# jhyau/AdaptiGraph

Hardware: AMD Instinct MI355X
Metric: rollout-steps/sec (higher is better)
Workload: dtype f32; 1 GPU; BASELINE configs[3]: cloth, 1024 candidates x 20 rollout steps (2 look-ahead x repeat 10) x 2025+1 particles, radius graph rebuilt every step; candidates=1024, horizon=20, particles=2026, parallelism=candidates sharded over 1 GPU(s), all-gather of costs

## Files before the change

### adaptigraph_amd/csrc/ag_api.hip

```cpp
#include "ag_host.h"

#include <cstdarg>

using namespace ag;

namespace {

const char* kFamilyNames[FAM_COUNT] = {"edge_count", "edge_emit", "prep", "node_enc", "edge_enc",
                                       "mp", "node_prop", "node_final", "roll_init", "roll_update", "cost", "fps", "assemble", "rule", "surface"};

struct OptName { const char* name; const char* env; int Options::* field; bool env_negates; int lo, hi; };
const OptName kOptions[] = {
    {"streams", "AG_STREAMS", &Options::streams, false, 0, ag_ctx::kMaxStreams},
    {"chunk", "AG_CHUNK", &Options::chunk, false, 0, 1 << 20},
    {"latency", "AG_LATENCY", &Options::latency, false, -1, 1},
    {"ragged", "AG_NO_RAGGED", &Options::ragged, true, 0, 1},
    {"ell_graph", "AG_NO_ELL_GRAPH", &Options::ell_graph, true, 0, 1},
    {"self_dedupe", "AG_NO_SELF_DEDUPE", &Options::self_dedupe, true, 0, 1},
    {"repeat_sort", "AG_NO_REPEAT_SORT", &Options::repeat_sort, true, 0, 1},
    {"edge_wgs", "AG_EDGE_WGS", &Options::edge_wgs, false, 1, 1 << 16},
    {"edge_block_min", "AG_EDGE_BLOCK_MIN", &Options::edge_block_min, false, -1, 0x7fffffff},
    {"enc_persist", "AG_ENC_PERSIST", &Options::enc_persist, false, 0, 1 << 20},
    {"stagger_us", "AG_STAGGER_US", &Options::stagger_us, false, 0, 1000},
    {"device_decode", "AG_DEVICE_DECODE", &Options::device_decode, false, -1, 1},
    {"zigzag", "AG_ZIGZAG", &Options::zigzag, false, 0, 1},
    {"share_first", "AG_SHARE_FIRST", &Options::share_first, false, -1, 1},
    {"zero_skip", "AG_ZERO_SKIP", &Options::zero_skip, false, 0, 1},
    {"half_step", "AG_HALF_STEP", &Options::half_step, false, 0, 1},
    {"share_prefix", "AG_SHARE_PREFIX", &Options::share_prefix, false, -1, 1},
    {"stream_min_rows", "AG_STREAM_MIN_ROWS", &Options::stream_min_rows, false, 0, 0x7fffffff},
    {"pipeline_fork", "AG_PIPELINE_FORK", &Options::pipeline_fork, false, 0, 1},
    {"edge_order", "AG_EDGE_ORDER", &Options::edge_order, false, 0, 1},
    {"ell_lds_words", "AG_ELL_LDS_WORDS", &Options::ell_lds_words, false, 0, 16384},
};
void options_from_env(Options& o) {
    for (const OptName& n : kOptions)
        if (const char* e = getenv(n.env)) o.*(n.field) = n.env_negates ? (atoi(e) ? 0 : 1) : std::min(n.hi, std::max(n.lo, atoi(e)));
}

}

namespace ag {

int fail(ag_ctx* c, int code, const char* fmt, ...) {
    char buf[512];
    va_list ap;
    va_start(ap, fmt);
    vsnprintf(buf, sizeof buf, fmt, ap);
    va_end(ap);
    if (c) c->err = buf;
    return code;
}

int slot_acquire(ag_ctx* c, hipStream_t st, bool capturing, CallSlot** out) {
    CallSlot* s = nullptr;
    for (CallSlot& k : c->slots) if (k.bound && k.stream == st) { s = &k; break; }
    if (!s) for (CallSlot& k : c->slots) if (!k.bound) { s = &k; break; }
    if (!s) {
        s = &c->slots[0];
        for (CallSlot& k : c->slots) if (k.tick < s->tick) s = &k;
        if (!capturing && s->have_done) HIPCHK(c, hipStreamWaitEvent(st, s->ev_done, 0));
        s->census_pending = false;
    }
    if (!s->ev_done) {
        HIPCHK(c, event_new(c, &s->ev_done));
        HIPCHK(c, event_new(c, &s->ev_plan));
        HIPCHK(c, event_new(c, &s->ev_census));
        HIPCHK(c, event_new(c, &s->ev_fork));
        HIPCHK(c, dev_alloc(c, reinterpret_cast<void**>(&s->d_words), 256));
        HIPCHK(c, dev_alloc(c, reinterpret_cast<void**>(&s->d_share_stats), 256));
        HIPCHK(c, hipMemset(s->d_share_stats, 0, 256));
        HIPCHK(c, pin_alloc(c, reinterpret_cast<void**>(&s->h_census), 64));
    }
    s->bound = true; s->stream = st; s->tick = ++c->slot_tick;
    *out = s;
    return AG_OK;
}
void slot_release(CallSlot* s, hipStream_t st, bool capturing) {
    if (capturing || !s || !s->ev_done) return;
    if (hipEventRecord(s->ev_done, st) == hipSuccess) s->have_done = true;
}
bool other_slot_busy(ag_ctx* c, const CallSlot* me) {
    bool busy = false;
    for (CallSlot& k : c->slots)
        if (&k != me && k.bound && k.have_done) {
            if (hipEventQuery(k.ev_done) == hipErrorNotReady) busy = true;
            (void)hipGetLastError();
        }
    return busy;
}
int begin_call(ag_ctx* c, void* stream, SlotGuard& call, bool watch_capture) {
    HIPCHK(c, hipSetDevice(c->device));
    call.st = static_cast<hipStream_t>(stream);
    c->prof_stream = call.st;
    if (watch_capture) {
        hipStreamCaptureStatus status = hipStreamCaptureStatusNone;
        call.capturing = hipStreamIsCapturing(call.st, &status) == hipSuccess && status == hipStreamCaptureStatusActive;
    }
    return slot_acquire(c, call.st, call.capturing, &call.sl);
}
void slot_destroy(ag_ctx* c, CallSlot& s) {
    for (hipEvent_t e : {s.ev_plan, s.ev_census, s.ev_done, s.ev_fork}) if (e) (void)hipEventDestroy(e);
    for (int i = 1; i < CallSlot::kMaxStreams; ++i) {
        if (s.ev_join[i]) (void)hipEventDestroy(s.ev_join[i]);
        if (s.aux_stream[i]) (void)hipStreamDestroy(s.aux_stream[i]);
    }
    if (s.h_plan_max) (void)hipHostFree(s.h_plan_max);
    if (s.h_rep_pin) (void)hipHostFree(s.h_rep_pin);
    if (s.h_census) (void)hipHostFree(s.h_census);
    if (s.d_words) (void)hipFree(s.d_words);
    if (s.d_share_stats) (void)hipFree(s.d_share_stats);
    if (s.d_repeat) (void)hipFree(s.d_repeat);
    if (s.d_plan) (void)hipFree(s.d_plan);
    if (s.d_work) (void)hipFree(s.d_work);
    if (s.slab.base) (void)hipFree(s.slab.base);
    s = CallSlot();
}

void prof_mark(void* vc, int fam, int phase) {
    ag_ctx* c = static_cast<ag_ctx*>(vc);
    if (!(c->prof_mask & (1u << fam))) return;
    auto get = [&]() {
        hipEvent_t e;
        if (!c->prof_pool.empty()) { e = c->prof_pool.back(); c->prof_pool.pop_back(); }
        else (void)hipEventCreate(&e);
        return e;
    };
    if (phase == 0) {
        ProfEvent p{fam, get(), get()};
        (void)hipEventRecord(p.e0, c->prof_stream);
        c->prof_live.push_back(p);
    } else {
        for (auto it = c->prof_live.rbegin(); it != c->prof_live.rend(); ++it)
            if (it->fam == fam) { (void)hipEventRecord(it->e1, c->prof_stream); break; }
    }
}

void carve_work(const ag_ctx* c, Slab& s, Work& w, int Bc, int N, int n_inst, int edge_cap, int c_cap, int slices, bool own_edges,
                bool roll, bool own_group, int N_o, int ell_stride) {
    const size_t rows = (size_t)Bc * N;
    w.g.node_in = s.take<float>(rows * NODE_IN);
    w.g.feat12 = s.take<float>(rows * F15_PITCH);
    w.g.group = own_group ? s.take<float>(rows * n_inst) : nullptr;
    w.g.eff = s.take<float>(rows * NFP);
    w.g.P = s.take<float>(rows * NFP);
    for (int par = 0; par < 2; ++par)
        for (int k = 0; k < 2; ++k) w.g.UV[par][k] = s.take<float>(rows * NFP);
    w.g.C = s.take<float>(((size_t)Bc * c_cap + 256) * NFP);
    w.g.B = Bc; w.g.N = N; w.g.n_inst = n_inst; w.g.edge_cap = edge_cap; w.g.c_cap = c_cap; w.g.n_p = N_o;
    w.g.enc_persist = c->opt.enc_persist; w.g.stagger_us = c->opt.stagger_us; w.g.zigzag = c->opt.zigzag; w.g.diag = c->diag;
    w.g.zero_skip = c->opt.zero_skip && c->w_finite; w.g.half_step = w.g.zero_skip && c->opt.half_step;
    if (own_edges) {
        w.ell = s.take<int>(rows * (size_t)std::max(1, ell_stride));
        w.deg = s.take<int>(rows);
        w.slice_tot = s.take<int>((size_t)Bc * slices);
        w.cta_flag = s.take<int>(Bc);
        w.recv = s.take<int>((size_t)Bc * edge_cap);
        w.send = s.take<int>((size_t)Bc * edge_cap);
        w.row_ptr = s.take<int>((size_t)Bc * (N + 1));
        w.n_edges = s.take<int>(Bc);
        w.ns_edge = s.take<int>((size_t)Bc * edge_cap);
        w.n_ns = s.take<int>(Bc);
        w.n_oo = s.take<int>(Bc);
        w.g.recv = w.recv; w.g.send = w.send; w.g.row_ptr = w.row_ptr; w.g.n_edges = w.n_edges;
    }
    if (roll) {
        w.send_pk = s.take<int>((size_t)Bc * edge_cap);
        w.rowlist = s.take<int>(rows);
        w.n_rows = s.take<int>((size_t)Bc + 64);
        w.r.hist = s.take<float>((size_t)Bc * N_HIS_MAX * N * 3);
        w.r.pred = s.take<float>((size_t)Bc * N_o * 3);
        w.r.motion = s.take<float>((size_t)Bc * N_o * 3);
        w.r.mask = s.take<uint8_t>(rows);
        w.r.tool = s.take<uint8_t>(rows);
        const size_t cr = (size_t)cls_rows(N_o, N - N_o, Bc);
        w.g.cls_on = 1; w.g.N_o = N_o; w.g.M = N - N_o; w.g.vmask = w.r.mask;
        w.g.c_node_in = s.take<float>(cr * NODE_IN);
        w.g.c_eff = s.take<float>(cr * NFP);
        w.g.c_P = s.take<float>(cr * NFP);
        w.g.c_U = s.take<float>(cr * NFP);
        w.g.c_V = s.take<float>(cr * NFP);
    }
}

int pick_slices(const ag_ctx* c, int B, int N) {
    const int target = std::max(1, c->opt.edge_wgs);
    int s = (target + B - 1) / B;
    s = std::min(s, std::max(1, N / 16));
    return std::max(1, std::min(s, 128));
}

int clamp_chunk_for_offsets(int Bc, int N, int c_cap) {
    const long max_rows = ((1L << 32) / NFP) - 512;
    const long by_c = max_rows / std::max(1, c_cap);
    const long by_n = max_rows / std::max(1, N);
    return (int)std::max(1L, std::min<long>(Bc, std::min(by_c, by_n)));
}

int auto_chunk(const ag_ctx* c, int B, int N) {
    if (c->chunk > 0) return std::min(c->chunk, B);
    if (c->opt.chunk > 0) return std::min(c->opt.chunk, B);
    const long max_rows = 4L * 256 * 256;
    long bc = max_rows / N;
    return (int)std::max(1L, std::min<long>(bc, B));
}

bool lat_available(const ag_ctx* c, const GraphBufs& g) { return c->d_wlat && !g.wb3 && g.n_his != 5; }
bool lat_edge_for(const ag_ctx* c, const GraphBufs& g) {
    const long edge_wgs = (long)g.B * g.c_cap / 128;
    return lat_available(c, g) && (c->opt.latency >= 0 ? c->opt.latency == 1 : edge_wgs <= 128);
}
hipError_t node_enc_for(const ag_ctx* c, const GraphBufs& g, long row0, long nrows, hipStream_t st) {
    const long rows = g.cls_on ? nrows : (long)g.B * g.N;
    const bool lat = lat_available(c, g) && (c->opt.latency >= 0 ? c->opt.latency == 1 : rows <= 512L * 32);
    return lat ? launch_node_enc_lat(c->d_wlat, g, row0, nrows, st) : launch_node_enc(c->d_w, g, row0, nrows, st);
}
bool lat_node_for(const ag_ctx* c, const GraphBufs& g) {
    const long node_wgs = ((long)g.B * g.N + 127) / 128;
    return lat_available(c, g) && (c->opt.latency >= 0 ? c->opt.latency == 1 : node_wgs <= 64);
}
int run_edge_chain(ag_ctx* c, const GraphBufs& g, hipStream_t st) {
    Scoped p(c, FAM_EDGE_ENC);
    if (lat_edge_for(c, g)) HIPCHK(c, launch_edge_enc_lat(c->d_wlat, g, st));
    else HIPCHK(c, launch_edge_enc(c->d_w, g, st));
    return AG_OK;
}

int run_model(ag_ctx* c, const GraphBufs& g, float* pred_pos, float* pred_motion, hipStream_t st) {
    if (!g.cls_on) { Scoped p(c, FAM_NODE_ENC); HIPCHK(c, node_enc_for(c, g, 0, (long)g.B * g.N, st)); }
    const bool lat_node = lat_node_for(c, g);
    if (g.send_pk && lat_node) return fail(c, AG_ERR_INVALID, "internal: shared first forward on the latency-mode chains");
    int rc = run_edge_chain(c, g, st);
    if (rc) return rc;
    for (int ps = 0; ps < c->dims.pstep; ++ps) {
        const bool last = ps + 1 == c->dims.pstep;
        Scoped p(c, last ? FAM_NODE_FINAL : FAM_NODE_PROP);
        if (lat_node) HIPCHK(c, launch_node_prop_lat(c->d_wlat, g, ps, last, c->dims.motion_clamp, pred_pos, pred_motion, st));
        else if (!last) HIPCHK(c, launch_node_prop(c->d_w, g, ps, st));
        else HIPCHK(c, launch_node_final(c->d_w, g, ps, c->dims.motion_clamp, pred_pos, pred_motion, st));
    }
    return AG_OK;
}

struct SelfMini { float node_in[2 * NODE_IN]; float feat12[2 * F15_PITCH]; float group[2]; int recv[2]; int send[2]; int n_edges; int pad; };
int enqueue_self_rows(ag_ctx* c, hipStream_t st) {
    HIPCHK(c, hipSetDevice(c->device));
    if (!c->d_cself) HIPCHK(c, dev_alloc(c, reinterpret_cast<void**>(&c->d_cself), 256 * NFP * 4));
    if (!c->d_self_mini) {
        SelfMini h{};
        h.node_in[0] = 1.f; h.node_in[6] = 1.f;
        h.node_in[NODE_IN + 1] = 1.f; h.node_in[NODE_IN + 6] = 1.f;
        h.group[0] = 1.f;
        h.recv[0] = 0; h.recv[1] = 1; h.send[0] = 0; h.send[1] = 1; h.n_edges = 2;
        HIPCHK(c, dev_alloc(c, reinterpret_cast<void**>(&c->d_self_mini), sizeof(SelfMini)));
        HIPCHK(c, hipMemcpy(c->d_self_mini, &h, sizeof(SelfMini), hipMemcpyHostToDevice));
    }
    char* d = c->d_self_mini;
    GraphBufs g{};
    g.n_his = c->dims.n_his;
    g.node_in = reinterpret_cast<float*>(d + offsetof(SelfMini, node_in));
    g.feat12 = reinterpret_cast<float*>(d + offsetof(SelfMini, feat12));
    g.group = reinterpret_cast<float*>(d + offsetof(SelfMini, group));
    g.recv = reinterpret_cast<int*>(d + offsetof(SelfMini, recv));
    g.send = reinterpret_cast<int*>(d + offsetof(SelfMini, send));
    g.n_edges = reinterpret_cast<int*>(d + offsetof(SelfMini, n_edges));
    g.C = c->d_cself; g.B = 1; g.N = 2; g.n_p = 1; g.n_inst = 1; g.edge_cap = 2; g.c_cap = 256;
    g.wb3 = c->precision == 1 ? c->d_wb3 : nullptr;
    hipError_t e = launch_edge_enc(c->d_w, g, st);
    if (e != hipSuccess) return fail(c, AG_ERR_HIP, "self-loop C rows: %s", hipGetErrorString(e));
    return AG_OK;
}
int compute_self_rows(ag_ctx* c) {
    int rc = enqueue_self_rows(c, nullptr);
    if (rc) return rc;
    hipError_t e = hipDeviceSynchronize();
    if (e != hipSuccess) return fail(c, AG_ERR_HIP, "self-loop C rows: %s", hipGetErrorString(e));
    return AG_OK;
}

int check_topk(ag_ctx* c, int N, int topk) {
    if (N < 1 || topk < 1) return fail(c, AG_ERR_INVALID, "N and topk must be >= 1");
    if ((size_t)N > edge_build_max_particles()) return fail(c, AG_ERR_UNSUPPORTED, "N=%d exceeds the LDS-resident edge builder limit %zu", N, edge_build_max_particles());
    if (topk < N && topk > 128) return fail(c, AG_ERR_UNSUPPORTED, "topk=%d: 128 < topk < N is not implemented", topk);
    return AG_OK;
}

ForwardFrame::ForwardFrame(const ag_ctx* c, int B, int N_, int n_inst_, int edge_cap_, int n_p_, int n_guard_)
    : N(N_), n_inst(n_inst_), edge_cap(edge_cap_), n_p(n_p_), n_guard(n_guard_), c_cap((int)round_up(edge_cap_, 256)),
      Bc(clamp_chunk_for_offsets(auto_chunk(c, B, N_), N_, c_cap)) {}
void ForwardFrame::carve(const ag_ctx* c, Slab& s) {
    carve_work(c, s, w, Bc, N, n_inst, edge_cap, c_cap, 1, false, false, false, n_p, 0);
    n_eff = n_guard ? s.take<int>((size_t)n_guard) : nullptr;
}

int enqueue_forward(ag_ctx* c, const ForwardFrame& f, const float* d_state, const float* d_attrs, const float* d_action,
                    const float* d_phys, const float* d_group, const int32_t* d_recv, const int32_t* d_send,
                    const int32_t* d_row_ptr, const int* n_eff, int B, float* d_pred_pos, float* d_pred_motion, hipStream_t st) {
    const int Bc = f.Bc, N = f.N, n_inst = f.n_inst, edge_cap = f.edge_cap, n_p = f.n_p;
    int rc = AG_OK;
    for (int b0 = 0; b0 < B; b0 += Bc) {
        const int nb = std::min(Bc, B - b0);
        GraphBufs g = f.w.g;
        g.B = nb; g.n_p = n_p; g.n_his = c->dims.n_his;
        g.wb3 = c->precision == 1 ? c->d_wb3 : nullptr;
        g.group = const_cast<float*>(d_group) + (size_t)b0 * N * n_inst;
        g.recv = d_recv + (size_t)b0 * edge_cap; g.send = d_send + (size_t)b0 * edge_cap;
        g.row_ptr = d_row_ptr + (size_t)b0 * (N + 1); g.n_edges = n_eff + b0; g.n_guard = n_eff + b0;
        { Scoped p(c, FAM_PREP);
          HIPCHK(c, launch_prep(d_state + (size_t)b0 * c->dims.n_his * N * 3, d_attrs + (size_t)b0 * N * 2,
                                d_action + (size_t)b0 * N * 3, d_phys + (size_t)b0 * N, g, st)); }
        rc = run_model(c, g, d_pred_pos + (size_t)b0 * n_p * 3, d_pred_motion + (size_t)b0 * n_p * 3, st);
        if (rc) return rc;
    }
    return AG_OK;
}

// ... 321 lines not shown
```

### adaptigraph_amd/csrc/ag_api_rollout.hip

```cpp
#include "ag_host.h"

using namespace ag;

namespace {
struct ActionSrc {
    const float* d_eef_xz = nullptr; const float* d_eef_delta = nullptr; const int32_t* h_repeat = nullptr;
    const float* d_action = nullptr; float push_length = 0.f; const float* h_tool_off = nullptr; int max_repeat = 0;
    float* d_action_seqs = nullptr;
    int32_t* h_work = nullptr;
};

struct RollCall {
    ag_ctx* c = nullptr; const ag_rollout_params* p = nullptr; const ActionSrc* src = nullptr;
    const float* d_state0 = nullptr; const uint8_t* d_obj_mask = nullptr; const float* d_phys_vec = nullptr;
    float* d_state_seqs = nullptr; int32_t* d_overflow = nullptr;
    hipStream_t st = nullptr; CallSlot* sl = nullptr;
    bool capturing = false, dev_plan = false, work_only = false;
    int N = 0, n_his = 0, R = 0;
    size_t nrep = 0;
    int k = 0, edge_cap = 0;
    bool dedupe = false, ell_full = false, ragged = false, sort_on = false;
    int ns = 1, Bc = 1, Ba = 1, slices = 1, ell = 0, n_chunks_all = 0;
    bool prefix = false, auto_prefix = false, base_in_ctx = false, share = false;
    int R_base = 0, kb = 0, base_cap = 0, base_slices = 0;
// ... 105 lines not shown
            r.b_zero = s.take<int>(1);
        }
        for (int i = 0; i < r.ns; ++i)
            carve_work(c, s, r.ws[i], r.Ba, r.N, 1, r.edge_cap, r.edge_cap, r.slices, true, true, true, p->N_o, r.ell);
        if (r.share) {
            RollCall::BaseGraph& b = r.bg;
            b.C = s.take<float>((size_t)r.base_cap * NFP);
            b.send = s.take<int>(r.base_cap); b.recv = s.take<int>(r.base_cap); b.ns = s.take<int>(r.base_cap);
            b.node_in = s.take<float>((size_t)p->N_o * NODE_IN); b.feat = s.take<float>((size_t)p->N_o * F15_PITCH);
            b.group = s.take<float>(p->N_o); b.deg = s.take<int>(p->N_o);
            b.mask = s.take<uint8_t>(p->N_o); b.tool = s.take<uint8_t>(p->N_o);
            b.slice_tot = s.take<int>(r.base_slices); b.cta = s.take<int>(1);
            b.n_edges = s.take<int>(1); b.n_ns = s.take<int>(1);
        }
    });
    if (rc) return rc;
    if (r.prefix || r.work_only) return grow(c, true, sl.h_rep_pin, sl.rep_pin_cap, 2 * nrep + 8, 2 * nrep + 64);
    return AG_OK;
}

int upload_host_plan(RollCall& r, const int32_t* rep_src) {
    ag_ctx* c = r.c; const ag_rollout_params* p = r.p; CallSlot& sl = *r.sl; const size_t nrep = r.nrep; const int Bc = r.Bc;
    int rc = grow(c, false, sl.d_repeat, sl.repeat_cap, 2 * nrep, 2 * nrep + (nrep >> 2));
    if (rc) return rc;
    sl.h_repeat.resize(2 * nrep);
    if (rep_src != sl.h_repeat.data()) std::copy(rep_src, rep_src + nrep, sl.h_repeat.begin());
    const int32_t* h_repeat = r.h_repeat = sl.h_repeat.data();
    int* h_cand = r.h_cand = sl.h_repeat.data() + nrep;
    for (int li = 0; li < p->H; ++li)
        for (int b0 = 0; b0 < p->B; b0 += Bc) {
            const int nb = std::min(Bc, p->B - b0);
            int* seg = h_cand + (size_t)li * p->B + b0;
            for (int b = 0; b < nb; ++b) seg[b] = b0 + b;
            if (r.sort_on)
                std::stable_sort(seg, seg + nb, [&](int x, int y) { return h_repeat[(size_t)x * p->H + li] > h_repeat[(size_t)y * p->H + li]; });
        }
    HIPCHK(c, hipMemcpyAsync(sl.d_repeat, h_repeat, 2 * nrep * 4, hipMemcpyHostToDevice, r.st));
    return AG_OK;
}

int launch_device_plan(RollCall& r) {
    ag_ctx* c = r.c; const ag_rollout_params* p = r.p; CallSlot& sl = *r.sl; const size_t nrep = r.nrep; const int R = r.R;
    const size_t tab = (size_t)r.n_chunks_all * p->H * (R + 2);
    const size_t n_int = 2 * nrep + 2 * tab + (size_t)r.n_chunks_all * p->H * 3;
    const size_t n_flt = nrep * p->M * 5;
    const size_t bytes = round_up(n_int * 4, 256) + n_flt * 4;
    int rc = grow(c, false, sl.d_plan, sl.plan_cap, bytes, bytes + (bytes >> 2));
    if (rc) return rc;
    r.pl_repeat = reinterpret_cast<int*>(sl.d_plan); r.pl_cand = r.pl_repeat + nrep; r.pl_live = r.pl_cand + nrep;
    r.pl_rows = r.pl_live + tab; r.pl_sums = r.pl_rows + tab;
    float* pl_xz = reinterpret_cast<float*>(sl.d_plan + round_up(n_int * 4, 256)); float* pl_delta = pl_xz + nrep * p->M * 2;
    RollPlan rp{};
    rp.action = r.src->d_action; rp.push_length = r.src->push_length; rp.M = p->M;
    for (int kk = 1; kk < p->M; ++kk) rp.tool_off[kk] = r.src->h_tool_off[kk];
    rp.B = p->B; rp.H = p->H; rp.Bc = r.Bc; rp.N = r.N; rp.max_repeat = R;
    rp.decoded = r.src->d_action_seqs; rp.eef_xz = pl_xz; rp.eef_delta = pl_delta; rp.repeat = r.pl_repeat; rp.cand = r.pl_cand;
    rp.live = r.pl_live; rp.rows = r.pl_rows; rp.sums = r.pl_sums; rp.flags = r.d_overflow; rp.sort = r.sort_on ? 1 : 0;
    rp.maxrep = r.pl_sums + (size_t)r.n_chunks_all * p->H * 2;
    HIPCHK(c, launch_roll_plan(rp, r.st));
    const size_t n_max = (size_t)r.n_chunks_all * p->H;
    rc = grow(c, true, sl.h_plan_max, sl.plan_max_cap, n_max, n_max + 64);
    if (rc) return rc;
    if (!r.capturing) {
        HIPCHK(c, hipMemcpyAsync(sl.h_plan_max, rp.maxrep, n_max * 4, hipMemcpyDeviceToHost, r.st));
        HIPCHK(c, hipEventRecord(sl.ev_plan, r.st));
    }
    r.d_eef_xz = pl_xz; r.d_eef_delta = pl_delta;
    c->d_plan_sums = r.pl_sums; c->plan_sums_n = r.n_chunks_all * p->H;
    c->fwd_executed = -1; c->fwd_needed = -1;
    return AG_OK;
}

int contact_plan_and_wait(RollCall& r, const float* base_states, const float* base_y, int R, const int* d_cnt) {
    ag_ctx* c = r.c; const ag_rollout_params* p = r.p; CallSlot& sl = *r.sl; const size_t nrep = r.nrep; hipStream_t st = r.st;
    ContactPlan cp{};
    cp.base_states = base_states; cp.base_y = base_y; cp.R = R;
    cp.R_bound = r.dev_plan ? r.R : 0x7fffffff;
    cp.eef_xz = r.d_eef_xz; cp.eef_delta = r.d_eef_delta; cp.repeat = r.rep_orig();
    cp.B = p->B; cp.H = p->H; cp.N_o = p->N_o; cp.M = p->M; cp.thr = p->adj_thresh; cp.rep_eff = r.b_rep_eff; cp.start = r.b_start;
    cp.state_seqs = r.d_state_seqs;
    HIPCHK(c, launch_contact_plan(cp, st));
    HIPCHK(c, hipMemcpyAsync(sl.h_rep_pin, r.b_rep_eff, nrep * 4, hipMemcpyDeviceToHost, st));
    if (r.dev_plan) HIPCHK(c, hipMemcpyAsync(sl.h_rep_pin + nrep, r.pl_repeat, nrep * 4, hipMemcpyDeviceToHost, st));
    HIPCHK(c, hipMemcpyAsync(sl.h_rep_pin + 2 * nrep, r.d_overflow, 4, hipMemcpyDeviceToHost, st));
    if (d_cnt) HIPCHK(c, hipMemcpyAsync(sl.h_rep_pin + 2 * nrep + 1, d_cnt, 16, hipMemcpyDeviceToHost, st));
    HIPCHK(c, hipEventRecord(sl.ev_plan, st));
    HIPCHK(c, hipEventSynchronize(sl.ev_plan));
    return AG_OK;
}

int decide_prefix(RollCall& r) {
    ag_ctx* c = r.c; const ag_rollout_params* p = r.p; CallSlot& sl = *r.sl; hipStream_t st = r.st;
    BaseKey& key = r.key;
    memset(&key, 0, sizeof key);
    key.N_o = p->N_o; key.M = p->M; key.topk = p->topk; key.cta = p->connect_tools_all;
    key.max_nR = p->max_nR; key.n_his = r.n_his; key.precision = c->precision;
    key.pstep = c->dims.pstep; key.grip_on = p->gripper_enable; key.thr = p->adj_thresh;
    key.grip = p->gripper_offset; key.phys = p->physics_param; key.clamp = c->dims.motion_clamp;
    key.phys_vec = r.d_phys_vec; key.weights_version = c->weights_version;
    for (CallSlot& q : c->slots)
        if (q.census_pending && !r.capturing) {
            if (hipEventQuery(q.ev_census) == hipSuccess) {
                q.census_pending = false;
                const int free_now = q.h_census[1] - q.h_census[0], rb = std::min(q.census_R, std::max(1, q.h_census[2]));
                if (c->decision.decline && c->decision.B == q.census_B && c->decision.H == q.census_H &&
                    memcmp(&c->decision.key, &q.census_key, sizeof(BaseKey)) == 0 && free_now >= std::max(64, 8 * rb))
                    c->decision.decline = false;
            } else (void)hipGetLastError();
        }
    if (!r.auto_prefix) return AG_OK;
    int* d_cnt = sl.d_words + 8;
    const bool key_ok = c->base_cache_R >= 1 && !r.d_phys_vec && memcmp(&key, &c->base_key, sizeof key) == 0;
    const bool declined = !key_ok && c->decision.decline && c->decision.B == p->B && c->decision.H == p->H &&
                          memcmp(&key, &c->decision.key, sizeof key) == 0;
    if (declined) {
        r.prefix = false;
        if (sl.census_pending) return AG_OK;
    }
    ContactPlan cen{};
    cen.base_states = r.d_state0; cen.R = 1; cen.eef_xz = r.d_eef_xz; cen.eef_delta = r.d_eef_delta; cen.repeat = r.rep_orig();
    cen.B = p->B; cen.H = p->H; cen.N_o = p->N_o; cen.M = p->M; cen.thr = p->adj_thresh;
    cen.grip = p->gripper_offset; cen.grip_on = p->gripper_enable; cen.count = d_cnt;
    HIPCHK(c, hipMemsetAsync(d_cnt, 0, 16, st));
    HIPCHK(c, launch_contact_plan(cen, st));
    if (declined) {
        HIPCHK(c, hipMemcpyAsync(sl.h_census, d_cnt, 16, hipMemcpyDeviceToHost, st));
        HIPCHK(c, hipEventRecord(sl.ev_census, st));
        sl.census_pending = true; sl.census_B = p->B; sl.census_H = p->H; sl.census_R = r.R_base;
        memcpy(&sl.census_key, &key, sizeof key);
        return AG_OK;
    }
    const int* h_cnt = nullptr;
    if (key_ok) {
        HIPCHK(c, launch_count_diff(r.d_state0, c->d_base_cache, (long)p->N_o * 3, d_cnt + 3, st));
        const int rc = contact_plan_and_wait(r, c->d_base_cache, c->d_base_cache + (size_t)(c->base_cache_capR + 1) * p->N_o * 3,
                                             c->base_cache_R, d_cnt);
        if (rc) return rc;
        h_cnt = sl.h_rep_pin + 2 * r.nrep + 1;
    } else {
        HIPCHK(c, hipMemcpyAsync(sl.h_census + 4, d_cnt, 16, hipMemcpyDeviceToHost, st));
        HIPCHK(c, hipEventRecord(sl.ev_plan, st));
        HIPCHK(c, hipEventSynchronize(sl.ev_plan));
        h_cnt = sl.h_census + 4;
    }
    r.R_base = std::min(r.R_base, std::max(1, h_cnt[2]));
    r.kept = key_ok && h_cnt[3] == 0 && c->base_cache_R >= r.R_base;
    if (key_ok && !r.kept && r.d_state_seqs) HIPCHK(c, hipMemsetAsync(r.d_state_seqs, 0, (size_t)p->B * p->H * p->N_o * 3 * 4, st));
    if (!r.kept && h_cnt[1] - h_cnt[0] < std::max(64, 8 * r.R_base)) r.prefix = false;
    c->decision.decline = !r.prefix;
    if (!r.prefix) { memcpy(&c->decision.key, &key, sizeof key); c->decision.B = p->B; c->decision.H = p->H; }
    return AG_OK;
}

int workspace_graph(RollCall& r, Work& w, int nb, hipStream_t s, GraphBufs& g) {
    ag_ctx* c = r.c;
    g = w.g;
    g.B = nb; g.n_p = r.p->N_o; g.n_his = r.n_his;
    g.wb3 = c->precision == 1 ? c->d_wb3 : nullptr;
    if (r.dedupe) {
        g.c_self = c->d_cself; g.ns_edge = w.ns_edge; g.n_ns = w.n_ns;
        g.n_oo = r.ell_full && c->opt.edge_order ? w.n_oo : nullptr;
        g.self_row = (long)r.Ba * r.edge_cap;
        HIPCHK(c, hipMemcpyAsync(w.g.C + (size_t)g.self_row * NFP, c->d_cself, 2 * NFP * 4, hipMemcpyDeviceToDevice, s));
    }
    if (r.ell_full) { g.deg = w.deg; g.ell_stride = r.k + r.p->M; }
    w.r.ragged = r.ragged ? 1 : 0; w.r.clamp = c->dims.motion_clamp;
    return AG_OK;
}

EdgeArgs workspace_edge_args(const RollCall& r, const Work& w, int nb) {
    const ag_rollout_params* p = r.p; const int N = r.N, n_his = r.n_his;
    EdgeArgs ea{};
    ea.pos = w.r.hist + (size_t)(n_his - 1) * N * 3; ea.pos_bstride = (long)n_his * N * 3;
    ea.mask = w.r.mask; ea.tool = w.r.tool; ea.thr_vec = nullptr; ea.thr = p->adj_thresh;
    ea.B = nb; ea.N = N; ea.topk = p->topk; ea.cta = p->connect_tools_all ? 1 : 0; ea.edge_cap = r.edge_cap;
    ea.slices = r.slices; ea.ell = w.ell; ea.deg = w.deg; ea.slice_tot = w.slice_tot; ea.cta_flag = w.cta_flag;
    ea.recv = w.recv; ea.send = w.send; ea.row_ptr = w.row_ptr; ea.n_edges = w.n_edges;
    ea.overflow = r.d_overflow; ea.max_nR = p->max_nR; ea.zero_on_overflow = 1; ea.block_min_rows = r.c->opt.edge_block_min;
    if (r.ell_full) {
        ea.ell_full = 1; ea.ell = w.send; ea.ell_stride = r.k + p->M; ea.ell_bstride = r.edge_cap;
        ea.ns_edge = w.ns_edge; ea.n_ns = w.n_ns;
        ea.n_oo = r.c->opt.edge_order ? w.n_oo : nullptr; ea.lds_words = r.c->opt.ell_lds_words;
    }
    return ea;
}

RollArgs roll_args(const RollCall& r, int b0, int nb) {
    const ag_rollout_params* p = r.p;
    RollArgs ra{};
    ra.B = nb; ra.B_slots = nb; ra.b0 = b0; ra.N_o = p->N_o; ra.M = p->M;
    ra.grip = p->gripper_offset; ra.grip_on = p->gripper_enable; ra.phys = p->physics_param; ra.phys_vec = r.d_phys_vec;
    ra.state0 = r.d_state0;
    return ra;
}

int build_shared_base_graph(RollCall& r) {
    ag_ctx* c = r.c; const ag_rollout_params* p = r.p; hipStream_t st = r.st; const int base_cap = r.base_cap;
    const RollCall::BaseGraph& b = r.bg;
    HIPCHK(c, launch_share_prep(r.d_state0, p->N_o, r.n_his, b.node_in, b.feat, b.group, b.mask, b.tool, st));
    EdgeArgs be{};
    be.pos = r.d_state0; be.pos_bstride = (long)p->N_o * 3; be.mask = b.mask; be.tool = b.tool; be.thr = p->adj_thresh;
    be.B = 1; be.N = p->N_o; be.topk = p->topk; be.cta = 0; be.edge_cap = base_cap; be.slices = r.base_slices;
    be.ell_full = 1; be.ell = b.send; be.ell_stride = r.kb; be.ell_bstride = base_cap; be.deg = b.deg;
    be.slice_tot = b.slice_tot; be.cta_flag = b.cta; be.recv = b.recv; be.send = b.send; be.n_edges = b.n_edges;
    be.ns_edge = b.ns; be.n_ns = b.n_ns; be.max_nR = 0x7fffffff; be.block_min_rows = c->opt.edge_block_min;
    HIPCHK(c, launch_edge_build(be, st, prof_mark, c));
    GraphBufs gb{};
    gb.node_in = b.node_in; gb.feat12 = b.feat; gb.group = b.group; gb.C = b.C; gb.recv = b.recv; gb.send = b.send;
    gb.n_edges = b.n_edges; gb.ns_edge = b.ns; gb.n_ns = b.n_ns; gb.B = 1; gb.N = p->N_o; gb.n_p = p->N_o; gb.n_inst = 1;
    gb.edge_cap = base_cap; gb.c_cap = base_cap; gb.n_his = r.n_his; gb.wb3 = c->precision == 1 ? c->d_wb3 : nullptr;
    gb.diag = c->diag; gb.zero_skip = c->opt.zero_skip && c->w_finite; gb.half_step = gb.zero_skip && c->opt.half_step;
    int rc = run_edge_chain(c, gb, st);
    if (rc) return rc;
    r.base_send = b.send; r.base_deg = b.deg; r.C_share = b.C; c->d_share_nns = b.n_ns;
    return AG_OK;
}

int run_base_rollout(RollCall& r) {
    ag_ctx* c = r.c; const ag_rollout_params* p = r.p; hipStream_t st = r.st;
    const float far = 1.0e6f;
    int far_bits; memcpy(&far_bits, &far, 4);
    HIPCHK(c, hipMemsetD32Async(reinterpret_cast<hipDeviceptr_t>(r.b_eef), far_bits, (size_t)2 * p->M, st));
    HIPCHK(c, hipMemsetAsync(r.b_eef + 2 * p->M, 0, (size_t)3 * p->M * 4, st));
    HIPCHK(c, hipMemsetAsync(r.b_zero, 0, 4, st));
    HIPCHK(c, hipMemcpyAsync(r.b_states, r.d_state0, (size_t)p->N_o * 3 * 4, hipMemcpyDeviceToDevice, st));
    Work& w = r.ws[0];
    GraphBufs g;
    int rc = workspace_graph(r, w, 1, st, g);
    if (rc) return rc;
    RollArgs ra = roll_args(r, 0, 1);
    ra.H = 1; ra.eef_xz = r.b_eef; ra.eef_delta = r.b_eef + 2 * p->M; ra.repeat = r.b_zero;
    ra.write_obj_cls = 1; ra.all_states = r.b_states; ra.all_y = r.b_y;
    const EdgeArgs ea = workspace_edge_args(r, w, 1);
    { Scoped sc(c, FAM_ROLL_INIT); HIPCHK(c, launch_roll_init(ra, w.r, g, st)); }
    { Scoped sc(c, FAM_NODE_ENC); HIPCHK(c, node_enc_for(c, g, 0, 2L * p->N_o + p->M, st)); }
    for (int ai = 1; ai <= r.R_base; ++ai) {
        HIPCHK(c, launch_edge_build(ea, st, prof_mark, c));
        if (g.ns_edge && !r.ell_full) { Scoped sc(c, FAM_EDGE_EMIT); HIPCHK(c, launch_edge_nonself(w.recv, w.send, w.row_ptr, 1, r.N, r.edge_cap, w.ns_edge, w.n_ns, nullptr, st)); }
        rc = run_model(c, g, w.r.pred, w.r.motion, st);
        if (rc) return rc;
        ra.ai = ai;
        { Scoped sc(c, FAM_ROLL_UPDATE); HIPCHK(c, launch_roll_update(ra, w.r, g, st)); }
    }
    return AG_OK;
}

int run_prefix(RollCall& r) {
    ag_ctx* c = r.c; const ag_rollout_params* p = r.p; CallSlot& sl = *r.sl; const size_t nrep = r.nrep;
    int rc = AG_OK;
    if (r.base_in_ctx) {
        const size_t row = (size_t)p->N_o * 3 + 1;
        if (!r.kept) {
            for (CallSlot& q : c->slots)
                if (&q != &sl && q.bound && q.have_done) HIPCHK(c, hipStreamWaitEvent(r.st, q.ev_done, 0));
            c->base_cache_R = -1;
            const size_t need = (size_t)(r.R_base + 1) * row;
            rc = grow(c, false, c->d_base_cache, c->base_cache_cap, need, std::max(need, (size_t)((r.dev_plan ? r.R : r.R_base) + 1) * row));
            if (rc) return rc;
            c->base_cache_capR = (int)(c->base_cache_cap / row) - 1;
        }
        r.b_states = c->d_base_cache; r.b_y = c->d_base_cache + (size_t)(c->base_cache_capR + 1) * p->N_o * 3;
    }
    if (!r.kept) {
        rc = run_base_rollout(r);
        if (rc) return rc;
        rc = contact_plan_and_wait(r, r.b_states, r.b_y, r.R_base, nullptr);
        if (rc) return rc;
        if (r.base_in_ctx) {
            const bool clean = sl.h_rep_pin[2 * nrep] <= p->max_nR;
            c->base_cache_R = clean ? r.R_base : -1;
            memcpy(&c->base_key, &r.key, sizeof r.key);
        }
    }
    if (r.dev_plan) {
        c->fwd_needed = 0;
        for (size_t i = 0; i < nrep; ++i) c->fwd_needed += std::min(std::max(0, sl.h_rep_pin[nrep + i]), r.R);
        c->d_plan_sums = nullptr;
    }
    c->fwd_executed = r.kept ? 0 : r.R_base;
    if (!r.work_only) {
        rc = upload_host_plan(r, sl.h_rep_pin);
        if (rc) return rc;
    }
    r.d_start = r.b_start; r.d_base_states = r.b_states; r.d_base_y = r.b_y;
    return AG_OK;
}

int report_work(RollCall& r) {
    ag_ctx* c = r.c; const ag_rollout_params* p = r.p; CallSlot& sl = *r.sl;
    if (!r.prefix) {
        HIPCHK(c, hipMemcpyAsync(sl.h_rep_pin, r.pl_repeat, r.nrep * 4, hipMemcpyDeviceToHost, r.st));
        HIPCHK(c, hipEventRecord(sl.ev_plan, r.st));
        HIPCHK(c, hipEventSynchronize(sl.ev_plan));
    }
    for (int b = 0; b < p->B; ++b) {
        long w = 0;
        for (int li = 0; li < p->H; ++li) w += std::min(std::max(0, sl.h_rep_pin[(size_t)b * p->H + li]), r.R);
        r.src->h_work[b] = (int32_t)w;
    }
    c->d_plan_sums = nullptr;
    return AG_OK;
}

int enqueue_chunks(RollCall& r) {
    ag_ctx* c = r.c; const ag_rollout_params* p = r.p; CallSlot& sl = *r.sl;
    const int N = r.N, ns = r.ns, Bc = r.Bc, R = r.R; const size_t nrep = r.nrep; const int32_t* h_repeat = r.h_repeat;
    const bool loop_dev = r.dev_plan && !r.prefix;
    int fail_at = -1, timing_skip = 0;
#ifdef AG_DIAG
    fail_at = diag_fail_at_chunk(c->diag);
    timing_skip = diag_timing_skip(c->diag);
#endif
    bool obj_cls_ready[ag_ctx::kMaxStreams] = {false, false, false, false};
    bool plan_landed = false;
    c->steps_enqueued = 0; c->steps_bound = 0;
    int ci = 0;
    for (int b0 = 0; b0 < p->B; b0 += Bc, ++ci) {
        if (ci == fail_at) return fail(c, AG_ERR_HIP, "test hook: injected failure before chunk %d", ci);
        const int nb = std::min(Bc, p->B - b0);
        Work& w = r.ws[ci % ns];
        hipStream_t cs = r.streams[ci % ns];
        c->prof_stream = cs;
        GraphBufs g;
        int rc = workspace_graph(r, w, nb, cs, g);
        if (rc) return rc;
        RollArgs ra = roll_args(r, b0, nb);
        ra.H = p->H; ra.y_mode = p->y_mode; ra.state0_batched = p->y_mode == 1; ra.obj_mask = r.d_obj_mask;
        ra.eef_xz = r.d_eef_xz; ra.eef_delta = r.d_eef_delta; ra.repeat = loop_dev ? r.pl_repeat : sl.d_repeat; ra.state_seqs = r.d_state_seqs;
        ra.start = r.d_start; ra.base_states = r.d_base_states; ra.base_y = r.d_base_y;
        EdgeArgs ea = workspace_edge_args(r, w, nb);
        if (r.ragged) {
            const int* d_cand0 = r.sort_on ? sl.d_repeat + nrep + b0 : nullptr;
            HIPCHK(c, launch_build_rowlist(r.d_obj_mask, d_cand0, b0, nb, p->N_o, p->M, w.rowlist, w.n_rows, w.r.mask, w.deg, cs));
            HIPCHK(c, hipMemsetAsync(w.row_ptr + (size_t)nb * (N + 1), 0, (size_t)(N + 1) * 4, cs));
            g.rowlist = w.rowlist; g.n_rows = w.n_rows + nb;
        }
        for (int li = 0; li < p->H; ++li) {
            const int* seg = loop_dev ? nullptr : r.h_cand + (size_t)li * p->B + b0;
            int max_rep = loop_dev ? R : 0;
            if (!loop_dev) for (int b = 0; b < nb; ++b) max_rep = std::max(max_rep, h_repeat[(size_t)seg[b] * p->H + li]);
            if (max_rep == 0 && !loop_dev) continue;
            ra.li = li; ra.ai = 0; ra.B = nb; ra.live = nullptr;
            ra.cand = loop_dev ? r.pl_cand + (size_t)li * p->B + b0 : r.sort_on ? sl.d_repeat + nrep + (size_t)li * p->B + b0 : nullptr;
            const int* live_row = loop_dev ? r.pl_live + ((size_t)ci * p->H + li) * (R + 2) : nullptr;
            const int* rows_row = loop_dev ? r.pl_rows + ((size_t)ci * p->H + li) * (R + 2) : nullptr;
            ra.write_obj_cls = obj_cls_ready[ci % ns] ? 0 : 1;
            { Scoped s(c, FAM_ROLL_INIT); HIPCHK(c, launch_roll_init(ra, w.r, g, cs)); }
            { Scoped s(c, FAM_NODE_ENC);
              const long tool0 = 2L * p->N_o;
              if (!obj_cls_ready[ci % ns]) HIPCHK(c, node_enc_for(c, g, 0, tool0 + (long)nb * p->M, cs));
              else HIPCHK(c, node_enc_for(c, g, tool0, (long)nb * p->M, cs)); }
            obj_cls_ready[ci % ns] = true;
            int n_live = nb;
            c->steps_bound += max_rep;
            for (int ai = 1; ai <= max_rep; ++ai) {
                if (loop_dev) {
                    if (!plan_landed && ai > 1 && !r.capturing) {
                        if (hipEventQuery(sl.ev_plan) == hipSuccess) plan_landed = true;
                        else (void)hipGetLastError();
                    }
                    if (plan_landed && ai > sl.h_plan_max[(size_t)ci * p->H + li]) break;
                }
                ++c->steps_enqueued;
                if (loop_dev) {
                    ea.live = live_row + ai; ra.live = live_row + ai; g.n_rows = rows_row + ai;
                } else {
                    if (r.sort_on) while (n_live > 0 && h_repeat[(size_t)seg[n_live - 1] * p->H + li] < ai) --n_live;
                    c->fwd_executed += n_live;
                    if (r.ragged) g.n_rows = w.n_rows + n_live;
                }
                ea.B = n_live; g.B = n_live; ra.B = n_live;
                const bool share_step = r.share && li == 0 && ai == 1 && !lat_node_for(c, g);
                ea.send_pk = share_step ? w.send_pk : nullptr; g.send_pk = ea.send_pk;
                if (share_step) {
                    ea.base_send = r.base_send; ea.base_deg = r.base_deg; ea.base_stride = r.kb; ea.share_No = p->N_o;
                    ea.share_stats = sl.d_share_stats; g.C_share = r.C_share; g.share_kb = r.kb;
                    ea.share_start = r.d_start; ea.share_cand = ra.cand; ea.share_b0 = b0;
                }
                if (!(timing_skip & 1) || ai == 1) {
                    HIPCHK(c, launch_edge_build(ea, cs, prof_mark, c));
                    if (g.ns_edge && !r.ell_full) { Scoped s(c, FAM_EDGE_EMIT); HIPCHK(c, launch_edge_nonself(w.recv, w.send, w.row_ptr, n_live, N, r.edge_cap, w.ns_edge, w.n_ns, ea.live, cs)); }
                }
                rc = run_model(c, g, w.r.pred, w.r.motion, cs);
                if (rc) return rc;
                ra.ai = ai;
                if (!(timing_skip & 2) || ai == max_rep) { Scoped s(c, FAM_ROLL_UPDATE); HIPCHK(c, launch_roll_update(ra, w.r, g, cs)); }
            }
        }
    }
    return AG_OK;
}

int rollout_impl(ag_ctx* c, void* stream, const ag_rollout_params* p, const float* d_state0, const uint8_t* d_obj_mask,
                 const ActionSrc& src, const float* d_phys_vec, float* d_state_seqs, int32_t* d_overflow_flag) {
    int rc = check_rollout_args(c, p, d_state0, src, d_state_seqs, d_overflow_flag);
    if (rc) return rc;
    RollCall r;
    SlotGuard call;
    rc = begin_call(c, stream, call, true);
    if (rc) return rc;
    r.c = c; r.p = p; r.src = &src; r.st = call.st; r.sl = call.sl; r.capturing = call.capturing;
    r.d_state0 = d_state0; r.d_obj_mask = d_obj_mask; r.d_phys_vec = d_phys_vec; r.d_state_seqs = d_state_seqs; r.d_overflow = d_overflow_flag;
    r.dev_plan = src.d_action != nullptr; r.work_only = src.h_work != nullptr; r.R = src.max_repeat;
    r.h_repeat = src.h_repeat; r.d_eef_xz = src.d_eef_xz; r.d_eef_delta = src.d_eef_delta;
    r.N = p->N_o + p->M; r.n_his = c->dims.n_his;
    r.nrep = (size_t)p->B * p->H;
    c->last_slot = (int)(r.sl - c->slots);
    c->d_share_nns = nullptr;
    if (d_state_seqs) HIPCHK(c, hipMemsetAsync(d_state_seqs, 0, (size_t)p->B * p->H * p->N_o * 3 * 4, r.st));

    plan_launch(r);
    rc = reserve_call_memory(r);
    if (rc) return rc;
    rc = r.dev_plan ? launch_device_plan(r) : upload_host_plan(r, src.h_repeat);
    if (rc) return rc;
    if (!r.dev_plan) {
        c->fwd_executed = 0; c->fwd_needed = 0;
        for (size_t i = 0; i < r.nrep; ++i) c->fwd_needed += std::max(0, r.h_repeat[i]);
    }
    rc = decide_prefix(r);
    if (rc) return rc;
    HIPCHK(c, hipMemsetAsync(r.sl->d_share_stats, 0, 16, r.st));
    if (r.share) {
        rc = build_shared_base_graph(r);
        if (rc) return rc;
    }
    if (r.prefix) {
        rc = run_prefix(r);
        if (rc) return rc;
    }
    if (r.work_only) return report_work(r);
    CallSlot& sl = *r.sl;
    for (hipStream_t& s : r.streams) s = r.st;
    if (r.ns > 1) {
        HIPCHK(c, hipEventRecord(sl.ev_fork, r.st));
        for (int i = 1; i < r.ns; ++i) {
            if (!sl.aux_stream[i]) {
                HIPCHK(c, stream_new(c, &sl.aux_stream[i]));
                HIPCHK(c, event_new(c, &sl.ev_join[i]));
            }
            r.streams[i] = sl.aux_stream[i];
            HIPCHK(c, hipStreamWaitEvent(sl.aux_stream[i], sl.ev_fork, 0));
        }
    }
    const int rc_loop = enqueue_chunks(r);
    int rc_join = AG_OK;
    for (int i = 1; i < r.ns; ++i) {
        hipError_t e = hipEventRecord(sl.ev_join[i], sl.aux_stream[i]);
        if (e == hipSuccess) e = hipStreamWaitEvent(r.st, sl.ev_join[i], 0);
        if (e != hipSuccess && rc_join == AG_OK && rc_loop == AG_OK)
            rc_join = fail(c, AG_ERR_HIP, "joining stream %d failed: %s", i, hipGetErrorString(e));
    }
    c->prof_stream = r.st;
    return rc_loop ? rc_loop : rc_join;
}
}

extern "C" {

int ag_rollout_async(ag_ctx* c, void* stream, const ag_rollout_params* p, const float* d_state0,
                     const uint8_t* d_obj_mask, const float* d_eef_xz, const float* d_eef_delta,
                     const int32_t* h_repeat, const float* d_phys_vec, float* d_state_seqs, int32_t* d_overflow_flag) {
    ActionSrc src;
    src.d_eef_xz = d_eef_xz; src.d_eef_delta = d_eef_delta; src.h_repeat = h_repeat;
    if (c && (!d_eef_xz || !d_eef_delta || !h_repeat)) return fail(c, AG_ERR_INVALID, "ag_rollout: null pointer");
    return rollout_impl(c, stream, p, d_state0, d_obj_mask, src, d_phys_vec, d_state_seqs, d_overflow_flag);
}

int ag_rollout_actions(ag_ctx* c, void* stream, const ag_rollout_params* p, const float* d_state0, const float* d_action,
                       float push_length, const float* h_tool_offsets, int32_t max_repeat, const float* d_phys_vec,
                       float* d_state_seqs, float* d_action_seqs, int32_t* d_flags) {
    if (!c) return AG_ERR_INVALID;
    if (!d_action || !d_action_seqs || !d_flags) return fail(c, AG_ERR_INVALID, "ag_rollout_actions: null pointer");
    ActionSrc src;
    src.d_action = d_action; src.push_length = push_length; src.h_tool_off = h_tool_offsets; src.max_repeat = max_repeat;
    src.d_action_seqs = d_action_seqs;
    return rollout_impl(c, stream, p, d_state0, nullptr, src, d_phys_vec, d_state_seqs, d_flags);
}

int ag_rollout_work(ag_ctx* c, void* stream, const ag_rollout_params* p, const float* d_state0, const float* d_action,
                    float push_length, const float* h_tool_offsets, int32_t max_repeat, const float* d_phys_vec, int32_t* h_work) {
    if (!c) return AG_ERR_INVALID;
    if (!p || !d_action || !h_work) return fail(c, AG_ERR_INVALID, "ag_rollout_work: null pointer");
    SlotGuard call;
    int rc = begin_call(c, stream, call);
    if (rc) return rc;
    hipStream_t st = call.st; CallSlot* sl = call.sl;
    const size_t nrep = (size_t)p->B * p->H;
    rc = grow(c, false, sl->d_work, sl->work_cap, nrep * 4 + 64, (nrep * 4 + 64) * 2);
    if (rc) return rc;
    HIPCHK(c, hipMemsetAsync(sl->d_work, 0, 64 * 4, st));
    ActionSrc src;
    src.d_action = d_action; src.push_length = push_length; src.h_tool_off = h_tool_offsets; src.max_repeat = max_repeat;
    src.d_action_seqs = sl->d_work + 64; src.h_work = h_work;
    return rollout_impl(c, stream, p, d_state0, nullptr, src, d_phys_vec, nullptr, reinterpret_cast<int32_t*>(sl->d_work));
}

int ag_rollout(ag_ctx* c, void* stream, const ag_rollout_params* p, const float* d_state0, const uint8_t* d_obj_mask,
               const float* d_eef_xz, const float* d_eef_delta, const int32_t* h_repeat, const float* d_phys_vec,
               float* d_state_seqs) {
    if (!c) return AG_ERR_INVALID;
    SlotGuard call;
    int rc = begin_call(c, stream, call);
    if (rc) return rc;
    hipStream_t st = call.st; CallSlot* sl = call.sl;
    int* d_word = sl->d_words;
    HIPCHK(c, hipMemsetAsync(d_word, 0, 4, st));
    rc = ag_rollout_async(c, stream, p, d_state0, d_obj_mask, d_eef_xz, d_eef_delta, h_repeat, d_phys_vec, d_state_seqs, d_word);
    if (rc) return rc;
    int seen = 0;
    HIPCHK(c, hipMemcpyAsync(&seen, d_word, 4, hipMemcpyDeviceToHost, st));
    HIPCHK(c, hipStreamSynchronize(st));
    if (seen > p->max_nR) return fail(c, AG_ERR_MAX_NR, "Exceeds max dims: a graph had %d edges, max_nR=%d", seen, p->max_nR);
    return AG_OK;
}

}
```

### adaptigraph_amd/csrc/ag_common.h

```cpp
#pragma once
#include <hip/hip_runtime.h>
#include <stdint.h>

namespace ag {

constexpr int NF = 150;
constexpr int NFP = 160;
constexpr int ONE_F = 150;
constexpr int N_HIS = 4;
constexpr int IN_DIM = 6;
constexpr int REL_DIM = 17;
constexpr int F12 = 3 * N_HIS;
constexpr int N_HIS_MAX = 5;
constexpr int F15_PITCH = 16;
inline int feat_pitch(int n_his) { return n_his == 5 ? F15_PITCH : F12; }
constexpr int NODE_IN = 8;

constexpr int KSTEPS = 76;
constexpr int KCH = 19;
constexpr int KCH_H0 = 10;
constexpr int KCH_H1 = KCH - KCH_H0;
constexpr int CHUNK_FLOATS_MB5 = 5 * 64 * 4;
constexpr int CHUNK_FLOATS_MB1 = 1 * 64 * 4;
constexpr int HALF0_FLOATS = KCH_H0 * CHUNK_FLOATS_MB5;
constexpr int HALF1_FLOATS = KCH_H1 * CHUNK_FLOATS_MB5;
constexpr int LAYER_FLOATS = HALF0_FLOATS + HALF1_FLOATS;
constexpr int EDGE_L1_CHUNKS = 3;
constexpr int NODE_L1_CHUNKS = 1;
constexpr int OUT3_FLOATS = KCH * CHUNK_FLOATS_MB1;

struct WeightLayout {
    static constexpr int E_L1 = 0;
    static constexpr int E_L2 = E_L1 + EDGE_L1_CHUNKS * CHUNK_FLOATS_MB5;
    static constexpr int E_L3 = E_L2 + LAYER_FLOATS;
    static constexpr int E_W1 = E_L3 + LAYER_FLOATS;
    static constexpr int N_L1 = E_W1 + LAYER_FLOATS;
    static constexpr int N_L2 = N_L1 + NODE_L1_CHUNKS * CHUNK_FLOATS_MB5;
    static constexpr int N_L3 = N_L2 + LAYER_FLOATS;
    static constexpr int N_WA = N_L3 + LAYER_FLOATS;
    static constexpr int N_W2 = N_WA + LAYER_FLOATS;
    static constexpr int N_W3 = N_W2 + LAYER_FLOATS;
    static constexpr int P_WB = N_W3 + LAYER_FLOATS;
    static constexpr int P_P0 = P_WB + LAYER_FLOATS;
    static constexpr int P_P1 = P_P0 + LAYER_FLOATS;
    static constexpr int P_P2 = P_P1 + LAYER_FLOATS;
    static constexpr int TOTAL = P_P2 + OUT3_FLOATS;
};

#ifndef AG_ZS_EDGE
#define AG_ZS_EDGE 2
#endif
#ifndef AG_ZS_ENC
#define AG_ZS_ENC 0
#endif
#ifndef AG_ZS_NODE
#define AG_ZS_NODE 1
#endif
#ifndef AG_HS_EDGE
#define AG_HS_EDGE 1
#endif
#ifndef AG_HS_NODE
#define AG_HS_NODE 1
#endif
constexpr bool ZS_EDGE = AG_ZS_EDGE != 0, ZS_EDGE_ALL = AG_ZS_EDGE == 2, ZS_ENC = AG_ZS_ENC != 0, ZS_NODE = AG_ZS_NODE != 0;
constexpr bool HS_EDGE = ZS_EDGE && AG_HS_EDGE != 0, HS_NODE = ZS_NODE && AG_HS_NODE != 0;

enum Family { FAM_EDGE_COUNT = 0, FAM_EDGE_EMIT, FAM_PREP, FAM_NODE_ENC, FAM_EDGE_ENC, FAM_MP, FAM_NODE_PROP,
              FAM_NODE_FINAL, FAM_ROLL_INIT, FAM_ROLL_UPDATE, FAM_COST, FAM_FPS, FAM_ASSEMBLE, FAM_RULE, FAM_SURFACE, FAM_COUNT };

struct Options {
    int streams = 0;
    int chunk = 0;
    int latency = -1;
    int ragged = 1;
    int ell_graph = 1;
    int self_dedupe = 1;
    int repeat_sort = 1;
    int edge_wgs = 256;
    int edge_block_min = -1;
    int enc_persist = 0;
    int stagger_us = 0;
    int zigzag = 1;
    int device_decode = -1;
    int share_prefix = -1;
    int stream_min_rows = 32768;
    int pipeline_fork = 0;
    int zero_skip = 1;
    int half_step = 1;
    int edge_order = 1;
    int ell_lds_words = 0;
    int share_first = -1;
};

struct EdgeArgs {
    const float* pos;
    long pos_bstride;
    const uint8_t* mask;
    const uint8_t* tool;
    const float* thr_vec;
    float thr;
    float thr2_override; int use_thr2;
    const float* thr2_vec;
    int B, N, topk, cta, edge_cap, slices;
    int* ell;
    int* deg;
    int* slice_tot;
    int* cta_flag;
    int* recv; int* send;
    int* row_ptr;
    int* n_edges;
    int* overflow;
    int max_nR;
    int zero_on_overflow;
    int ell_full; int ell_stride; long ell_bstride;
    int* ns_edge; int* n_ns;
    int* n_oo; int lds_words;
    int block_min_rows;
    const int* live;
    int* send_pk; const int* base_send; const int* base_deg; int base_stride; int share_No;
    unsigned long long* share_stats;
    const int* share_start; const int* share_cand; int share_b0;
};
hipError_t launch_edge_build(const EdgeArgs& a, hipStream_t st, void (*mark)(void*, int, int), void* mark_ctx);
struct FpsArgs {
    const float* pos; const long long* pt_off; const long long* npts; int stride;
    const int* fps_start; const float* fps_radius; const int* rad_start;
    int B, max_nobj, max_pts;
    int* fps_idx; int* n_obj;
};
hipError_t launch_fps_batch(const FpsArgs& a, hipStream_t st);
size_t fps_max_points();
int fps_max_nobj();
hipError_t launch_fps_cloud(const FpsArgs& a, float* ws, hipStream_t st);
size_t fps_cloud_max_points();
size_t fps_cloud_switch_points();
size_t fps_cloud_ws_floats(int B, int max_pts);
struct RuleArgs {
    const float* pos; const uint8_t* mask; const uint8_t* tool; const uint8_t* subset;
    const int* send_in; const int* row_ptr_in;
    int N, n_tools, edge_cap, use_knn; double kNN;
    int* tlist; int* misc; float* pdis; uint8_t* keep; uint8_t* kept;
    int* recv; int* send; int* row_ptr; int* n_out;
};
hipError_t launch_tool_rule(const RuleArgs& a, hipStream_t st);
struct RuleGraphsBase {
    const float* pos; long pos_bstride; const uint8_t* mask; const uint8_t* tool;
    const int* send_in; const int* row_ptr_in; const int* n_edges_in; int base_cap;
    int B, N, n_tools, edge_cap;
    const float* bnd_pos; long bnd_points; const long long* bnd_first; const int* bnd_idx; int idx_stride; const int* bnd_n;
    int pad_rows; float ratio;
    int* recv; int* send; int* row_ptr; int* n_out;
};
constexpr int RULE_GRAPHS_MAX_PAIRS = 8192;
constexpr int RULE_GRAPHS_MAX_TOOLS = 64;
struct RuleGraphsArgs {
    RuleGraphsBase g;
    const double* kNN; float* thr_out;
};
hipError_t launch_rule_graphs(const RuleGraphsArgs& a, hipStream_t st);
struct SurfaceGraphsArgs {
    RuleGraphsBase g;
    int bounds_order; float one_minus_ratio;
    float* bounds_out; int* planes_out;
};
hipError_t launch_surface_graphs(const SurfaceGraphsArgs& a, hipStream_t st);
hipError_t launch_edge_nonself(const int* recv, const int* send, const int* row_ptr, int B, int N, int edge_cap,
                               int* ns_edge, int* n_ns, const int* live, hipStream_t st);

struct GraphBufs {
    float* node_in;
    float* feat12;
    float* group;
    float* eff;
    float* P;
    float* UV[2][2];
    float* C;
    const int* recv; const int* send; const int* row_ptr; const int* n_edges;
    const int* deg; int ell_stride;
    int B, N, n_p, n_inst;
    int edge_cap;
    int c_cap;
    int cls_on, N_o, M;
    const uint8_t* vmask;
    float* c_node_in;
    float* c_eff; float* c_P; float* c_U; float* c_V;
    const float* c_self;
    long self_row;
    const int* ns_edge; const int* n_ns;
    const int* n_oo;
    const float* wb3;
    const int* n_guard;
    const int* rowlist; const int* n_rows;
    const int* send_pk; const float* C_share; int share_kb;
    int n_his;
    int enc_persist, stagger_us, zigzag;
    int zero_skip;
    int half_step;
    void* diag;
};
constexpr int B3_PHASE_BYTES = 2 * 5 * 3 * 64 * 16;
constexpr int B3_PHASES = 58;
inline long cls_rows(int N_o, int M, int B) { return 2L * N_o + (long)B * M; }
hipError_t launch_node_enc(const float* wblob, const GraphBufs& g, long row0, long nrows, hipStream_t st);
hipError_t launch_edge_enc(const float* wblob, const GraphBufs& g, hipStream_t st);
hipError_t launch_node_prop(const float* wblob, const GraphBufs& g, int round, hipStream_t st);
hipError_t launch_node_final(const float* wblob, const GraphBufs& g, int round, float clamp, float* pred_pos,
                             float* pred_motion, hipStream_t st);

hipError_t launch_edge_guard(const int* n_edges, int B, int edge_cap, int* n_eff, int* overflow, hipStream_t st);
hipError_t launch_prep(const float* state, const float* attrs, const float* action, const float* phys,
                       const GraphBufs& g, hipStream_t st);

struct RollBufs {
    float* hist;
    float* pred;
    float* motion;
    int ragged;
    float clamp;
    uint8_t* mask;
    uint8_t* tool;
};
struct RollArgs {
    int B, N_o, M, H, li, ai, y_mode, b0;
    int B_slots;
    float grip; int grip_on; float phys;
    int write_obj_cls;
    const float* phys_vec;
    const float* state0; int state0_batched;
    const uint8_t* obj_mask;
    const float* eef_xz; const float* eef_delta;
    const int* repeat;
    const int* live;
    const int* cand;
    float* state_seqs;
    const float* base_states; const float* base_y; const int* start;
    float* all_states; float* all_y;
};
struct ContactPlan {
    const float* base_states; const float* base_y; int R;
    const float* eef_xz; const float* eef_delta; const int* repeat;
    int B, H, N_o, M; float thr;
    int* rep_eff;
    int* start;
    float* state_seqs;
    int* count; float grip; int grip_on;
    int R_bound;
};
hipError_t launch_count_diff(const float* a, const float* b, long n, int* count, hipStream_t st);
hipError_t launch_contact_plan(const ContactPlan& p, hipStream_t st);
hipError_t launch_chamfer(const float* x, const float* y, const uint8_t* xm, const uint8_t* ym, int R, int N, int M,
                          int By, float* out, hipStream_t st);
hipError_t launch_state_stats(const float* state, int R, int N, const float* box4, float* out, hipStream_t st);
hipError_t launch_penalty(const float* state_pred, const float* action, const float* state_init, int B, int H, int N,
                          int kind, float ratio, float* out, hipStream_t st);
size_t chamfer_max_points();
hipError_t launch_chamfer_backward(const float* x, const float* y, const uint8_t* xm, const uint8_t* ym, int R, int N, int M,
                                   int By, const float* gout, int* nn, float* cnt, float* gx, hipStream_t st);
hipError_t launch_reward(const float* error, const float* pen, const float* stats, const float* emax, const double* bbox4, int B,
                         int H, float* out, hipStream_t st);
hipError_t launch_cloth_combine(const float* raw, const float* dmax, long n, float* out, hipStream_t st);

hipError_t launch_mppi_sample(const float* act_seq, const float* lo, const float* hi, const float* rnd,
                              const float* scale, int S, int H, int mode, float pl, float* out, hipStream_t st);
hipError_t launch_mppi_update(const float* acts, const float* reward, const float* lo, const float* hi, int B, int H,
                              float rw, float pl, float* out, hipStream_t st);
hipError_t launch_mppi_clip(const float* in, const float* lo, const float* hi, float* out, long n, hipStream_t st);

struct RollPlan {
    const float* action;
    float push_length; int M; float tool_off[8];
    int B, H, Bc, N, max_repeat;
    float* decoded;
    float* eef_xz; float* eef_delta; int* repeat;
    int* cand;
    int* live; int* rows;
    int* sums;
    int* maxrep;
    int* flags;
    int sort;
};
hipError_t launch_roll_plan(const RollPlan& p, hipStream_t st);

hipError_t launch_build_rowlist(const uint8_t* obj_mask, const int* cand, int b0, int B, int N_o, int M, int* rowlist, int* tab,
                                uint8_t* mask, int* deg, hipStream_t st);
hipError_t launch_share_prep(const float* state0, int N_o, int n_his, float* node_in, float* feat, float* group, uint8_t* mask,
                             uint8_t* tool, hipStream_t st);
hipError_t launch_roll_init(const RollArgs& a, const RollBufs& r, const GraphBufs& g, hipStream_t st);
hipError_t launch_roll_update(const RollArgs& a, const RollBufs& r, const GraphBufs& g, hipStream_t st);

struct TrainArgs {
    const float* state; const float* attrs; const float* action; const float* phys; const float* group; int n_inst;
    const int* recv; const int* send; const int* row_ptr; const int* n_edges; int edge_cap;
    int B, N, n_p, n_his, pstep; float clamp;
    int Ep;
    const float* w[22]; float* g[22];
    const float* dpos; const float* dmot;
    float* dstate;
    float* dphys; float* daction;
    bool want_w;
    bool wide;
};
size_t train_slab_floats();
size_t train_work_floats(int Bc, int N, int Ep, int n_his, int pstep);
size_t train_work_ints(int Bc, int N, int Ep);
hipError_t train_backward_chunk(const TrainArgs& t, int b0, int nb, float* wsf, int* wsi, float* slab, hipStream_t st);

void pack_weights_host(int rel_dim, const float* const* t, float* blob, uint16_t* b3, float* lat);
hipError_t launch_pack_weights(int rel_dim, const float* const* d_t, float* d_blob, uint16_t* d_b3, float* d_lat, hipStream_t st);
void weight_tensor_sizes(int rel_dim, int* n22);
struct AdamArgs {
    float* w[22]; const float* g[22]; float* m[22]; float* v[22]; int n[22];
    float wd, one_minus_b1, b2, one_minus_b2, bc2_sqrt, eps, neg_step_size;
    int* status;
};
hipError_t launch_adam(const AdamArgs& a, hipStream_t st);
size_t train_glue_doubles();
hipError_t launch_step_loss(const float* pred, const float* fut, int B, int n_p, int n_future, int fi, int B_total, int accumulate,
                            double* part, float* loss, hipStream_t st);
hipError_t launch_next_state(const float* state, const float* pred, const float* eef, const float* act_f, int B, int N, int n_p,
                             int n_his, int n_future, int fi, int rest, float* state_next, float* action_next, hipStream_t st);
hipError_t launch_pred_grad(const float* pred, const float* fut, const float* dnext, int B, int N, int n_p, int n_his, int n_future,
                            int fi, int B_total, float* dpos, hipStream_t st);
hipError_t launch_dstate_carry(float* d, const float* dnext, int B, int N, int n_his, int rest, hipStream_t st);
hipError_t launch_mse_part(const float* pred, const float* fut, int B, int n_p, int n_future, int fi, double* part, hipStream_t st);
hipError_t launch_pred_grad_scaled(const float* pred, const float* fut, const float* dnext, int B, int N, int n_p, int n_his,
                                   int n_future, int fi, float mse_scale, float* dpos, hipStream_t st);

constexpr int SET_LOSS_MSE = 0, SET_LOSS_CHAMFER = 1, SET_LOSS_HAUSDORFF = 2, SET_LOSS_EMD = 3;
constexpr int SET_LOSS_ROWS = 16;
struct SetRows {
    const int* nx; const int* ny;
};
__device__ __forceinline__ int clamp_count(int v, int n) { return v < 0 ? 0 : (v > n ? n : v); }
__device__ __forceinline__ void set_rows_of(const SetRows& r, int b, int N, int M, int& nx, int& ny) {
    nx = clamp_count(r.nx[b], N); ny = clamp_count(r.ny[b], M);
    if (nx == 0 || ny == 0) nx = ny = 0;
}
__device__ __forceinline__ float set_dist(float ax, float ay, float az, float bx, float by, float bz) {
    const float dx = __fsub_rn(ax, bx), dy = __fsub_rn(ay, by), dz = __fsub_rn(az, bz);
    return __fsqrt_rn(__fadd_rn(__fadd_rn(__fmul_rn(dx, dx), __fmul_rn(dy, dy)), __fmul_rn(dz, dz)));
}
__device__ __forceinline__ void set_pull(const float* xi, const float* yj, float s, float (&g)[3]) {
// ... 85 lines not shown
```

### adaptigraph_amd/csrc/ag_diag.hip

```cpp
#ifdef AG_DIAG
#include "ag_common.h"
#include <algorithm>
#include <cstdio>
#include <cstdlib>
#include <vector>

namespace ag {

struct Diag {
    int clock_left = 0, node_left = 0, fail_at_chunk = -1, timing_skip = 0;
    bool node_tail = false;
    unsigned long long* dbg_e = nullptr; unsigned cap_e = 0;
    unsigned long long* dbg_n = nullptr; unsigned cap_n = 0; unsigned tail_nwg = 0;
};

void* diag_create() {
    Diag* d = new Diag();
    if (const char* e = getenv("AG_CLOCK_PROBE")) d->clock_left = atoi(e);
    if (const char* e = getenv("AG_NODE_PROBE")) { const int v = atoi(e); d->node_left = v > 0 ? v : 0; d->node_tail = v < 0; }
    if (const char* e = getenv("AG_TEST_FAIL_AT_CHUNK")) d->fail_at_chunk = atoi(e);
    if (const char* e = getenv("AG_TIMING_SKIP")) d->timing_skip = atoi(e);
    return d;
}
int diag_fail_at_chunk(void* v) { return v ? static_cast<Diag*>(v)->fail_at_chunk : -1; }
int diag_timing_skip(void* v) { return v ? static_cast<Diag*>(v)->timing_skip : 0; }

static double node_clock(const std::vector<unsigned long long>& h, unsigned nwg, int* n_out) {
    double ghz = 0; int n = 0;
    for (unsigned i = 0; i < nwg; ++i) {
        const unsigned long long c0 = h[(size_t)nwg * 5 + 2 * i], c1 = h[(size_t)nwg * 5 + 2 * i + 1];
        if (c1 > c0 && h[4 * i + 3] > h[4 * i]) { ghz += (double)(c1 - c0) / (double)(h[4 * i + 3] - h[4 * i]) * 0.1; ++n; }
    }
    *n_out = n;
    return n ? ghz / n : 0.0;
}

void diag_destroy(void* v) {
    Diag* d = static_cast<Diag*>(v);
    if (!d) return;
    if (d->node_tail && d->dbg_n && d->tail_nwg) {
        (void)hipDeviceSynchronize();
        std::vector<unsigned long long> h((size_t)d->tail_nwg * 7);
        (void)hipMemcpy(h.data(), d->dbg_n, (size_t)d->tail_nwg * 56, hipMemcpyDeviceToHost);
        int n = 0;
        const double ghz = node_clock(h, d->tail_nwg, &n);
        if (n) fprintf(stderr, "[ag node probe] last k_node_prop<false> launch of the context: in-kernel clock %.3f GHz over %d workgroups\n", ghz, n);
    }
    if (d->dbg_e) (void)hipFree(d->dbg_e);
    if (d->dbg_n) (void)hipFree(d->dbg_n);
    delete d;
}

unsigned long long* diag_edge_begin(void* v, unsigned nwg, hipStream_t st) {
    Diag* d = static_cast<Diag*>(v);
    if (!d || d->clock_left <= 0) return nullptr;
    if (d->cap_e < nwg) { if (d->dbg_e) (void)hipFree(d->dbg_e); (void)hipMalloc((void**)&d->dbg_e, (size_t)nwg * 32); d->cap_e = nwg; }
    (void)hipMemsetAsync(d->dbg_e, 0, (size_t)nwg * 32, st);
    return d->dbg_e;
}
void diag_edge_end(void* v, unsigned nwg, hipStream_t st) {
    Diag* d = static_cast<Diag*>(v);
    --d->clock_left;
    (void)hipStreamSynchronize(st);
    std::vector<unsigned long long> h((size_t)nwg * 4);
    (void)hipMemcpy(h.data(), d->dbg_e, (size_t)nwg * 32, hipMemcpyDeviceToHost);
    double sum = 0, sumc = 0; int n = 0; double mn = 1e9, mx = 0;
    for (unsigned i = 0; i < nwg; ++i) {
        if (!h[4 * i + 3] || h[4 * i + 3] == h[4 * i + 1]) continue;
        const double cyc = (double)(h[4 * i + 2] - h[4 * i + 0]), rt = (double)(h[4 * i + 3] - h[4 * i + 1]);
        const double ghz = cyc / rt * 0.1;
        sum += ghz; sumc += cyc; ++n; mn = ghz < mn ? ghz : mn; mx = ghz > mx ? ghz : mx;
    }
    if (n) fprintf(stderr, "[ag clock probe] k_edge_enc: %d workgroups, in-kernel clock mean %.3f GHz (min %.3f max %.3f), mean WG lifetime %.0f cycles\n", n, sum / n, mn, mx, sumc / n);
}

unsigned long long* diag_node_begin(void* v, unsigned nwg, hipStream_t st) {
    Diag* d = static_cast<Diag*>(v);
    if (!d || (!d->node_tail && d->node_left <= 0)) return nullptr;
    if (d->cap_n < nwg) {
        if (d->dbg_n) (void)hipFree(d->dbg_n);
        (void)hipMalloc((void**)&d->dbg_n, (size_t)nwg * 56); d->cap_n = nwg;
        (void)hipMemset(d->dbg_n, 0, (size_t)nwg * 56);
    }
    if (d->node_tail) d->tail_nwg = nwg;
    else (void)hipMemsetAsync(d->dbg_n, 0, (size_t)nwg * 56, st);
    return d->dbg_n;
}
void diag_node_end(void* v, unsigned nwg, int round, hipStream_t st) {
    Diag* d = static_cast<Diag*>(v);
    if (d->node_tail) return;
    --d->node_left;
    (void)hipStreamSynchronize(st);
    std::vector<unsigned long long> h((size_t)nwg * 7);
    (void)hipMemcpy(h.data(), d->dbg_n, (size_t)nwg * 56, hipMemcpyDeviceToHost);
    int nghz = 0;
    const double ghz = node_clock(h, nwg, &nghz);
    unsigned long long t0 = ~0ull, t1 = 0;
    double a = 0, b = 0, c2 = 0; int n = 0;
    for (unsigned i = 0; i < nwg; ++i) {
        if (!h[4 * i + 3]) continue;
        t0 = std::min(t0, h[4 * i]); t1 = std::max(t1, h[4 * i + 3]);
        a += (double)(h[4 * i + 1] - h[4 * i]); b += (double)(h[4 * i + 2] - h[4 * i + 1]); c2 += (double)(h[4 * i + 3] - h[4 * i + 2]); ++n;
    }
    std::vector<std::vector<unsigned>> by_cu(2048);
    for (unsigned i = 0; i < nwg; ++i) if (h[4 * i + 3]) by_cu[h[(size_t)nwg * 4 + i] & 0x7ff].push_back(i);
    double chain[3] = {0, 0, 0}, gath[3] = {0, 0, 0}; int ncu = 0;
    for (auto& vv : by_cu) {
        if (vv.empty()) continue;
        ++ncu;
        std::vector<std::pair<unsigned long long, int>> ev, eg;
        for (unsigned i : vv) {
            ev.push_back({h[4 * i + 1], +1}); ev.push_back({h[4 * i + 3], -1});
            eg.push_back({h[4 * i + 0], +1}); eg.push_back({h[4 * i + 1], -1});
        }
        auto sweep = [&](std::vector<std::pair<unsigned long long, int>>& e, double* acc) {
            std::sort(e.begin(), e.end());
            int lvl = 0; unsigned long long prev = t0;
            for (auto& x : e) { acc[std::min(lvl, 2)] += (double)(x.first - prev); prev = x.first; lvl += x.second; }
            acc[0] += (double)(t1 - prev);
        };
        sweep(ev, chain); sweep(eg, gath);
    }
    const double span = (double)(t1 - t0) * ncu;
    if (n) fprintf(stderr, "[ag node probe] round %d: %d workgroups on %d CUs, span %.1f us; mean per workgroup: gather+loads %.1f us, Wb layer %.1f us, "
                           "W2+W3 layers+stores %.1f us, in-kernel clock %.3f GHz | CU time with 0/1/2 workgroups in chain: %.0f%% %.0f%% %.0f%%; in gather: %.0f%% %.0f%% %.0f%%\n",
                   round, n, ncu, (t1 - t0) * 0.01, a / n * 0.01, b / n * 0.01, c2 / n * 0.01, ghz,
                   100 * chain[0] / span, 100 * chain[1] / span, 100 * chain[2] / span, 100 * gath[0] / span, 100 * gath[1] / span, 100 * gath[2] / span);
}

}
#endif
```

### adaptigraph_amd/csrc/ag_edges.hip

```cpp
#include "ag_common.h"
#include <cstdlib>

namespace ag {

constexpr int EW = 1024;
constexpr int EWAVES = EW / 64;
constexpr int CAP = 256;
constexpr int MAXCH = 64;
constexpr unsigned long long KEY_INF = ~0ull;

struct EdgeDev {
    const float* pos; long pos_bstride;
    const uint8_t* mask; const uint8_t* tool; const float* thr_vec; float thr;
    float thr2_override; int use_thr2;
    const float* thr2_vec;
    int B, N, k, topk_active, cta, edge_cap, slices, rows_per_slice;
    int* ell;
    int ell_full, ell_stride; long ell_bstride;
    int* ns_edge; int* n_ns;
    int* n_oo; int n_cls;
    int* deg; int* slice_tot; int* cta_flag;
    int* recv; int* send; int* row_ptr; int* n_edges; int* overflow; int max_nR; int zero_on_overflow;
    int block_min_rows;
    const int* live;
    int* send_pk; const int* base_send; const int* base_deg; int base_stride, share_No;
    unsigned long long* share_stats;
    const int* share_start; const int* share_cand; int share_b0;
};

__device__ __forceinline__ float dist_exact(float xi, float yi, float zi, float xj, float yj, float zj) {
    const float dx = __fsub_rn(xi, xj), dy = __fsub_rn(yi, yj), dz = __fsub_rn(zi, zj);
    return __fadd_rn(__fadd_rn(__fmul_rn(dx, dx), __fmul_rn(dy, dy)), __fmul_rn(dz, dz));
}
__device__ __forceinline__ int lane_id() { return threadIdx.x & 63; }
__device__ __forceinline__ void wave_lds_sync() {
    __builtin_amdgcn_fence(__ATOMIC_SEQ_CST, "wavefront");
    __builtin_amdgcn_wave_barrier();
}
__device__ __forceinline__ unsigned long long lanes_below(int lane) { return (1ull << lane) - 1ull; }

struct EdgeLds {
    unsigned long long* keys;
    int* scan;
    unsigned short* tprefix;
    unsigned short* tlist;
    float* x; float* y; float* z;
    float* bb;
    int* misc;
    uint8_t* fl;
};
__host__ __device__ inline size_t edge_lds_bytes(int N) {
    const size_t Np = (size_t)((N + 3) & ~3), Nc = (size_t)((N + 63) & ~63);
    return (size_t)EWAVES * CAP * 8 + EW * 4 + (2 * Np + 8) * 2 + Nc * 12 + 6 * MAXCH * 4 + 64 * 4 + Np + 16;
}
__device__ __forceinline__ EdgeLds carve(unsigned char* base, int N) {
    EdgeLds l;
    const int Np = (N + 3) & ~3, Nc = (N + 63) & ~63;
    l.keys = reinterpret_cast<unsigned long long*>(base);
    l.scan = reinterpret_cast<int*>(base + (size_t)EWAVES * CAP * 8);
    l.x = reinterpret_cast<float*>(l.scan + EW);
    l.y = l.x + Nc;
    l.z = l.y + Nc;
    l.bb = l.z + Nc;
    l.misc = reinterpret_cast<int*>(l.bb + 6 * MAXCH);
    l.tprefix = reinterpret_cast<unsigned short*>(l.misc + 64);
    l.tlist = l.tprefix + Np + 4;
    l.fl = reinterpret_cast<uint8_t*>(l.tlist + Np + 4);
    return l;
}

__device__ __forceinline__ float wave_min(float v) {
#pragma unroll
    for (int o = 32; o > 0; o >>= 1) v = fminf(v, __shfl_xor(v, o));
    return v;
}
__device__ __forceinline__ float wave_max(float v) {
#pragma unroll
    for (int o = 32; o > 0; o >>= 1) v = fmaxf(v, __shfl_xor(v, o));
    return v;
}

__device__ void load_candidate(const EdgeDev& a, const EdgeLds& l, int b, bool want_pos) {
    const float* p = a.pos + (long)b * a.pos_bstride;
    if (threadIdx.x < 64) l.misc[threadIdx.x] = 0;
#pragma unroll 2
    for (int i = threadIdx.x; i < a.N; i += EW) {
        if (want_pos) {
            l.x[i] = p[3 * i + 0];
            l.y[i] = p[3 * i + 1];
            l.z[i] = p[3 * i + 2];
        }
        l.fl[i] = (a.mask[(long)b * a.N + i] ? 1 : 0) | (a.tool[(long)b * a.N + i] ? 2 : 0);
    }
    __syncthreads();
    const int lane = lane_id(), wave = threadIdx.x >> 6;
    const int nch = (a.N + 63) >> 6;
    int ntool = 0;
    for (int c = wave; c < nch; c += EWAVES) {
        const int j = 64 * c + lane;
        const bool inb = j < a.N;
        const int f = inb ? l.fl[j] : 0;
        ntool += __popcll(__ballot(inb && (f & 2)));
        if (want_pos) {
            const bool v = inb && (f & 1);
            const float INF = __builtin_huge_valf();
            const float xj = v ? l.x[j] : 0.f, yj = v ? l.y[j] : 0.f, zj = v ? l.z[j] : 0.f;
            const float mnx = wave_min(v ? xj : INF), mxx = wave_max(v ? xj : -INF);
            const float mny = wave_min(v ? yj : INF), mxy = wave_max(v ? yj : -INF);
            const float mnz = wave_min(v ? zj : INF), mxz = wave_max(v ? zj : -INF);
            if (lane == 0) {
                l.bb[0 * MAXCH + c] = mnx; l.bb[1 * MAXCH + c] = mxx; l.bb[2 * MAXCH + c] = mny;
                l.bb[3 * MAXCH + c] = mxy; l.bb[4 * MAXCH + c] = mnz; l.bb[5 * MAXCH + c] = mxz;
            }
        }
    }
    if (lane == 0 && ntool) atomicAdd(&l.misc[2], ntool);
    if (want_pos) {
        const int Nc = (a.N + 63) & ~63;
        for (int j = threadIdx.x; j < Nc; j += EW)
            if (j >= a.N || !(l.fl[j] & 1)) { l.x[j] = __builtin_huge_valf(); l.y[j] = 0.f; l.z[j] = 0.f; }
    }
    __syncthreads();
}

__device__ __forceinline__ unsigned long long survivors(const EdgeLds& l, int N, float xi, float yi, float zi, float thr) {
    thr = fabsf(thr);
    const int lane = lane_id();
    const int nch = (N + 63) >> 6;
    bool keep = false;
    if (lane < nch) {
        const float mnx = l.bb[0 * MAXCH + lane], mxx = l.bb[1 * MAXCH + lane];
        const float mny = l.bb[2 * MAXCH + lane], mxy = l.bb[3 * MAXCH + lane];
        const float mnz = l.bb[4 * MAXCH + lane], mxz = l.bb[5 * MAXCH + lane];
        const bool out = (__fsub_rn(xi, mxx) >= thr) || (__fsub_rn(mnx, xi) >= thr) ||
                         (__fsub_rn(yi, mxy) >= thr) || (__fsub_rn(mny, yi) >= thr) ||
                         (__fsub_rn(zi, mxz) >= thr) || (__fsub_rn(mnz, zi) >= thr);
        keep = !out;
    }
    return __ballot(keep);
}

__device__ __forceinline__ bool pair_within(const EdgeLds& l, int N, float xi, float yi, float zi, int fi, int j,
                                            float thr2, float& d, int& fj) {
    const bool vj = j < N;
    const int jj = vj ? j : 0;
    fj = l.fl[jj];
    d = dist_exact(xi, yi, zi, l.x[jj], l.y[jj], l.z[jj]);
    if (!(fj & 1) || ((fi & 2) && (fj & 2))) d = 1e10f;
    return vj && (__fsub_rn(d, thr2) < 0.0f);
}

template <int U>
__device__ __forceinline__ unsigned long long select_kth_slots(unsigned long long* keys, int nb, int k, bool compact) {
    const int lane = lane_id();
    unsigned long long mine[U];
    int rank[U];
#pragma unroll
    for (int u = 0; u < U; ++u) {
        const int e = lane + 64 * u;
        mine[u] = e < nb ? keys[e] : KEY_INF;
        rank[u] = 0;
    }
#pragma unroll 4
    for (int t = 0; t < nb; ++t) {
        const unsigned long long other = keys[t];
#pragma unroll
        for (int u = 0; u < U; ++u) rank[u] += other < mine[u] ? 1 : 0;
    }
    wave_lds_sync();
    unsigned long long kth = 0;
#pragma unroll
    for (int u = 0; u < U; ++u) {
        const int e = lane + 64 * u;
// ... 323 lines not shown
            d += ntool;
        }
        a.deg[(long)b * a.N + i] = d;
        my += d;
    }
#pragma unroll
    for (int o = 32; o > 0; o >>= 1) my += __shfl_xor(my, o);
    if (lane == 0 && my) atomicAdd(&l.misc[1], my);
    __syncthreads();
    if (threadIdx.x == 0) {
        a.slice_tot[b * a.slices + sl] = l.misc[1];
        if (sl == 0) a.cta_flag[b] = flag;
    }
}

__global__ __launch_bounds__(EW) void k_edge_emit(EdgeDev a) {
    extern __shared__ __attribute__((aligned(16))) unsigned char smem[];
    const int b = blockIdx.x / a.slices, sl = blockIdx.x % a.slices;
    if (a.live && b >= *a.live) {
        if (sl == 0 && threadIdx.x == 0) a.n_edges[b] = 0;
        return;
    }
    const EdgeLds l = carve(smem, a.N);
    load_candidate(a, l, b, !a.topk_active);
    const int lane = lane_id(), wave = threadIdx.x >> 6;
    const int r0 = sl * a.rows_per_slice;
    const int r1 = min(a.N, r0 + a.rows_per_slice);
    const int nrows = max(0, r1 - r0);
    const int flag = a.cta_flag[b];
    const int ntool = l.misc[2];
    const bool tools_on = a.cta && flag && ntool > 0;
    int base = 0, total = 0;
    {
        int pb = 0, pt = 0;
        for (int s = threadIdx.x; s < a.slices; s += EW) {
            const int v = a.slice_tot[b * a.slices + s];
            pb += s < sl ? v : 0;
            pt += v;
        }
#pragma unroll
        for (int o = 32; o > 0; o >>= 1) { pb += __shfl_xor(pb, o); pt += __shfl_xor(pt, o); }
        if (lane == 0) { l.scan[2 * wave] = pb; l.scan[2 * wave + 1] = pt; }
        __syncthreads();
#pragma unroll
        for (int w = 0; w < EWAVES; ++w) { base += l.scan[2 * w]; total += l.scan[2 * w + 1]; }
        __syncthreads();
    }
    const int per = (nrows + EW - 1) / EW;
    const int t0 = min(nrows, (int)threadIdx.x * per), t1 = min(nrows, t0 + per);
    int mysum = 0;
    for (int t = t0; t < t1; ++t) mysum += a.deg[(long)b * a.N + r0 + t];
    l.scan[threadIdx.x] = mysum;
    __syncthreads();
    for (int off = 1; off < EW; off <<= 1) {
        int v = 0;
        if ((int)threadIdx.x >= off) v = l.scan[threadIdx.x - off];
        __syncthreads();
        l.scan[threadIdx.x] += v;
        __syncthreads();
    }
    int run = base + l.scan[threadIdx.x] - mysum;
    const bool fits = total <= a.edge_cap;
    const bool hide = !fits && a.zero_on_overflow;
    for (int t = t0; t < t1; ++t) {
        a.row_ptr[(long)b * (a.N + 1) + r0 + t] = hide ? 0 : run;
        run += a.deg[(long)b * a.N + r0 + t];
    }
    if (sl == a.slices - 1 && threadIdx.x == 0) {
        a.row_ptr[(long)b * (a.N + 1) + a.N] = hide ? 0 : total;
        a.n_edges[b] = hide ? 0 : total;
        if (a.overflow && total > a.max_nR) atomicMax(a.overflow, total);
    }
    if (tools_on) {
        __syncthreads();
        const int perN = (a.N + EW - 1) / EW;
        const int j0 = min(a.N, (int)threadIdx.x * perN), j1 = min(a.N, j0 + perN);
        int c = 0;
        for (int j = j0; j < j1; ++j) c += (l.fl[j] & 2) ? 1 : 0;
        l.scan[threadIdx.x] = c;
        __syncthreads();
        for (int off = 1; off < EW; off <<= 1) {
            int v = 0;
            if ((int)threadIdx.x >= off) v = l.scan[threadIdx.x - off];
            __syncthreads();
            l.scan[threadIdx.x] += v;
            __syncthreads();
        }
        int r = l.scan[threadIdx.x] - c;
        for (int j = j0; j < j1; ++j) {
            l.tprefix[j] = (unsigned short)r;
            if (l.fl[j] & 2) { l.tlist[r] = (unsigned short)j; ++r; }
        }
    }
    __syncthreads();
    if (!fits) return;
    int* recv = a.recv + (long)b * a.edge_cap;
    int* send = a.send + (long)b * a.edge_cap;
    if (a.topk_active) {
        for (int i = r0 + wave; i < r1; i += EWAVES) {
            const int off = a.row_ptr[(long)b * (a.N + 1) + i];
            const int d = a.deg[(long)b * a.N + i];
            const bool row_tools = tools_on && (l.fl[i] & 1) && !(a.cta == 2 && (l.fl[i] & 2));
            const int nt = row_tools ? ntool : 0;
            const int nk = d - nt;
            const int* ell = a.ell + (long)b * a.ell_bstride + (long)i * a.ell_stride;
            for (int t = lane; t < nk; t += 64) {
                const int j = ell[t];
                const int p = off + t + (row_tools ? l.tprefix[j] : 0);
                recv[p] = i; send[p] = j;
            }
            for (int m = lane; m < nt; m += 64) {
                const int j = l.tlist[m];
                int before = 0;
                for (int t = 0; t < nk; ++t) before += ell[t] < j ? 1 : 0;
                const int p = off + m + before;
                recv[p] = i; send[p] = j;
            }
        }
    } else {
        const float thr = thr_of(a, b);
        const float thr2 = thr2_of(a, b, thr);
        for (int i = r0 + wave; i < r1; i += EWAVES) {
            const float xi = l.x[i], yi = l.y[i], zi = l.z[i];
            const int fi = l.fl[i];
            int off = a.row_ptr[(long)b * (a.N + 1) + i];
            unsigned long long todo = (a.cta && flag) ? ~0ull : survivors(l, a.N, xi, yi, zi, thr);
            const int nch = (a.N + 63) >> 6;
            if (nch < 64) todo &= (1ull << nch) - 1ull;
            while (todo) {
                const int c = __ffsll((long long)todo) - 1;
                todo &= todo - 1;
                const bool m = member_radius(a, l, i, 64 * c + lane, xi, yi, zi, fi, thr2, flag);
                const unsigned long long bm = __ballot(m);
                if (m) {
                    const int p = off + __popcll(bm & lanes_below(lane));
                    recv[p] = i; send[p] = 64 * c + lane;
                }
                off += __popcll(bm);
            }
        }
    }
}

constexpr int ELL_BITMAP_MAX_WORDS64 = 16384;
constexpr int ELL_CLASSES = 25;
__device__ __forceinline__ int edge_class(const float* __restrict__ p, int i, int j) {
    const float dx = __fsub_rn(p[3 * i + 0], p[3 * j + 0]), dy = __fsub_rn(p[3 * i + 1], p[3 * j + 1]), dz = __fsub_rn(p[3 * i + 2], p[3 * j + 2]);
    int ax = 0;
    float m = fabsf(dx);
    if (fabsf(dy) > m) { ax = 1; m = fabsf(dy); }
    if (fabsf(dz) > m) ax = 2;
    return ((dx < 0.0f ? 1 : 0) | (dy < 0.0f ? 2 : 0) | (dz < 0.0f ? 4 : 0)) * 3 + ax;
}
template <bool CLS>
__global__ __launch_bounds__(EW) void k_ell_index(EdgeDev a) {
    extern __shared__ __attribute__((aligned(16))) unsigned char smem[];
    unsigned long long* bits = reinterpret_cast<unsigned long long*>(smem);
    __shared__ int wave_tot[EWAVES];
    __shared__ int n_shared;
    const int b = blockIdx.x, tid = threadIdx.x, lane = tid & 63, wave = tid >> 6;
    if (a.live && b >= *a.live) {
        if (tid == 0) { a.n_ns[b] = 0; a.n_edges[b] = 0; if (a.n_oo) a.n_oo[b] = 0; }
        return;
    }
    if (tid == 0) n_shared = 0;
    int total = 0;
    {
        int part = 0;
        for (int s = tid; s < a.slices; s += EW) part += a.slice_tot[b * a.slices + s];
#pragma unroll
        for (int o = 32; o > 0; o >>= 1) part += __shfl_xor(part, o);
        if (lane == 0) wave_tot[wave] = part;
        __syncthreads();
#pragma unroll
        for (int w = 0; w < EWAVES; ++w) total += wave_tot[w];
        __syncthreads();
    }
    const bool hide = total > a.max_nR && a.zero_on_overflow;
    int* deg = a.deg + (long)b * a.N;
    const int* ell = a.ell + (long)b * a.ell_bstride;
    int* recv = a.recv + (long)b * a.edge_cap;
    int* ns = a.ns_edge + (long)b * a.edge_cap;
    int* pk = a.send_pk ? a.send_pk + (long)b * a.edge_cap : nullptr;
    const bool eligible = !a.share_start || a.share_start[a.share_cand ? a.share_cand[b] : a.share_b0 + b] == 0;
    const int stride = a.ell_stride;
    const int nslots = a.N * stride;
    const int nw = (nslots + 63) >> 6;
    const int K = CLS ? a.n_cls : 1;
    const float* cpos = a.pos + (long)b * a.pos_bstride;
    const uint8_t* ctool = a.tool + (long)b * a.N;
    int shared = 0;
    constexpr int UN = 8;
    for (int eb = wave * 64; eb < nw * 64; eb += UN * EW) {
      int iu[UN], du[UN], ju[UN];
#pragma unroll
      for (int u = 0; u < UN; ++u) {
        const int e = eb + u * EW + lane;
        const bool in = e < nslots;
        iu[u] = in ? e / stride : 0;
        du[u] = (in && !hide) ? deg[iu[u]] : 0;
        ju[u] = in ? ell[e] : 0;
      }
#pragma unroll
      for (int u = 0; u < UN; ++u) {
        const int e0 = eb + u * EW;
        if (e0 >= nw * 64) break;
        const int e = e0 + lane;
        const bool in = e < nslots;
        const int i = iu[u], d = du[u], j = ju[u];
        const int t = e - i * stride;
        const bool valid = in && t < d;
        bool own = valid && j != i;
        if (pk && valid) {
            int v = j;
            if (own && eligible && i < a.share_No && j < a.share_No) {
                const int bd = a.base_deg[i];
                const int* brow = a.base_send + (long)i * a.base_stride;
                for (int u = 0; u < bd; ++u)
                    if (brow[u] == j) { v = j | ((u + 1) << 12); own = false; ++shared; break; }
            }
            pk[e] = v;
        }
        if (valid) recv[e] = i;
        if (CLS) {
            int cls = 0;
            if (own) cls = (ctool[i] | ctool[j]) ? K - 1 : (K == 2 ? 0 : edge_class(cpos, i, j));
            unsigned long long keep = 0;
            for (int k = 0; k < K; ++k) {
                const unsigned long long bal = __ballot(own && cls == k);
                if (lane == k) keep = bal;
            }
            if (lane < K) bits[lane * nw + (e0 >> 6)] = keep;
        } else {
        const unsigned long long bal = __ballot(own);
        if (lane == 0) bits[e0 >> 6] = bal;
        }
      }
    }
    if (hide) for (int i = tid; i < a.N; i += EW) deg[i] = 0;
    __syncthreads();
    const int nwt = K * nw;
    const int per = (nwt + EW - 1) / EW;
    const int w0 = min(nwt, tid * per), w1 = min(nwt, w0 + per);
    int mine = 0;
    for (int w = w0; w < w1; ++w) mine += __popcll(bits[w]);
    int incl = mine;
#pragma unroll
    for (int o = 1; o < 64; o <<= 1) {
        const int v = __shfl_up(incl, o);
        if (lane >= o) incl += v;
    }
    if (lane == 63) wave_tot[wave] = incl;
    __syncthreads();
    int before = 0, all = 0;
#pragma unroll
    for (int w = 0; w < EWAVES; ++w) { const int v = wave_tot[w]; before += w < wave ? v : 0; all += v; }
    int pos = before + incl - mine;
    if (CLS) {
        const int wt = (K - 1) * nw;
        for (int w = w0; w < w1; ++w) {
            if (w == wt) a.n_oo[b] = pos;
            const int ws = w % nw;
            unsigned long long m = bits[w];
            while (m) {
                ns[pos++] = (ws << 6) + __ffsll((long long)m) - 1;
                m &= m - 1;
            }
        }
    } else {
    for (int w = w0; w < w1; ++w) {
        unsigned long long m = bits[w];
        while (m) {
            ns[pos++] = (w << 6) + __ffsll((long long)m) - 1;
            m &= m - 1;
        }
    }
    }
    if (pk && a.share_stats) {
#pragma unroll
        for (int o = 32; o > 0; o >>= 1) shared += __shfl_xor(shared, o);
        if (lane == 0 && shared) atomicAdd(&n_shared, shared);
        __syncthreads();
    }
    if (tid == EW - 1) {
        a.n_ns[b] = all;
        if (!CLS && a.n_oo) a.n_oo[b] = 0;
        a.n_edges[b] = hide ? 0 : total;
        if (a.overflow && total > a.max_nR) atomicMax(a.overflow, total);
        if (pk && a.share_stats) {
            atomicAdd(a.share_stats + 0, (unsigned long long)n_shared);
            atomicAdd(a.share_stats + 1, (unsigned long long)all);
        }
    }
}

hipError_t launch_edge_build(const EdgeArgs& h, hipStream_t st, void (*mark)(void*, int, int), void* mark_ctx) {
    EdgeDev a;
    a.pos = h.pos; a.pos_bstride = h.pos_bstride; a.mask = h.mask; a.tool = h.tool; a.thr_vec = h.thr_vec; a.thr = h.thr;
    a.thr2_override = h.thr2_override; a.use_thr2 = h.use_thr2; a.thr2_vec = h.thr2_vec;
    a.B = h.B; a.N = h.N; a.k = min(h.N, h.topk); a.topk_active = a.k < h.N; a.cta = h.cta; a.edge_cap = h.edge_cap;
    a.slices = h.slices; a.rows_per_slice = (h.N + h.slices - 1) / h.slices;
    a.ell = h.ell; a.deg = h.deg; a.slice_tot = h.slice_tot; a.cta_flag = h.cta_flag;
    a.ell_full = h.ell_full && a.topk_active;
    a.ell_stride = a.ell_full ? h.ell_stride : a.k;
    a.ell_bstride = a.ell_full ? h.ell_bstride : (long)h.N * a.k;
    a.ns_edge = h.ns_edge; a.n_ns = h.n_ns; a.n_oo = h.n_oo; a.n_cls = 1;
    a.recv = h.recv; a.send = h.send; a.row_ptr = h.row_ptr; a.n_edges = h.n_edges; a.overflow = h.overflow;
    a.max_nR = h.max_nR; a.zero_on_overflow = h.zero_on_overflow; a.live = h.live;
    a.send_pk = a.ell_full ? h.send_pk : nullptr; a.base_send = h.base_send; a.base_deg = h.base_deg; a.base_stride = h.base_stride;
    a.share_No = h.share_No; a.share_stats = h.share_stats;
    a.share_start = h.share_start; a.share_cand = h.share_cand; a.share_b0 = h.share_b0;
    a.block_min_rows = h.block_min_rows >= 0 ? h.block_min_rows : BLOCK_MIN_ROWS;
    const size_t lds = edge_lds_bytes(h.N);
    static unsigned long long attr_devices = 0;
    int dev_id = 0;
    if (hipGetDevice(&dev_id) != hipSuccess) dev_id = 0;
    if (dev_id >= 64 || !(attr_devices >> dev_id & 1ull)) {
        hipError_t e = hipFuncSetAttribute(reinterpret_cast<const void*>(k_edge_count),
                                           hipFuncAttributeMaxDynamicSharedMemorySize, 160 * 1024 - 256);
        if (e != hipSuccess) return e;
        e = hipFuncSetAttribute(reinterpret_cast<const void*>(k_edge_emit), hipFuncAttributeMaxDynamicSharedMemorySize,
                                160 * 1024 - 256);
        if (e != hipSuccess) return e;
        e = hipFuncSetAttribute(reinterpret_cast<const void*>(k_ell_index<false>), hipFuncAttributeMaxDynamicSharedMemorySize,
                                160 * 1024 - 256);
        if (e != hipSuccess) return e;
        e = hipFuncSetAttribute(reinterpret_cast<const void*>(k_ell_index<true>), hipFuncAttributeMaxDynamicSharedMemorySize,
                                160 * 1024 - 256);
        if (e != hipSuccess) return e;
        if (dev_id < 64) attr_devices |= 1ull << dev_id;
    }
    if (mark) mark(mark_ctx, FAM_EDGE_COUNT, 0);
    hipLaunchKernelGGL(k_edge_count, dim3(h.B * h.slices), dim3(EW), lds, st, a);
    if (mark) mark(mark_ctx, FAM_EDGE_COUNT, 1);
    if (mark) mark(mark_ctx, FAM_EDGE_EMIT, 0);
    if (a.ell_full) {
        const long nw = ((long)h.N * a.ell_stride + 63) >> 6;
        if (nw > ELL_BITMAP_MAX_WORDS64) return hipErrorInvalidValue;
        const long budget = h.lds_words > 0 && h.lds_words < ELL_BITMAP_MAX_WORDS64 ? h.lds_words : ELL_BITMAP_MAX_WORDS64;
        a.n_cls = !a.n_oo ? 1 : ELL_CLASSES * nw <= budget ? ELL_CLASSES : 2 * nw <= budget ? 2 : 1;
        if (a.n_cls > 1) hipLaunchKernelGGL(k_ell_index<true>, dim3(h.B), dim3(EW), (size_t)a.n_cls * nw * 8, st, a);
        else hipLaunchKernelGGL(k_ell_index<false>, dim3(h.B), dim3(EW), (size_t)nw * 8, st, a);
    }
    else hipLaunchKernelGGL(k_edge_emit, dim3(h.B * h.slices), dim3(EW), lds, st, a);
    if (mark) mark(mark_ctx, FAM_EDGE_EMIT, 1);
    return hipGetLastError();
}

__global__ __launch_bounds__(EW) void k_edge_nonself(const int* __restrict__ send_all, const int* __restrict__ row_ptr_all,
                                                      int N, int edge_cap, int* __restrict__ ns_all, int* __restrict__ n_ns,
                                                      const int* __restrict__ live) {
    __shared__ int scan[EW];
    const int b = blockIdx.x, tid = threadIdx.x;
    if (live && b >= *live) { if (tid == 0) n_ns[b] = 0; return; }
    const int* send = send_all + (long)b * edge_cap;
    const int* rp = row_ptr_all + (long)b * (N + 1);
    int* ns = ns_all + (long)b * edge_cap;
    const int per = (N + EW - 1) / EW;
    const int i0 = min(N, tid * per), i1 = min(N, i0 + per);
    int mine = 0;
    for (int i = i0; i < i1; ++i) {
        const int e0 = rp[i], e1 = rp[i + 1];
        for (int e = e0; e < e1; ++e) mine += send[e] == i ? 1 : 0;
    }
    scan[tid] = mine;
    __syncthreads();
    for (int off = 1; off < EW; off <<= 1) {
        int v = 0;
        if (tid >= off) v = scan[tid - off];
        __syncthreads();
        scan[tid] += v;
        __syncthreads();
    }
    int S = scan[tid] - mine;
    for (int i = i0; i < i1; ++i) {
        const int e0 = rp[i], e1 = rp[i + 1];
        for (int e = e0; e < e1; ++e) {
            if (send[e] == i) ++S;
            else ns[e - S] = e;
        }
    }
    if (tid == EW - 1) n_ns[b] = rp[N] - scan[EW - 1];
}
hipError_t launch_edge_nonself(const int* recv, const int* send, const int* row_ptr, int B, int N, int edge_cap,
                               int* ns_edge, int* n_ns, const int* live, hipStream_t st) {
    (void)recv;
    hipLaunchKernelGGL(k_edge_nonself, dim3(B), dim3(EW), 0, st, send, row_ptr, N, edge_cap, ns_edge, n_ns, live);
    return hipGetLastError();
}

size_t edge_build_max_particles() { return MAXCH * 64; }
int edge_ell_stride(int N, int topk) { return topk < N ? topk : 0; }

}
```

### adaptigraph_amd/csrc/ag_host.h

```cpp
#pragma once
#include "../../include/adaptigraph_amd.h"
#include "ag_common.h"

#include <algorithm>
#include <cmath>
#include <cstddef>
#include <cstdio>
#include <cstdlib>
#include <cstring>
#include <string>
#include <vector>

namespace ag {
size_t edge_build_max_particles();
int edge_ell_stride(int N, int topk);
size_t lat_weights_floats();
hipError_t launch_edge_enc_lat(const float* wl, const GraphBufs& g, hipStream_t st);
hipError_t launch_node_enc_lat(const float* wl, const GraphBufs& g, long row0, long nrows, hipStream_t st);
hipError_t launch_node_prop_lat(const float* wl, const GraphBufs& g, int round, bool last, float clamp, float* pred_pos,
                                float* pred_motion, hipStream_t st);
#ifdef AG_DIAG
void* diag_create();
void diag_destroy(void* diag);
int diag_fail_at_chunk(void* diag);
int diag_timing_skip(void* diag);
#endif

struct Slab {
    char* base = nullptr;
    size_t cap = 0, used = 0;
    template <typename T> T* take(size_t n) {
        used = (used + 255) & ~size_t(255);
        T* p = base ? reinterpret_cast<T*>(base + used) : nullptr;
        used += n * sizeof(T);
        return p;
    }
};
struct ProfEvent { int fam; hipEvent_t e0, e1; };

struct BaseKey { int N_o, M, topk, cta, max_nR, n_his, precision, pstep, grip_on; float thr, grip, phys, clamp; const float* phys_vec;
                 unsigned long long weights_version; };

struct CallSlot {
    hipStream_t stream = nullptr; bool bound = false; unsigned long long tick = 0;
    Slab slab;
    int* d_repeat = nullptr; size_t repeat_cap = 0;
    std::vector<int> h_repeat;
    char* d_plan = nullptr; size_t plan_cap = 0;
    int* h_rep_pin = nullptr; size_t rep_pin_cap = 0;
    int* h_plan_max = nullptr; size_t plan_max_cap = 0;
    int* h_census = nullptr;
    hipEvent_t ev_plan = nullptr;
    hipEvent_t ev_census = nullptr; bool census_pending = false;
    BaseKey census_key{}; int census_B = 0, census_H = 0, census_R = 0;
    hipEvent_t ev_done = nullptr; bool have_done = false;
    float* d_work = nullptr; size_t work_cap = 0;
    int* d_words = nullptr;
    unsigned long long* d_share_stats = nullptr;
    static constexpr int kMaxStreams = 4;
    hipStream_t aux_stream[kMaxStreams] = {nullptr, nullptr, nullptr, nullptr};
    hipEvent_t ev_fork = nullptr, ev_join[kMaxStreams] = {nullptr, nullptr, nullptr, nullptr};
};
}

struct ag_ctx {
    int device = 0;
    ag_dims dims{};
    std::string err;
    float* d_w = nullptr;
    float* d_wb3 = nullptr;
    float* d_wlat = nullptr;
    int precision = 0;
    bool have_w = false;
    bool w_finite = false;
    int chunk = 0;
    ag::Options opt;
    void* diag = nullptr;
    static constexpr int kMaxSlots = 8;
    static constexpr int kMaxStreams = ag::CallSlot::kMaxStreams;
    ag::CallSlot slots[kMaxSlots];
    unsigned long long slot_tick = 0;
    int last_slot = 0;
    long long n_allocs = 0;
    long long fwd_executed = 0, fwd_needed = 0;
    int* d_plan_sums = nullptr; int plan_sums_n = 0;
    float* d_base_cache = nullptr; size_t base_cache_cap = 0; int base_cache_R = -1, base_cache_capR = 0;
    ag::BaseKey base_key{};
    struct Decision { bool decline = false; ag::BaseKey key{}; int B = 0, H = 0; } decision;
    unsigned long long weights_version = 0;
    long long steps_enqueued = 0, steps_bound = 0;
    const int* d_share_nns = nullptr;
    float* d_cself = nullptr;
    char* d_self_mini = nullptr;
    int n_streams = 2;
    unsigned prof_mask = 0;
    std::vector<ag::ProfEvent> prof_live;
    std::vector<hipEvent_t> prof_pool;
    double prof_ms[ag::FAM_COUNT] = {0};
    long long prof_n[ag::FAM_COUNT] = {0};
    hipStream_t prof_stream = nullptr;
};

namespace ag {

int fail(ag_ctx* c, int code, const char* fmt, ...);
#define HIPCHK(c, expr)                                                                                   \
    do {                                                                                                  \
        hipError_t _e = (expr);                                                                           \
        if (_e != hipSuccess) return fail(c, AG_ERR_HIP, "%s failed: %s", #expr, hipGetErrorString(_e)); \
    } while (0)

inline hipError_t dev_alloc(ag_ctx* c, void** p, size_t bytes) { ++c->n_allocs; return hipMalloc(p, bytes); }
inline hipError_t dev_free(ag_ctx* c, void* p) { ++c->n_allocs; return hipFree(p); }
inline hipError_t pin_alloc(ag_ctx* c, void** p, size_t bytes) { ++c->n_allocs; return hipHostMalloc(p, bytes, hipHostMallocDefault); }
inline hipError_t pin_free(ag_ctx* c, void* p) { ++c->n_allocs; return hipHostFree(p); }
inline hipError_t event_new(ag_ctx* c, hipEvent_t* e) { ++c->n_allocs; return hipEventCreateWithFlags(e, hipEventDisableTiming); }
inline hipError_t stream_new(ag_ctx* c, hipStream_t* s) { ++c->n_allocs; return hipStreamCreateWithFlags(s, hipStreamNonBlocking); }
template <typename T>
int grow(ag_ctx* c, bool pinned, T*& buf, size_t& cap, size_t need, size_t want) {
    if (cap >= need) return AG_OK;
    if (buf) HIPCHK(c, pinned ? pin_free(c, buf) : dev_free(c, buf));
    buf = nullptr; cap = 0;
    void** q = reinterpret_cast<void**>(&buf);
    HIPCHK(c, pinned ? pin_alloc(c, q, want * sizeof(T)) : dev_alloc(c, q, want * sizeof(T)));
    cap = want;
    return AG_OK;
}

int slot_acquire(ag_ctx* c, hipStream_t st, bool capturing, CallSlot** out);
void slot_release(CallSlot* s, hipStream_t st, bool capturing);
bool other_slot_busy(ag_ctx* c, const CallSlot* me);
struct SlotGuard {
    hipStream_t st = nullptr; CallSlot* sl = nullptr; bool capturing = false;
    SlotGuard() = default;
    SlotGuard(const SlotGuard&) = delete; SlotGuard& operator=(const SlotGuard&) = delete;
    ~SlotGuard() { slot_release(sl, st, capturing); }
};
int begin_call(ag_ctx* c, void* stream, SlotGuard& call, bool watch_capture = false);

void prof_mark(void* vc, int fam, int phase);
struct Scoped {
    ag_ctx* c; int fam;
    Scoped(ag_ctx* c_, int f) : c(c_), fam(f) { prof_mark(c, fam, 0); }
    ~Scoped() { prof_mark(c, fam, 1); }
};

struct Work {
    GraphBufs g{};
    RollBufs r{};
    int* ell; int* deg; int* slice_tot; int* cta_flag;
    int* recv; int* send; int* row_ptr; int* n_edges;
    int* ns_edge; int* n_ns; int* n_oo;
    int* send_pk;
    int* rowlist; int* n_rows;
};

inline size_t round_up(size_t v, size_t m) { return (v + m - 1) / m * m; }
inline int ensure_slab(ag_ctx* c, CallSlot& sl, size_t bytes) {
    sl.slab.used = 0;
    return grow(c, false, sl.slab.base, sl.slab.cap, bytes, round_up(bytes + (bytes >> 3), 1 << 20));
}
template <typename Carve>
int carve_slab(ag_ctx* c, CallSlot& sl, Carve&& carve) {
    Slab measure;
    carve(measure);
    int rc = ensure_slab(c, sl, measure.used);
    if (rc) return rc;
    carve(sl.slab);
    if (sl.slab.used > sl.slab.cap) return fail(c, AG_ERR_INVALID, "internal: workspace carve overflow");
    return AG_OK;
}
void carve_work(const ag_ctx* c, Slab& s, Work& w, int Bc, int N, int n_inst, int edge_cap, int c_cap, int slices, bool own_edges,
                bool roll, bool own_group, int N_o, int ell_stride);

int pick_slices(const ag_ctx* c, int B, int N);
int clamp_chunk_for_offsets(int Bc, int N, int c_cap);
int auto_chunk(const ag_ctx* c, int B, int N);
bool lat_node_for(const ag_ctx* c, const GraphBufs& g);
hipError_t node_enc_for(const ag_ctx* c, const GraphBufs& g, long row0, long nrows, hipStream_t st);
int run_edge_chain(ag_ctx* c, const GraphBufs& g, hipStream_t st);
int run_model(ag_ctx* c, const GraphBufs& g, float* pred_pos, float* pred_motion, hipStream_t st);
int enqueue_self_rows(ag_ctx* c, hipStream_t st);
int check_topk(ag_ctx* c, int N, int topk);

struct ForwardFrame {
    int B, N, n_inst, edge_cap, n_p, n_guard, c_cap, Bc;
    Work w{}; int* n_eff = nullptr;
    ForwardFrame(const ag_ctx* c, int B, int N, int n_inst, int edge_cap, int n_p, int n_guard);
    void carve(const ag_ctx* c, Slab& s);
};
int enqueue_forward(ag_ctx* c, const ForwardFrame& f, const float* d_state, const float* d_attrs, const float* d_action,
                    const float* d_phys, const float* d_group, const int32_t* d_recv, const int32_t* d_send,
                    const int32_t* d_row_ptr, const int* n_eff, int B, float* d_pred_pos, float* d_pred_motion, hipStream_t st);

}
```

### adaptigraph_amd/csrc/ag_mlp.hip

```cpp
#include "ag_common.h"
#include <cstdint>

namespace ag {
#ifdef AG_DIAG
unsigned long long* diag_edge_begin(void* diag, unsigned nwg, hipStream_t st);
void diag_edge_end(void* diag, unsigned nwg, hipStream_t st);
unsigned long long* diag_node_begin(void* diag, unsigned nwg, hipStream_t st);
void diag_node_end(void* diag, unsigned nwg, int round, hipStream_t st);
#endif

typedef float f32x16 __attribute__((ext_vector_type(16)));
typedef float f32x32 __attribute__((ext_vector_type(32)));
typedef float f32x4 __attribute__((ext_vector_type(4)));

constexpr int WG = 256;
constexpr int WG_ROWS = 128;
constexpr int QCH = 5;
constexpr int BUF_FLOATS = QCH * CHUNK_FLOATS_MB5;
constexpr int Q_FLOATS = BUF_FLOATS;
constexpr int Q3_FLOATS = (KCH - 3 * QCH) * CHUNK_FLOATS_MB5;
constexpr int STG_TILE_PITCH = 36;
constexpr int STG_ROW_PITCH = 164;
constexpr int STG_ROWS = 8;
constexpr int STG_FLOATS = STG_ROWS * STG_ROW_PITCH;
// ... 105 lines not shown
        for (int r = 0; r < 16; ++r) a.t[t][r] = 0.0f;
}
__device__ __forceinline__ void materialize(Act& a) {
#pragma unroll
    for (int t = 0; t < 5; ++t) asm volatile("" : "+v"(a.t[t]));
}
__device__ __forceinline__ void relu_one(Act& a, int lane) {
#pragma unroll
    for (int t = 0; t < 5; ++t)
#pragma unroll
        for (int r = 0; r < 16; ++r) a.t[t][r] = __builtin_fmaxf(a.t[t][r], 0.0f);
    a.t[4][10] = lane >= 32 ? 1.0f : a.t[4][10];
    materialize(a);
}

template <bool HS = false>
__device__ __forceinline__ Live live_of(const Act& a, int on, int half = 0) {
    Live lv = {{~0u, ~0u, ~0u}, {~0u, ~0u, ~0u}, {~0u, ~0u, ~0u}};
    if (on) {
#pragma unroll
        for (int i = 0; i < 3; ++i) lv.m[i] = lv.lo[i] = lv.hi[i] = 0u;
#pragma unroll
        for (int s = 0; s < 4 * KCH; ++s) {
            const int t = s < 64 ? s / 16 : 4;
            const int r = s < 64 ? s % 16 : s - 64;
            const unsigned long long bal = __builtin_amdgcn_ballot_w64(a.t[t][r] != 0.0f);
            const bool any = bal != 0;
            lv.m[s >> 5] |= any ? 1u << (s & 31) : 0u;
            if (HS) {
                unsigned bh = (unsigned)(bal >> 32);
                asm("" : "+s"(bh));
                lv.lo[s >> 5] |= (unsigned)bal != 0u ? 1u << (s & 31) : 0u;
                lv.hi[s >> 5] |= bh != 0u ? 1u << (s & 31) : 0u;
            }
        }
        if (HS && !half) {
#pragma unroll
            for (int i = 0; i < 3; ++i) lv.lo[i] = lv.hi[i] = lv.m[i];
        }
    }
    return lv;
}

__device__ __forceinline__ void load_rows(Act& a, const float* __restrict__ base, long row, int lane) {
    const float* p = base + row * NFP + 4 * (lane >> 5);
#pragma unroll
    for (int t = 0; t < 5; ++t)
#pragma unroll
        for (int q = 0; q < 4; ++q) {
            const f32x4 v = *reinterpret_cast<const f32x4*>(p + 32 * t + 8 * q);
            a.t[t][4 * q + 0] = v[0]; a.t[t][4 * q + 1] = v[1]; a.t[t][4 * q + 2] = v[2]; a.t[t][4 * q + 3] = v[3];
        }
}
__device__ __forceinline__ long pin_after(Act& a) {
    int z = 0;
    float v = a.t[0][0];
    asm volatile("" : "+v"(z), "+v"(v));
    a.t[0][0] = v;
    return z;
}
template <int T0, int T1>
__device__ __forceinline__ void add_rows_part(Act& a, const float* __restrict__ base, long row, int lane) {
    const float* p = base + row * NFP + 4 * (lane >> 5);
#pragma unroll
    for (int t = T0; t < T1; ++t)
#pragma unroll
        for (int q = 0; q < 4; ++q) {
            const f32x4 v = *reinterpret_cast<const f32x4*>(p + 32 * t + 8 * q);
            a.t[t][4 * q + 0] += v[0]; a.t[t][4 * q + 1] += v[1]; a.t[t][4 * q + 2] += v[2]; a.t[t][4 * q + 3] += v[3];
        }
}
__device__ __forceinline__ void store_rows(const Act& a, float* __restrict__ base, long row, int lane, bool valid) {
    if (!valid) return;
    float* p = base + row * NFP + 4 * (lane >> 5);
#pragma unroll
    for (int t = 0; t < 5; ++t)
#pragma unroll
        for (int q = 0; q < 4; ++q) {
            f32x4 v;
            v[0] = a.t[t][4 * q + 0]; v[1] = a.t[t][4 * q + 1]; v[2] = a.t[t][4 * q + 2]; v[3] = a.t[t][4 * q + 3];
            *reinterpret_cast<f32x4*>(p + 32 * t + 8 * q) = v;
        }
    __builtin_amdgcn_sched_barrier(0);
}

__device__ __forceinline__ void store_rows_t(const Act& a, float* __restrict__ base, int myrow, bool valid, float* stg, int lane) {
    const int j = lane & 31, h = lane >> 5, sr = lane >> 3, sc = lane & 7;
    int srow[4];
#pragma unroll
    for (int i = 0; i < 4; ++i) {
        const int r = __shfl(valid ? myrow : -1, sr + 8 * i, 64);
        srow[i] = r;
    }
    float* wp = stg + j * STG_TILE_PITCH + 4 * h;
    const float* rp = stg + sr * STG_TILE_PITCH + 4 * sc;
#pragma unroll
    for (int t = 0; t < 5; ++t) {
#pragma unroll
        for (int q = 0; q < 4; ++q) {
            f32x4 v;
            v[0] = a.t[t][4 * q + 0]; v[1] = a.t[t][4 * q + 1]; v[2] = a.t[t][4 * q + 2]; v[3] = a.t[t][4 * q + 3];
            *reinterpret_cast<f32x4*>(wp + 8 * q) = v;
        }
#pragma unroll
        for (int i = 0; i < 4; ++i) {
            const f32x4 v = *reinterpret_cast<const f32x4*>(rp + 8 * i * STG_TILE_PITCH);
            if (srow[i] >= 0) *reinterpret_cast<f32x4*>(base + (long)srow[i] * NFP + 32 * t + 4 * sc) = v;
        }
    }
    __builtin_amdgcn_sched_barrier(0);
}

template <int NEXT, bool ZERO = true, bool PRE = false, bool SKIP = false, bool HS = false>
__device__ __forceinline__ void layer160(float* lds, const float* __restrict__ w, const float* __restrict__ next,
                                         const Act& in, Act& out, int tid, int lane, const Live& lv = Live()) {
    float* b0 = lds;
    float* b1 = lds + BUF_FLOATS;
    if (ZERO) zero(out);
    f32x32 pr[2];
    if (HS) { pr[0] = cat32(out.t[0], out.t[1]); pr[1] = cat32(out.t[2], out.t[3]); }
    if (!PRE) dma_copy<Q_FLOATS>(b1, w + Q_FLOATS, tid);
    mma_act<0, QCH, 5, SKIP, HS>(b0, in, out.t, lane, lv, pr);
    __syncthreads();
    dma_copy<Q_FLOATS>(b0, w + 2 * Q_FLOATS, tid);
    mma_act<QCH, 2 * QCH, 5, SKIP, HS>(b1, in, out.t, lane, lv, pr);
    __syncthreads();
    dma_copy<Q3_FLOATS>(b1, w + 3 * Q_FLOATS, tid);
    mma_act<2 * QCH, 3 * QCH, 5, SKIP, HS>(b0, in, out.t, lane, lv, pr);
    __syncthreads();
    if (NEXT > 0) dma_copy<(NEXT > 0 ? NEXT : 256)>(b0, next, tid);
    mma_act<3 * QCH, KCH, 5, SKIP, HS>(b1, in, out.t, lane, lv, pr);
    if (HS) { out.t[0] = lo16(pr[0]); out.t[1] = hi16(pr[0]); out.t[2] = lo16(pr[1]); out.t[3] = hi16(pr[1]); }
    if (NEXT > 0) __syncthreads();
}

template <int NFLOATS>
__device__ __forceinline__ void stage_now(float* dst, const float* __restrict__ src, int tid) {
    dma_copy<NFLOATS>(dst, src, tid);
    __syncthreads();
}

struct GDev {
    const float* w;
    const float* node_in; const float* feat12; const float* group;
    float* eff; float* P; float* U; float* V; float* C;
    const int* recv; const int* send; const int* row_ptr; const int* n_edges;
    int B, N, n_p, n_inst, edge_cap, c_cap;
    float clamp; float* pred_pos; float* pred_motion;
    int cls_on, N_o, M, first_round; const uint8_t* vmask;
    const float* c_eff; const float* c_P;
    long row0, nrows;
    const int* ns_edge; const int* n_ns;
    const int* n_oo;
    const float* wb3;
    const float* Uin; const float* Vin; const int* deg; int ell_stride; int dedupe; unsigned self_row; const int* n_guard;
    int stagger_ticks; unsigned first_wave;
    int reverse;
    unsigned n_tiles;
    const int* rowlist; const int* n_rows;
    const float* C_share; unsigned share_kb;
    int f_pitch, cur_off;
    int zero_skip;
    int half_step;
#ifdef AG_DIAG
    unsigned long long* dbg;
#endif
};

using WL = WeightLayout;

__device__ __forceinline__ long dense_row(const GDev& g, long slot, long nslots) {
    const long s = slot < nslots ? slot : nslots - 1;
    return g.rowlist ? (long)g.rowlist[s] : s;
}

struct EdgeBuf { f32x4 c[5], v[5]; };
struct PassRow {
    int i, deg, b, e0;
};
template <bool SHARE>
__device__ __forceinline__ void gather_addr(const GDev& g, const PassRow& r, bool cls, int k, int sjp, const float* __restrict__ C,
                                            const float* __restrict__ V, int lane, const float*& cp, const float*& vp) {
    const unsigned c4 = 4u * (lane & 7);
    const bool on = k < r.deg;
    const int sj = SHARE ? (sjp & 0xfff) : sjp;
    const unsigned selfrow = g.self_row + (r.i >= g.N_o ? 1u : 0u);
    const unsigned crow = (!on || (g.dedupe && sj == r.i)) ? selfrow : (unsigned)r.b * (unsigned)g.c_cap + (unsigned)(r.e0 + k);
    const unsigned tool0 = (unsigned)g.N_o + (unsigned)r.b * g.M;
    const unsigned vrow = cls ? (sj >= g.N_o ? tool0 + (unsigned)sj : (unsigned)sj) : (unsigned)r.b * (unsigned)g.N + (unsigned)sj;
    cp = C + crow * (unsigned)NFP + c4;
    if (SHARE) {
        const unsigned sp = (unsigned)sjp >> 12;
        const float* sh = g.C_share + ((unsigned)r.i * g.share_kb + (sp - 1u)) * (unsigned)NFP + c4;
        cp = (on && sp != 0u) ? sh : cp;
    }
    vp = V + vrow * (unsigned)NFP + c4;
}
template <bool SHARE>
__device__ __forceinline__ void gather_issue(const GDev& g, const PassRow& r, bool cls, int k, int sjp, EdgeBuf& buf,
                                             const float* __restrict__ C, const float* __restrict__ V, int lane) {
    const float *cp, *vp;
    gather_addr<SHARE>(g, r, cls, k, sjp, C, V, lane, cp, vp);
#pragma unroll
    for (int t = 0; t < 5; ++t) {
        buf.c[t] = *reinterpret_cast<const f32x4*>(cp + 32 * t);
        buf.v[t] = *reinterpret_cast<const f32x4*>(vp + 32 * t);
    }
}
__device__ __forceinline__ void gather_consume(const EdgeBuf& buf, const f32x4* u, f32x4* acc, bool on) {
#pragma unroll
    for (int t = 0; t < 5; ++t)
#pragma unroll
        for (int e = 0; e < 4; ++e) {
            const float m = fmaxf((buf.c[t][e] + u[t][e]) + buf.v[t][e], 0.0f);
            acc[t][e] += on ? m : 0.0f;
        }
}
__device__ __forceinline__ int wave_max(int v) {
#pragma unroll
    for (int o = 1; o < 64; o <<= 1) v = max(v, __shfl_xor(v, o, 64));
    return __builtin_amdgcn_readfirstlane(v);
}

template <bool SHARE>
__device__ __forceinline__ void gather_agg(const GDev& g, float* stg, long wave_row0, long nrows, Act& x, int lane) {
    const int rr = lane >> 3, c = lane & 7, j = lane & 31, h = lane >> 5;
    const bool cls = g.cls_on && g.first_round;
    const float* __restrict__ C = g.C;
    const float* __restrict__ U = g.Uin;
    const float* __restrict__ V = g.Vin;
    int pb[4], pe0[4], pdeg[4], pidx0[4], pkmax[4];
    long prow[4]; bool prv[4];
#pragma unroll
    for (int p = 0; p < 4; ++p) {
        const long slot = wave_row0 + 8 * p + rr;
        prv[p] = slot < nrows;
        prow[p] = dense_row(g, slot, nrows);
        pb[p] = (int)(prow[p] / g.N);
    }
    const bool ell = g.ell_stride != 0;
    int d0[4], d1[4];
#pragma unroll
    for (int p = 0; p < 4; ++p) {
        const int i = (int)(prow[p] - (long)pb[p] * g.N);
        const int* dp = ell ? g.deg + prow[p] : g.row_ptr + (long)pb[p] * (g.N + 1) + i;
        d0[p] = dp[0];
        d1[p] = ell ? 0 : dp[1];
        if (ell) pe0[p] = i * g.ell_stride;
    }
    if (ell) {
#pragma unroll
        for (int p = 0; p < 4; ++p) {
            const long o = (long)pb[p] * g.edge_cap + min(pe0[p] + c, g.edge_cap - 1);
            pidx0[p] = g.send[o];
        }
    }
#pragma unroll
    for (int p = 0; p < 4; ++p) {
        int deg = ell ? d0[p] : d1[p] - d0[p];
        if (!ell) pe0[p] = d0[p];
        const int guard = g.n_guard ? g.n_guard[pb[p]] : 1;
        if (!prv[p] || guard == 0) deg = 0;
        if (guard == 0) pe0[p] = 0;
        pdeg[p] = deg;
    }
    if (!ell) {
#pragma unroll
        for (int p = 0; p < 4; ++p) {
            const int e = min(max(pe0[p], 0) + c, g.edge_cap - 1);
            pidx0[p] = g.send[(long)pb[p] * g.edge_cap + e];
        }
    }
    auto row_of = [&](int p) {
        PassRow r;
        r.b = pb[p]; r.e0 = pe0[p]; r.deg = pdeg[p];
        r.i = (int)(prow[p] - (long)pb[p] * g.N);
        return r;
    };
    auto senders_of = [&](const PassRow& r) { return g.send + (long)r.b * g.edge_cap + r.e0; };
#pragma unroll
    for (int p = 0; p < 4; ++p) {
        if (c >= pdeg[p]) pidx0[p] = (int)(prow[p] - (long)pb[p] * g.N);
        pkmax[p] = wave_max(pdeg[p]);
    }
    const int N_o = g.N_o;
    auto issue_u = [&](const PassRow& r, f32x4* u) {
        const unsigned urow = cls ? (r.i >= N_o ? (unsigned)N_o + (unsigned)r.b * g.M + r.i : (unsigned)r.i)
                                  : (unsigned)r.b * (unsigned)g.N + (unsigned)r.i;
        const float* up = U + urow * (unsigned)NFP + 4u * c;
#pragma unroll
        for (int t = 0; t < 5; ++t) u[t] = *reinterpret_cast<const f32x4*>(up + 32 * t);
    };
    constexpr int KFAST = 32;
    f32x4 u[5];
    EdgeBuf A, B;
    PassRow r = row_of(0);
    int idx0 = pidx0[0];
    issue_u(r, u);
    if (pkmax[0] > 0) gather_issue<SHARE>(g, r, cls, 0, __shfl(idx0, lane & 56, 64), A, C, V, lane);
#pragma unroll
    for (int p = 0; p < 4; ++p) {
        const int kmax = pkmax[p], kfast = min(kmax, KFAST);
        const int* snd = senders_of(r);
        const int lastk = max(r.deg - 1, 0);
        const int room = g.edge_cap - 1 - r.e0;
        int idx1 = snd[min(min(8 + c, lastk), room)], idx2 = snd[min(min(16 + c, lastk), room)], idx3 = snd[min(min(24 + c, lastk), room)];
        if (8 + c >= r.deg) idx1 = r.i;
        if (16 + c >= r.deg) idx2 = r.i;
        if (24 + c >= r.deg) idx3 = r.i;
        auto sender = [&](int k) {
            const int blk = k >> 3;
            const int v = blk == 0 ? idx0 : blk == 1 ? idx1 : blk == 2 ? idx2 : idx3;
            return __shfl(v, (lane & 56) + (k & 7), 64);
        };
        f32x4 acc[5];
#pragma unroll
        for (int t = 0; t < 5; ++t) acc[t] = f32x4{0.f, 0.f, 0.f, 0.f};
        int k = 0;
        for (; k + 2 < kfast; k += 2) {
            gather_issue<SHARE>(g, r, cls, k + 1, sender(k + 1), B, C, V, lane);
            gather_consume(A, u, acc, k < r.deg);
            gather_issue<SHARE>(g, r, cls, k + 2, sender(k + 2), A, C, V, lane);
            gather_consume(B, u, acc, k + 1 < r.deg);
        }
        const int left = kfast - k;
        if (left == 2) gather_issue<SHARE>(g, r, cls, k + 1, sender(k + 1), B, C, V, lane);
        if (left >= 1) gather_consume(A, u, acc, k < r.deg);
        if (left == 2) gather_consume(B, u, acc, k + 1 < r.deg);
        for (k = KFAST; k < kmax; ++k) {
            const int sj = k < r.deg ? snd[k] : r.i;
            gather_issue<SHARE>(g, r, cls, k, sj, A, C, V, lane);
            gather_consume(A, u, acc, k < r.deg);
        }
        if (p + 1 < 4) {
            r = row_of(p + 1);
            idx0 = pidx0[p + 1];
            issue_u(r, u);
            if (pkmax[p + 1] > 0) gather_issue<SHARE>(g, r, cls, 0, __shfl(idx0, lane & 56, 64), A, C, V, lane);
        }
        float* wp = stg + rr * STG_ROW_PITCH + 4 * c;
#pragma unroll
        for (int t = 0; t < 5; ++t) *reinterpret_cast<f32x4*>(wp + 32 * t) = acc[t];
        if ((j >> 3) == p) {
            const float* rp = stg + (j & 7) * STG_ROW_PITCH + 4 * h;
#pragma unroll
            for (int t = 0; t < 5; ++t)
#pragma unroll
                for (int q = 0; q < 4; ++q) {
                    const f32x4 v = *reinterpret_cast<const f32x4*>(rp + 32 * t + 8 * q);
                    x.t[t][4 * q + 0] = v[0]; x.t[t][4 * q + 1] = v[1]; x.t[t][4 * q + 2] = v[2]; x.t[t][4 * q + 3] = v[3];
                }
        }
    }
}

__device__ __forceinline__ long cls_row(const GDev& g, int b, int i) {
    if (i >= g.N_o) return 2L * g.N_o + (long)b * g.M + (i - g.N_o);
    return g.vmask[(long)b * g.N + i] ? i : g.N_o + i;
}

__device__ __forceinline__ void stagger_second_workgroup(const GDev& g) {
    if (g.stagger_ticks > 0 && blockIdx.x < g.first_wave) {
        const unsigned lds_base = __builtin_amdgcn_s_getreg(6 | (0 << 6) | (7 << 11));
        if (lds_base != 0) {
            const unsigned long long t0 = __builtin_amdgcn_s_memrealtime();
            while (__builtin_amdgcn_s_memrealtime() - t0 < (unsigned long long)g.stagger_ticks) __builtin_amdgcn_s_sleep(64);
        }
    }
}

template <int NH>
__global__ __launch_bounds__(WG, 2) void k_edge_enc(GDev g) {
    constexpr int FP = NH == 5 ? F15_PITCH : F12, NQ = FP / 4, RD = 5 + 3 * NH;
    __shared__ __attribute__((aligned(16))) float lds[CHAIN_LDS_FLOATS];
    const int tid = threadIdx.x, lane = tid & 63, wave = tid >> 6;
    float* stg = lds + 2 * BUF_FLOATS + wave * STG_FLOATS;
    const unsigned n_tiles = g.n_tiles ? g.n_tiles : gridDim.x;
    for (unsigned blk = blockIdx.x; blk < n_tiles; blk += gridDim.x) {
    int zi = 0;
    asm volatile("" : "+s"(zi));
    const float* const wts = g.w + zi;
    const int b = (int)(blk % (unsigned)g.B);
    const int e0 = (int)(blk / (unsigned)g.B) * WG_ROWS;
    const int ne = g.n_ns ? g.n_ns[b] : g.n_edges[b];
    if (e0 >= ne) continue;
    int skip = 0;
    if (ZS_EDGE) skip = g.zero_skip && (ZS_EDGE_ALL || (g.n_oo && e0 < g.n_oo[b])) ? 1 : 0;
#ifdef AG_DIAG
    if (g.dbg && tid == 0) {
        g.dbg[blk * 4 + 0] = __builtin_amdgcn_s_memtime();
        g.dbg[blk * 4 + 1] = __builtin_amdgcn_s_memrealtime();
    }
#endif

    stage_now<EDGE_L1_CHUNKS * CHUNK_FLOATS_MB5>(lds + BUF_FLOATS, wts + WL::E_L1, tid);
    dma_copy<Q_FLOATS>(lds, wts + WL::E_L2, tid);

    const int t = e0 + wave * 32 + (lane & 31);
    const bool valid = t < ne;
    const int el = g.ns_edge ? g.ns_edge[(long)b * g.edge_cap + (valid ? t : 0)] : t;
    const int elc = valid ? el : (g.ns_edge ? el : 0);
    const int r = g.recv[(long)b * g.edge_cap + elc], s = g.send[(long)b * g.edge_cap + elc];
    const long pr = (long)b * g.N + r, ps = (long)b * g.N + s;
    float f[8 * EDGE_L1_CHUNKS];
    {
        const float* nr = g.node_in + pr * NODE_IN; const float* nsnd = g.node_in + ps * NODE_IN;
        f[0] = nr[0]; f[1] = nr[1]; f[2] = nsnd[0]; f[3] = nsnd[1];
        float gd = 0.0f;
        for (int k = 0; k < g.n_inst; ++k) gd += fabsf(g.group[pr * g.n_inst + k] - g.group[ps * g.n_inst + k]);
        f[4] = gd;
        const f32x4* fr = reinterpret_cast<const f32x4*>(g.feat12 + pr * FP);
        const f32x4* fs = reinterpret_cast<const f32x4*>(g.feat12 + ps * FP);
#pragma unroll
        for (int q = 0; q < NQ; ++q) {
            const f32x4 a = fr[q], c = fs[q];
            f[5 + 4 * q + 0] = a[0] - c[0]; f[5 + 4 * q + 1] = a[1] - c[1];
            f[5 + 4 * q + 2] = a[2] - c[2]; f[5 + 4 * q + 3] = a[3] - c[3];
        }
        f[RD] = 1.0f;
#pragma unroll
        for (int k = RD + 1; k < 8 * EDGE_L1_CHUNKS; ++k) f[k] = 0.0f;
    }
    Act x, y;
    zero(y);
    mma_feat<EDGE_L1_CHUNKS, (RD + 2) / 2>(lds + BUF_FLOATS, f, y.t, lane);
    __syncthreads();
    relu_one(y, lane);
    layer160<Q_FLOATS, true, false, ZS_EDGE, HS_EDGE>(lds, wts + WL::E_L2, wts + WL::E_L3, y, x, tid, lane, live_of<HS_EDGE>(y, skip, g.half_step));
    relu_one(x, lane);
    layer160<Q_FLOATS, true, false, ZS_EDGE, HS_EDGE>(lds, wts + WL::E_L3, wts + WL::E_W1, x, y, tid, lane, live_of<HS_EDGE>(x, skip, g.half_step));
    relu_one(y, lane);
    layer160<0, true, false, ZS_EDGE, HS_EDGE>(lds, wts + WL::E_W1, nullptr, y, x, tid, lane, live_of<HS_EDGE>(y, skip, g.half_step));
    store_rows_t(x, g.C, (int)((long)b * g.c_cap + el), valid, stg, lane);
#ifdef AG_DIAG
    if (g.dbg && tid == 0) {
        g.dbg[blk * 4 + 2] = __builtin_amdgcn_s_memtime();
        g.dbg[blk * 4 + 3] = __builtin_amdgcn_s_memrealtime();
    }
#endif
    __syncthreads();
    }
}

__global__ __launch_bounds__(WG, 2) void k_node_enc(GDev g) {
    __shared__ __attribute__((aligned(16))) float lds[CHAIN_LDS_FLOATS];
    const int tid = threadIdx.x, lane = tid & 63, wave = tid >> 6;
    float* stg = lds + 2 * BUF_FLOATS + wave * STG_FLOATS;
    const long rend = g.row0 + g.nrows;
    const long row = g.row0 + (long)blockIdx.x * WG_ROWS + wave * 32 + (lane & 31);
    const bool valid = row < rend;
    const long rowc = valid ? row : rend - 1;

    stage_now<NODE_L1_CHUNKS * CHUNK_FLOATS_MB5>(lds + BUF_FLOATS, g.w + WL::N_L1, tid);
    dma_copy<Q_FLOATS>(lds, g.w + WL::N_L2, tid);
    float f[8];
    {
        const f32x4* p = reinterpret_cast<const f32x4*>(g.node_in + rowc * NODE_IN);
        const f32x4 a = p[0], c = p[1];
        f[0] = a[0]; f[1] = a[1]; f[2] = a[2]; f[3] = a[3]; f[4] = c[0]; f[5] = c[1]; f[6] = c[2]; f[7] = c[3];
    }
    Act x, y;
    zero(y);
    mma_feat<NODE_L1_CHUNKS>(lds + BUF_FLOATS, f, y.t, lane);
    __syncthreads();
    relu_one(y, lane);
    layer160<Q_FLOATS, true, false, ZS_ENC>(lds, g.w + WL::N_L2, g.w + WL::N_L3, y, x, tid, lane, live_of(y, g.zero_skip));
    relu_one(x, lane);
    layer160<Q_FLOATS, true, false, ZS_ENC>(lds, g.w + WL::N_L3, g.w + WL::N_WA, x, y, tid, lane, live_of(x, g.zero_skip));
    relu_one(y, lane);
    const Live lv = live_of<HS_NODE>(y, g.zero_skip);
    store_rows_t(y, g.eff, (int)row, valid, stg, lane);
    layer160<Q_FLOATS, true, false, ZS_ENC>(lds, g.w + WL::N_WA, g.w + WL::N_W2, y, x, tid, lane, lv);
    store_rows_t(x, g.P, (int)row, valid, stg, lane);
    layer160<Q_FLOATS, true, false, ZS_ENC, HS_NODE>(lds, g.w + WL::N_W2, g.w + WL::N_W3, y, x, tid, lane, lv);
    store_rows_t(x, g.U, (int)row, valid, stg, lane);
    layer160<0, true, false, ZS_ENC, HS_NODE>(lds, g.w + WL::N_W3, nullptr, y, x, tid, lane, lv);
    store_rows_t(x, g.V, (int)row, valid, stg, lane);
}

template <bool LAST, bool SHARE>
__global__ __launch_bounds__(WG, 2) void k_node_prop(GDev g) {
    __shared__ __attribute__((aligned(16))) float lds[CHAIN_LDS_FLOATS];
    const int tid = threadIdx.x, lane = tid & 63, wave = tid >> 6;
    float* stg = lds + 2 * BUF_FLOATS + wave * STG_FLOATS;
    const long nrows = g.n_rows ? (long)*g.n_rows : (long)g.B * g.N;
    const unsigned bid = g.reverse ? gridDim.x - 1u - blockIdx.x : blockIdx.x;
    if ((long)bid * WG_ROWS >= nrows) return;
    const long slot = (long)bid * WG_ROWS + wave * 32 + (lane & 31);
    const bool valid = slot < nrows;
    const long rowc = dense_row(g, slot, nrows);
    const long row = rowc;

    stagger_second_workgroup(g);
#ifdef AG_DIAG
    if (g.dbg && tid == 0) {
        g.dbg[blockIdx.x * 4 + 0] = __builtin_amdgcn_s_memrealtime();
        const unsigned hw = __builtin_amdgcn_s_getreg(4 | (0 << 6) | (31 << 11));
        const unsigned xcc = __builtin_amdgcn_s_getreg(20 | (0 << 6) | (3 << 11));
        g.dbg[(unsigned long)gridDim.x * 4 + blockIdx.x] = (xcc << 8) | (((hw >> 13) & 7) << 4) | ((hw >> 8) & 15);
        g.dbg[(unsigned long)gridDim.x * 5 + 2 * blockIdx.x] = __builtin_amdgcn_s_memtime();
    }
#endif
    dma_copy<Q_FLOATS>(lds, g.w + WL::P_WB, tid);
    Act x, y;
    gather_agg<SHARE>(g, stg, (long)bid * WG_ROWS + wave * 32, nrows, x, lane);
    __builtin_amdgcn_sched_barrier(0);
#ifdef AG_DIAG
    if (g.dbg && tid == 0) g.dbg[blockIdx.x * 4 + 1] = __builtin_amdgcn_s_memrealtime();
#endif
    const int pb = (int)(rowc / g.N), pi = (int)(rowc - (long)pb * g.N);
    const long crow = g.cls_on ? cls_row(g, pb, pi) : rowc;
    const bool ceff = g.cls_on && g.first_round;
    load_rows(y, g.cls_on ? g.c_P : g.P, crow, lane);
    add_rows_part<0, 2>(y, ceff ? g.c_eff : g.eff, ceff ? crow : rowc, lane);
    materialize(y);
    add_rows_part<2, 5>(y, ceff ? g.c_eff : g.eff, (ceff ? crow : rowc) + pin_after(y), lane);
    __syncthreads();
    layer160<Q_FLOATS, false, false, ZS_NODE, HS_NODE>(lds, g.w + WL::P_WB, g.w + (LAST ? WL::P_P0 : WL::N_W2), x, y, tid, lane,
                                                       live_of<HS_NODE>(x, g.zero_skip, g.half_step));
    relu_one(y, lane);
    const Live lv = live_of<HS_NODE>(y, g.zero_skip, g.half_step);
#ifdef AG_DIAG
    if (g.dbg && tid == 0) g.dbg[blockIdx.x * 4 + 2] = __builtin_amdgcn_s_memrealtime();
#endif
    if (!LAST) {
        dma_copy<Q_FLOATS>(lds + BUF_FLOATS, g.w + WL::N_W2 + Q_FLOATS, tid);
        store_rows_t(y, g.eff, (int)row, valid, stg, lane);
        layer160<Q_FLOATS, true, true, ZS_NODE, HS_NODE>(lds, g.w + WL::N_W2, g.w + WL::N_W3, y, x, tid, lane, lv);
        dma_copy<Q_FLOATS>(lds + BUF_FLOATS, g.w + WL::N_W3 + Q_FLOATS, tid);
        store_rows_t(x, g.U, (int)row, valid, stg, lane);
        layer160<0, true, true, ZS_NODE, HS_NODE>(lds, g.w + WL::N_W3, nullptr, y, x, tid, lane, lv);
        store_rows_t(x, g.V, (int)row, valid, stg, lane);
#ifdef AG_DIAG
        if (g.dbg && tid == 0) {
            g.dbg[blockIdx.x * 4 + 3] = __builtin_amdgcn_s_memrealtime();
            g.dbg[(unsigned long)gridDim.x * 5 + 2 * blockIdx.x + 1] = __builtin_amdgcn_s_memtime();
        }
#endif
    } else {
        layer160<Q_FLOATS, true, false, ZS_NODE, HS_NODE>(lds, g.w + WL::P_P0, g.w + WL::P_P1, y, x, tid, lane, lv);
        relu_one(x, lane);
        layer160<OUT3_FLOATS, true, false, ZS_NODE, HS_NODE>(lds, g.w + WL::P_P1, g.w + WL::P_P2, x, y, tid, lane, live_of<HS_NODE>(x, g.zero_skip, g.half_step));
        relu_one(y, lane);
        f32x16 m[1];
#pragma unroll
        for (int r = 0; r < 16; ++r) m[0][r] = 0.0f;
        mma_act<0, KCH, 1, false>(lds, y, m, lane, Live());
        const int b = pb, i = pi;
        if (valid && lane < 32 && i < g.n_p) {
            const float* cur = g.feat12 + rowc * g.f_pitch + g.cur_off;
            const long o = ((long)b * g.n_p + i) * 3;
#pragma unroll
            for (int c = 0; c < 3; ++c) {
                const float mo = m[0][c];
                g.pred_motion[o + c] = mo;
                g.pred_pos[o + c] = cur[c] + fminf(fmaxf(mo, -g.clamp), g.clamp);
            }
        }
    }
}


typedef __bf16 bf16x8 __attribute__((ext_vector_type(8)));
constexpr int PH_FLOATS = 2 * 5 * 3 * 64 * 4;
struct WLB {
    static constexpr int E_L1 = 0, E_L2 = 1, E_L3 = 6, E_W1 = 11;
    static constexpr int N_L1 = 16, N_L2 = 17, N_L3 = 22, N_WA = 27, N_W2 = 32, N_W3 = 37;
    static constexpr int P_WB = 42, P_P0 = 47, P_P1 = 52, P_P2 = 57, TOTAL = 58;
};

__device__ __forceinline__ void split8(const float* x, bf16x8& h, bf16x8& m, bf16x8& l) {
#pragma unroll
    for (int i = 0; i < 8; ++i) {
        const __bf16 hi = (__bf16)x[i];
        const float r = x[i] - (float)hi;
        const __bf16 mi = (__bf16)r;
        const float q = r - (float)mi;
        h[i] = hi; m[i] = mi; l[i] = (__bf16)q;
    }
}
template <int NK, int MB>
__device__ __forceinline__ void mma_b3(const float* wl, const bf16x8* bh, const bf16x8* bm, const bf16x8* bl,
                                       f32x16* acc, int lane) {
    const bf16x8* w = reinterpret_cast<const bf16x8*>(wl);
    bf16x8 ah = w[0 * 64 + lane], am = w[1 * 64 + lane], al = w[2 * 64 + lane];
#pragma unroll
// ... 123 lines not shown
    const bool valid = t < ne;
    const int el = g.ns_edge ? g.ns_edge[(long)b * g.edge_cap + (valid ? t : 0)] : t;
    const int elc = valid ? el : (g.ns_edge ? el : 0);
    const int r = g.recv[(long)b * g.edge_cap + elc], s = g.send[(long)b * g.edge_cap + elc];
    const long pr = (long)b * g.N + r, ps = (long)b * g.N + s;
    float f[18];
    {
        const float* nr = g.node_in + pr * NODE_IN; const float* nsnd = g.node_in + ps * NODE_IN;
        f[0] = nr[0]; f[1] = nr[1]; f[2] = nsnd[0]; f[3] = nsnd[1];
        float gd = 0.0f;
        for (int k = 0; k < g.n_inst; ++k) gd += fabsf(g.group[pr * g.n_inst + k] - g.group[ps * g.n_inst + k]);
        f[4] = gd;
        const f32x4* fr = reinterpret_cast<const f32x4*>(g.feat12 + pr * F12);
        const f32x4* fs = reinterpret_cast<const f32x4*>(g.feat12 + ps * F12);
#pragma unroll
        for (int q = 0; q < 3; ++q) {
            const f32x4 a = fr[q], c = fs[q];
            f[5 + 4 * q + 0] = a[0] - c[0]; f[5 + 4 * q + 1] = a[1] - c[1];
            f[5 + 4 * q + 2] = a[2] - c[2]; f[5 + 4 * q + 3] = a[3] - c[3];
        }
        f[17] = 1.0f;
    }
    Act x, y;
    zero(y);
    unit<0, 0>(lds, W, tid, [&](const float* wl) { first_b3<2, 18>(wl, f, y.t, lane); });
    relu_one(y, lane);
    zero(x);
    layer_b3<0, 1>(lds, W, y, x, tid, lane);
    relu_one(x, lane);
    zero(y);
    layer_b3<0, 6>(lds, W, x, y, tid, lane);
    relu_one(y, lane);
    zero(x);
    layer_b3<0, 11>(lds, W, y, x, tid, lane);
    store_rows(x, g.C, (long)b * g.c_cap + el, lane, valid);
}

__global__ __launch_bounds__(WGB, WGB_PER_CU) void k_node_enc_b3(GDev g) {
    __shared__ __attribute__((aligned(16))) float lds[NSLOT * UNIT_FLOATS];
    const int tid = threadIdx.x, lane = tid & 63, wave = tid >> 6;
    const long rend = g.row0 + g.nrows;
    const long row = g.row0 + (long)blockIdx.x * WGB_ROWS + wave * 32 + (lane & 31);
    const bool valid = row < rend;
    const long rowc = valid ? row : rend - 1;
    const float* W = g.wb3;
    stream_begin<1>(lds, W, tid);
    float f[8];
    {
        const f32x4* p = reinterpret_cast<const f32x4*>(g.node_in + rowc * NODE_IN);
        const f32x4 a = p[0], c = p[1];
        f[0] = a[0]; f[1] = a[1]; f[2] = a[2]; f[3] = a[3]; f[4] = c[0]; f[5] = c[1]; f[6] = c[2]; f[7] = c[3];
    }
    Act x, y;
    zero(y);
    unit<1, 0>(lds, W, tid, [&](const float* wl) { first_b3<1, 8>(wl, f, y.t, lane); });
    relu_one(y, lane);
    zero(x);
    layer_b3<1, 1>(lds, W, y, x, tid, lane);
    relu_one(x, lane);
    zero(y);
    layer_b3<1, 6>(lds, W, x, y, tid, lane);
    relu_one(y, lane);
    store_rows(y, g.eff, row, lane, valid);
    zero(x);
    layer_b3<1, 11>(lds, W, y, x, tid, lane);
    store_rows(x, g.P, row, lane, valid);
    zero(x);
    layer_b3<1, 16>(lds, W, y, x, tid, lane);
    store_rows(x, g.U, row, lane, valid);
    zero(x);
    layer_b3<1, 21>(lds, W, y, x, tid, lane);
    store_rows(x, g.V, row, lane, valid);
}

template <bool LAST, bool SHARE>
__global__ __launch_bounds__(WGB, WGB_PER_CU) void k_node_prop_b3(GDev g) {
    __shared__ __attribute__((aligned(16))) float lds[NSLOT * UNIT_FLOATS];
    constexpr int KIND = LAST ? 3 : 2;
    const int tid = threadIdx.x, lane = tid & 63, wave = tid >> 6;
    const long nrows = g.n_rows ? (long)*g.n_rows : (long)g.B * g.N;
    if ((long)blockIdx.x * WGB_ROWS >= nrows) return;
    const long slot = (long)blockIdx.x * WGB_ROWS + wave * 32 + (lane & 31);
    const bool valid = slot < nrows;
    const long rowc = dense_row(g, slot, nrows);
    const long row = rowc;
    const float* W = g.wb3;
    Act x, y;
    gather_agg<SHARE>(g, lds + wave * STG_FLOATS, (long)blockIdx.x * WGB_ROWS + wave * 32, nrows, x, lane);
    __syncthreads();
    stream_begin<KIND>(lds, W, tid);
    const int pb = (int)(rowc / g.N), pi = (int)(rowc - (long)pb * g.N);
    const long crow = g.cls_on ? cls_row(g, pb, pi) : rowc;
    const bool ceff = g.cls_on && g.first_round;
    load_rows(y, g.cls_on ? g.c_P : g.P, crow, lane);
    add_rows_part<0, 2>(y, ceff ? g.c_eff : g.eff, ceff ? crow : rowc, lane);
    materialize(y);
    add_rows_part<2, 5>(y, ceff ? g.c_eff : g.eff, (ceff ? crow : rowc) + pin_after(y), lane);
    layer_b3<KIND, 0>(lds, W, x, y, tid, lane);
    relu_one(y, lane);
    if (!LAST) {
        store_rows(y, g.eff, row, lane, valid);
        zero(x);
        layer_b3<KIND, 5>(lds, W, y, x, tid, lane);
        store_rows(x, g.U, row, lane, valid);
        zero(x);
        layer_b3<KIND, 10>(lds, W, y, x, tid, lane);
        store_rows(x, g.V, row, lane, valid);
    } else {
        zero(x);
        layer_b3<KIND, 5>(lds, W, y, x, tid, lane);
        relu_one(x, lane);
        zero(y);
        layer_b3<KIND, 10>(lds, W, x, y, tid, lane);
        relu_one(y, lane);
        f32x16 m[1];
#pragma unroll
        for (int r = 0; r < 16; ++r) m[0][r] = 0.0f;
        unit<KIND, 15>(lds, W, tid, [&](const float* wl) {
#pragma unroll
            for (int t = 0; t < 5; ++t)
#pragma unroll
                for (int u = 0; u < 2; ++u) {
                    float xx[8];
#pragma unroll
                    for (int j = 0; j < 8; ++j) xx[j] = y.t[t][8 * u + j];
                    bf16x8 bh, bm, bl;
                    split8(xx, bh, bm, bl);
                    mma_b3<1, 1>(wl + (2 * t + u) * (3 * 64 * 4), &bh, &bm, &bl, m, lane);
                }
        });
        const int b = pb, i = pi;
        if (valid && lane < 32 && i < g.n_p) {
            const float* curp = g.feat12 + rowc * F12 + 9;
            const long o = ((long)b * g.n_p + i) * 3;
#pragma unroll
            for (int c = 0; c < 3; ++c) {
                const float mo = m[0][c];
                g.pred_motion[o + c] = mo;
                g.pred_pos[o + c] = curp[c] + fminf(fmaxf(mo, -g.clamp), g.clamp);
            }
        }
    }
}

static GDev to_dev(const float* w, const GraphBufs& g) {
    GDev d;
    d.w = w; d.node_in = g.node_in; d.feat12 = g.feat12; d.group = g.group; d.eff = g.eff; d.P = g.P; d.U = g.UV[1][0];
    d.V = g.UV[1][1]; d.C = g.C; d.recv = g.recv; d.send = g.send; d.row_ptr = g.row_ptr;
    d.n_edges = g.n_edges; d.B = g.B; d.N = g.N; d.n_p = g.n_p; d.n_inst = g.n_inst; d.edge_cap = g.edge_cap;
    d.c_cap = g.c_cap; d.clamp = 0; d.pred_pos = nullptr; d.pred_motion = nullptr; d.n_tiles = 0;
    d.cls_on = g.cls_on; d.N_o = g.N_o; d.M = g.M; d.first_round = 0; d.vmask = g.vmask; d.c_eff = g.c_eff; d.c_P = g.c_P;
    d.row0 = 0; d.nrows = (long)g.B * g.N;
    d.ns_edge = g.ns_edge; d.n_ns = g.n_ns; d.n_oo = g.n_oo;
    d.wb3 = g.wb3;
    d.Uin = nullptr; d.Vin = nullptr; d.deg = g.deg; d.ell_stride = g.ell_stride; d.dedupe = g.c_self ? 1 : 0;
    d.self_row = (unsigned)g.self_row; d.n_guard = g.n_guard;
    d.rowlist = g.rowlist; d.n_rows = g.n_rows;
    d.C_share = nullptr; d.share_kb = 0;
    d.f_pitch = feat_pitch(g.n_his); d.cur_off = g.n_his == 5 ? 12 : 9;
    d.zero_skip = g.zero_skip; d.half_step = g.half_step;
    d.stagger_ticks = g.stagger_us * 100; d.first_wave = 512; d.reverse = 0;
#ifdef AG_DIAG
    d.dbg = nullptr;
#endif
    return d;
}
static long node_slots(const GraphBufs& g) { return (long)g.B * g.N + (g.rowlist ? g.N_o : 0); }
static int node_grid(const GraphBufs& g) { return (int)((node_slots(g) + WG_ROWS - 1) / WG_ROWS); }
static int node_grid_b3(const GraphBufs& g) { return (int)((node_slots(g) + WGB_ROWS - 1) / WGB_ROWS); }

hipError_t launch_edge_enc(const float* w, const GraphBufs& g, hipStream_t st) {
    const long rows = (long)g.B * g.c_cap;
    const unsigned nwg = (unsigned)(rows / WG_ROWS);
    GDev d = to_dev(w, g);
    bool probing = false;
#ifdef AG_DIAG
    d.dbg = diag_edge_begin(g.diag, nwg, st);
    probing = d.dbg != nullptr;
#endif
    if (d.wb3) hipLaunchKernelGGL(k_edge_enc_b3, dim3((unsigned)g.B * (unsigned)((g.c_cap + WGB_ROWS - 1) / WGB_ROWS)), dim3(WGB), 0, st, d);
    else if (g.n_his == 5) hipLaunchKernelGGL(k_edge_enc<5>, dim3(nwg), dim3(WG), 0, st, d);
    else {
        unsigned grid = nwg;
        if (g.enc_persist > 0 && !probing && nwg > (unsigned)g.enc_persist) { d.n_tiles = nwg; grid = (unsigned)g.enc_persist; }
        hipLaunchKernelGGL(k_edge_enc<4>, dim3(grid), dim3(WG), 0, st, d);
    }
#ifdef AG_DIAG
    if (probing) diag_edge_end(g.diag, nwg, st);
#endif
    return hipGetLastError();
}
hipError_t launch_node_enc(const float* w, const GraphBufs& g, long row0, long nrows, hipStream_t st) {
    GDev d = to_dev(w, g);
    if (g.cls_on) {
        d.node_in = g.c_node_in; d.eff = g.c_eff; d.P = g.c_P; d.U = g.c_U; d.V = g.c_V;
        d.row0 = row0; d.nrows = nrows;
    }
    if (d.nrows <= 0) return hipSuccess;
    const dim3 grid((unsigned)((d.nrows + WG_ROWS - 1) / WG_ROWS));
    if (d.wb3) hipLaunchKernelGGL(k_node_enc_b3, dim3((unsigned)((d.nrows + WGB_ROWS - 1) / WGB_ROWS)), dim3(WGB), 0, st, d);
    else hipLaunchKernelGGL(k_node_enc, grid, dim3(WG), 0, st, d);
    return hipGetLastError();
}
static void set_round(GDev& d, const GraphBufs& g, int round) {
    const int first = round == 0;
    d.first_round = first;
    const bool cls = g.cls_on && first;
    d.Uin = cls ? g.c_U : g.UV[(round - 1) & 1][0];
    d.Vin = cls ? g.c_V : g.UV[(round - 1) & 1][1];
    d.U = g.UV[round & 1][0]; d.V = g.UV[round & 1][1];
    d.reverse = g.zigzag ? (round & 1) : 0;
    if (g.send_pk) { d.send = g.send_pk; d.C_share = g.C_share; d.share_kb = (unsigned)g.share_kb; }
}
hipError_t launch_node_prop(const float* w, const GraphBufs& g, int round, hipStream_t st) {
    GDev d = to_dev(w, g);
    set_round(d, g, round);
    const unsigned nwg = (unsigned)node_grid(g);
#ifdef AG_DIAG
    if (!d.wb3) d.dbg = diag_node_begin(g.diag, nwg, st);
#endif
    if (d.wb3) {
        if (d.C_share) hipLaunchKernelGGL((k_node_prop_b3<false, true>), dim3(node_grid_b3(g)), dim3(WGB), 0, st, d);
        else hipLaunchKernelGGL((k_node_prop_b3<false, false>), dim3(node_grid_b3(g)), dim3(WGB), 0, st, d);
    } else if (d.C_share) hipLaunchKernelGGL((k_node_prop<false, true>), dim3(nwg), dim3(WG), 0, st, d);
    else hipLaunchKernelGGL((k_node_prop<false, false>), dim3(nwg), dim3(WG), 0, st, d);
#ifdef AG_DIAG
    if (d.dbg) diag_node_end(g.diag, nwg, round, st);
#endif
    return hipGetLastError();
}
hipError_t launch_node_final(const float* w, const GraphBufs& g, int round, float clamp, float* pred_pos,
                             float* pred_motion, hipStream_t st) {
    GDev d = to_dev(w, g);
    set_round(d, g, round);
    d.clamp = clamp; d.pred_pos = pred_pos; d.pred_motion = pred_motion;
    if (d.wb3) {
        if (d.C_share) hipLaunchKernelGGL((k_node_prop_b3<true, true>), dim3(node_grid_b3(g)), dim3(WGB), 0, st, d);
        else hipLaunchKernelGGL((k_node_prop_b3<true, false>), dim3(node_grid_b3(g)), dim3(WGB), 0, st, d);
    } else if (d.C_share) hipLaunchKernelGGL((k_node_prop<true, true>), dim3(node_grid(g)), dim3(WG), 0, st, d);
    else hipLaunchKernelGGL((k_node_prop<true, false>), dim3(node_grid(g)), dim3(WG), 0, st, d);
    return hipGetLastError();
}

}
```

Before: 50640 rollout-steps/s.

## Order edge-encoder work by ELL slot across candidates and tool sector keys

Adds an edge_order=2 mode, now the default, in which the ELL index kernel writes per-candidate ownership and tool bitmaps plus a histogram of tool edges keyed by direction sector and distance ring. Three new kernels (count, scan, fill) then build a global edge list sorted by ELL slot across all candidates, followed by tool edges grouped by key. The edge encoder runs over this packed (candidate, slot) list instead of per-candidate ranges. The aim is to make waves process edges with similar features together, so the zero-skip and half-step paths fire more often and load imbalance drops. The cost is three extra launches, a single-block scan, and extra bitmap and list memory.

```diff
diff --git a/adaptigraph_amd/csrc/ag_api.hip b/adaptigraph_amd/csrc/ag_api.hip
--- a/adaptigraph_amd/csrc/ag_api.hip
+++ b/adaptigraph_amd/csrc/ag_api.hip
@@ -30,7 +30,7 @@
     {"share_prefix", "AG_SHARE_PREFIX", &Options::share_prefix, false, -1, 1},
     {"stream_min_rows", "AG_STREAM_MIN_ROWS", &Options::stream_min_rows, false, 0, 0x7fffffff},
     {"pipeline_fork", "AG_PIPELINE_FORK", &Options::pipeline_fork, false, 0, 1},
-    {"edge_order", "AG_EDGE_ORDER", &Options::edge_order, false, 0, 1},
+    {"edge_order", "AG_EDGE_ORDER", &Options::edge_order, false, 0, 2},
     {"ell_lds_words", "AG_ELL_LDS_WORDS", &Options::ell_lds_words, false, 0, 16384},
 };
 void options_from_env(Options& o) {
@@ -162,6 +162,13 @@
         w.ns_edge = s.take<int>((size_t)Bc * edge_cap);
         w.n_ns = s.take<int>(Bc);
         w.n_oo = s.take<int>(Bc);
+        w.ck_bits = nullptr; w.ck_off = nullptr; w.ck_list = nullptr;
+        if (roll && ell_stride > 0) {
+            const size_t slots = (size_t)N * (ell_stride + N - N_o);
+            w.ck_bits = s.take<unsigned long long>((size_t)Bc * 2 * ((slots + 63) / 64));
+            w.ck_off = s.take<int>(2 + slots + (size_t)CHUNK_TOOL_KEYS * Bc);
+            w.ck_list = s.take<unsigned>((size_t)Bc * edge_cap);
+        }
         w.g.recv = w.recv; w.g.send = w.send; w.g.row_ptr = w.row_ptr; w.g.n_edges = w.n_edges;
     }
     if (roll) {
diff --git a/adaptigraph_amd/csrc/ag_api_rollout.hip b/adaptigraph_amd/csrc/ag_api_rollout.hip
--- a/adaptigraph_amd/csrc/ag_api_rollout.hip
+++ b/adaptigraph_amd/csrc/ag_api_rollout.hip
@@ -281,6 +281,19 @@
     return AG_OK;
 }
 
+void chunk_list_for(const RollCall& r, const Work& w, EdgeArgs& ea, GraphBufs& g) {
+    ag_ctx* c = r.c;
+    ea.ck_list = nullptr; ea.ck_bits = nullptr; ea.ck_off = nullptr; ea.ck_shift = 0;
+    g.ck_list = nullptr; g.ck_n = nullptr; g.ck_shift = 0;
+    if (c->opt.edge_order != 2 || !r.ell_full || !r.dedupe || !w.ck_list || g.wb3 || g.B <= 0 || lat_edge_for(c, g)) return;
+    const long slots = (long)r.N * (r.k + r.p->M);
+    int shift = 1;
+    while ((1L << shift) < slots) ++shift;
+    if (shift >= 32 || ((unsigned long)(g.B - 1) >> (32 - shift)) != 0) return;
+    ea.ck_list = w.ck_list; ea.ck_bits = w.ck_bits; ea.ck_off = w.ck_off; ea.ck_shift = shift;
+    g.ck_list = w.ck_list; g.ck_n = w.ck_off; g.ck_shift = shift;
+}
+
 int workspace_graph(RollCall& r, Work& w, int nb, hipStream_t s, GraphBufs& g) {
     ag_ctx* c = r.c;
     g = w.g;
@@ -360,7 +373,8 @@
     RollArgs ra = roll_args(r, 0, 1);
     ra.H = 1; ra.eef_xz = r.b_eef; ra.eef_delta = r.b_eef + 2 * p->M; ra.repeat = r.b_zero;
     ra.write_obj_cls = 1; ra.all_states = r.b_states; ra.all_y = r.b_y;
-    const EdgeArgs ea = workspace_edge_args(r, w, 1);
+    EdgeArgs ea = workspace_edge_args(r, w, 1);
+    chunk_list_for(r, w, ea, g);
     { Scoped sc(c, FAM_ROLL_INIT); HIPCHK(c, launch_roll_init(ra, w.r, g, st)); }
     { Scoped sc(c, FAM_NODE_ENC); HIPCHK(c, node_enc_for(c, g, 0, 2L * p->N_o + p->M, st)); }
     for (int ai = 1; ai <= r.R_base; ++ai) {
@@ -506,8 +520,12 @@
                     ea.share_stats = sl.d_share_stats; g.C_share = r.C_share; g.share_kb = r.kb;
                     ea.share_start = r.d_start; ea.share_cand = ra.cand; ea.share_b0 = b0;
                 }
+                chunk_list_for(r, w, ea, g);
                 if (!(timing_skip & 1) || ai == 1) {
                     HIPCHK(c, launch_edge_build(ea, cs, prof_mark, c));
+#ifdef AG_DIAG
+                    diag_chunk_dump(c->diag, ea, p->M, cs);
+#endif
                     if (g.ns_edge && !r.ell_full) { Scoped s(c, FAM_EDGE_EMIT); HIPCHK(c, launch_edge_nonself(w.recv, w.send, w.row_ptr, n_live, N, r.edge_cap, w.ns_edge, w.n_ns, ea.live, cs)); }
                 }
                 rc = run_model(c, g, w.r.pred, w.r.motion, cs);
diff --git a/adaptigraph_amd/csrc/ag_common.h b/adaptigraph_amd/csrc/ag_common.h
--- a/adaptigraph_amd/csrc/ag_common.h
+++ b/adaptigraph_amd/csrc/ag_common.h
@@ -87,11 +87,12 @@
     int pipeline_fork = 0;
     int zero_skip = 1;
     int half_step = 1;
-    int edge_order = 1;
+    int edge_order = 2;
     int ell_lds_words = 0;
     int share_first = -1;
 };
 
+constexpr int CHUNK_TOOL_KEYS = 32 * 16;
 struct EdgeArgs {
     const float* pos;
     long pos_bstride;
@@ -115,6 +116,7 @@
     int ell_full; int ell_stride; long ell_bstride;
     int* ns_edge; int* n_ns;
     int* n_oo; int lds_words;
+    unsigned long long* ck_bits; int* ck_off; unsigned* ck_list; int ck_shift;
     int block_min_rows;
     const int* live;
     int* send_pk; const int* base_send; const int* base_deg; int base_stride; int share_No;
@@ -188,6 +190,7 @@
     long self_row;
     const int* ns_edge; const int* n_ns;
     const int* n_oo;
+    const unsigned* ck_list; const int* ck_n; int ck_shift;
     const float* wb3;
     const int* n_guard;
     const int* rowlist; const int* n_rows;
diff --git a/adaptigraph_amd/csrc/ag_diag.hip b/adaptigraph_amd/csrc/ag_diag.hip
--- a/adaptigraph_amd/csrc/ag_diag.hip
+++ b/adaptigraph_amd/csrc/ag_diag.hip
@@ -3,6 +3,7 @@
 #include <algorithm>
 #include <cstdio>
 #include <cstdlib>
+#include <string>
 #include <vector>
 
 namespace ag {
@@ -10,6 +11,7 @@
 struct Diag {
     int clock_left = 0, node_left = 0, fail_at_chunk = -1, timing_skip = 0;
     bool node_tail = false;
+    std::string chunk_dump; int chunk_dump_at = 0, chunk_lists = 0;
     unsigned long long* dbg_e = nullptr; unsigned cap_e = 0;
     unsigned long long* dbg_n = nullptr; unsigned cap_n = 0; unsigned tail_nwg = 0;
 };
@@ -20,10 +22,37 @@
     if (const char* e = getenv("AG_NODE_PROBE")) { const int v = atoi(e); d->node_left = v > 0 ? v : 0; d->node_tail = v < 0; }
     if (const char* e = getenv("AG_TEST_FAIL_AT_CHUNK")) d->fail_at_chunk = atoi(e);
     if (const char* e = getenv("AG_TIMING_SKIP")) d->timing_skip = atoi(e);
+    if (const char* e = getenv("AG_CHUNK_DUMP")) d->chunk_dump = e;
+    if (const char* e = getenv("AG_CHUNK_DUMP_AT")) d->chunk_dump_at = atoi(e);
     return d;
 }
 int diag_fail_at_chunk(void* v) { return v ? static_cast<Diag*>(v)->fail_at_chunk : -1; }
 int diag_timing_skip(void* v) { return v ? static_cast<Diag*>(v)->timing_skip : 0; }
+
+void diag_chunk_dump(void* v, const EdgeArgs& ea, int n_tools, hipStream_t st) {
+    Diag* d = static_cast<Diag*>(v);
+    if (!d || d->chunk_dump.empty() || !ea.ck_list || d->chunk_lists++ != d->chunk_dump_at) return;
+    (void)hipStreamSynchronize(st);
+    int B = ea.B;
+    if (ea.live) { int live = 0; (void)hipMemcpy(&live, ea.live, 4, hipMemcpyDeviceToHost); B = std::min(B, live); }
+    int n[2] = {0, 0};
+    (void)hipMemcpy(n, ea.ck_off, 8, hipMemcpyDeviceToHost);
+    const int head[8] = {B, ea.N, ea.ell_stride, ea.edge_cap, ea.ck_shift, n[0], n[1], n_tools};
+    std::vector<int> list((size_t)n[0]), deg((size_t)B * ea.N), send((size_t)B * ea.edge_cap);
+    std::vector<float> pos((size_t)B * ea.N * 3);
+    if (n[0]) (void)hipMemcpy(list.data(), ea.ck_list, list.size() * 4, hipMemcpyDeviceToHost);
+    if (B) {
+        (void)hipMemcpy(deg.data(), ea.deg, deg.size() * 4, hipMemcpyDeviceToHost);
+        (void)hipMemcpy(send.data(), ea.send, send.size() * 4, hipMemcpyDeviceToHost);
+        (void)hipMemcpy2D(pos.data(), (size_t)ea.N * 12, ea.pos, (size_t)ea.pos_bstride * 4, (size_t)ea.N * 12, B, hipMemcpyDeviceToHost);
+    }
+    if (FILE* f = fopen(d->chunk_dump.c_str(), "wb")) {
+        fwrite(head, 4, 8, f);
+        fwrite(list.data(), 4, list.size(), f); fwrite(deg.data(), 4, deg.size(), f); fwrite(send.data(), 4, send.size(), f);
+        fwrite(pos.data(), 4, pos.size(), f); fwrite(&ea.thr, 4, 1, f);
+        fclose(f);
+    }
+}
 
 static double node_clock(const std::vector<unsigned long long>& h, unsigned nwg, int* n_out) {
     double ghz = 0; int n = 0;
diff --git a/adaptigraph_amd/csrc/ag_edges.hip b/adaptigraph_amd/csrc/ag_edges.hip
--- a/adaptigraph_amd/csrc/ag_edges.hip
+++ b/adaptigraph_amd/csrc/ag_edges.hip
@@ -19,6 +19,7 @@
     int ell_full, ell_stride; long ell_bstride;
     int* ns_edge; int* n_ns;
     int* n_oo; int n_cls;
+    unsigned long long* ck_bits; int* ck_off; unsigned* ck_list; int ck_shift;
     int* deg; int* slice_tot; int* cta_flag;
     int* recv; int* send; int* row_ptr; int* n_edges; int* overflow; int max_nR; int zero_on_overflow;
     int block_min_rows;
@@ -648,18 +649,38 @@
     if (fabsf(dz) > m) ax = 2;
     return ((dx < 0.0f ? 1 : 0) | (dy < 0.0f ? 2 : 0) | (dz < 0.0f ? 4 : 0)) * 3 + ax;
 }
-template <bool CLS>
+__device__ __forceinline__ int chunk_tool_key(const float* __restrict__ p, int i, int j, float thr2) {
+    const float dx = __fsub_rn(p[3 * i + 0], p[3 * j + 0]), dy = __fsub_rn(p[3 * i + 1], p[3 * j + 1]), dz = __fsub_rn(p[3 * i + 2], p[3 * j + 2]);
+    const float ax = fabsf(dx), az = fabsf(dz);
+    const bool swap = az > ax;
+    const float mn = swap ? ax : az, mx = swap ? az : ax;
+    const int fine = (mn >= __fmul_rn(0.19891237f, mx) ? 1 : 0) + (mn >= __fmul_rn(0.41421357f, mx) ? 1 : 0) +
+                     (mn >= __fmul_rn(0.66817864f, mx) ? 1 : 0);
+    const int sector = ((dx < 0.0f ? 1 : 0) | (dz < 0.0f ? 2 : 0) | (swap ? 4 : 0)) * 4 + fine;
+    const float d2 = __fadd_rn(__fadd_rn(__fmul_rn(dx, dx), __fmul_rn(dy, dy)), __fmul_rn(dz, dz));
+    int ring = 0;
+#pragma unroll
+    for (int k = 1; k < 16; ++k) ring += d2 >= __fmul_rn((float)(k * k), thr2) ? 1 : 0;
+    return sector * 16 + ring;
+}
+template <int MODE>
 __global__ __launch_bounds__(EW) void k_ell_index(EdgeDev a) {
+    constexpr bool CLS = MODE == 1;
     extern __shared__ __attribute__((aligned(16))) unsigned char smem[];
     unsigned long long* bits = reinterpret_cast<unsigned long long*>(smem);
     __shared__ int wave_tot[EWAVES];
     __shared__ int n_shared;
     const int b = blockIdx.x, tid = threadIdx.x, lane = tid & 63, wave = tid >> 6;
+    __shared__ int tool_hist[MODE == 2 ? CHUNK_TOOL_KEYS : 1];
+    static_assert(CHUNK_TOOL_KEYS <= EW, "one thread per tool key");
+    int* tool_cnt = MODE == 2 ? a.ck_off + 2 + a.N * a.ell_stride + (long)b * CHUNK_TOOL_KEYS : nullptr;
     if (a.live && b >= *a.live) {
+        if (MODE == 2 && tid < CHUNK_TOOL_KEYS) tool_cnt[tid] = 0;
         if (tid == 0) { a.n_ns[b] = 0; a.n_edges[b] = 0; if (a.n_oo) a.n_oo[b] = 0; }
         return;
     }
     if (tid == 0) n_shared = 0;
+    if (MODE == 2 && tid < CHUNK_TOOL_KEYS) tool_hist[tid] = 0;
     int total = 0;
     {
         int part = 0;
@@ -685,7 +706,9 @@
     const int K = CLS ? a.n_cls : 1;
     const float* cpos = a.pos + (long)b * a.pos_bstride;
     const uint8_t* ctool = a.tool + (long)b * a.N;
-    int shared = 0;
+    int shared = 0, kept = 0;
+    unsigned long long* gbits = MODE == 2 ? a.ck_bits + (long)b * 2 * nw : nullptr;
+    const float ck_thr2 = MODE == 2 ? thr2_of(a, b, thr_of(a, b)) : 0.0f;
     constexpr int UN = 8;
     for (int eb = wave * 64; eb < nw * 64; eb += UN * EW) {
       int iu[UN], du[UN], ju[UN];
@@ -718,7 +741,14 @@
             pk[e] = v;
         }
         if (valid) recv[e] = i;
-        if (CLS) {
+        if (MODE == 2) {
+            bool tl = false;
+            if (own) tl = (ctool[i] | ctool[j]) != 0;
+            if (tl) atomicAdd(&tool_hist[chunk_tool_key(cpos, i, j, ck_thr2)], 1);
+            const unsigned long long bo = __ballot(own && !tl), bt = __ballot(tl);
+            if (lane == 0) { gbits[e0 >> 6] = bo; gbits[nw + (e0 >> 6)] = bt; }
+            kept += __popcll(bo) + __popcll(bt);
+        } else if (CLS) {
             int cls = 0;
             if (own) cls = (ctool[i] | ctool[j]) ? K - 1 : (K == 2 ? 0 : edge_class(cpos, i, j));
             unsigned long long keep = 0;
@@ -734,13 +764,15 @@
       }
     }
     if (hide) for (int i = tid; i < a.N; i += EW) deg[i] = 0;
-    __syncthreads();
-    const int nwt = K * nw;
+    if (MODE == 2 && lane == 63) wave_tot[wave] = kept;
+    __syncthreads();
+    const int nwt = MODE == 2 ? 0 : K * nw;
     const int per = (nwt + EW - 1) / EW;
     const int w0 = min(nwt, tid * per), w1 = min(nwt, w0 + per);
     int mine = 0;
     for (int w = w0; w < w1; ++w) mine += __popcll(bits[w]);
     int incl = mine;
+    if (MODE != 2) {
 #pragma unroll
     for (int o = 1; o < 64; o <<= 1) {
         const int v = __shfl_up(incl, o);
@@ -748,11 +780,14 @@
     }
     if (lane == 63) wave_tot[wave] = incl;
     __syncthreads();
+    }
     int before = 0, all = 0;
 #pragma unroll
     for (int w = 0; w < EWAVES; ++w) { const int v = wave_tot[w]; before += w < wave ? v : 0; all += v; }
     int pos = before + incl - mine;
-    if (CLS) {
+    if (MODE == 2) {
+        if (tid < CHUNK_TOOL_KEYS) tool_cnt[tid] = tool_hist[tid];
+    } else if (CLS) {
         const int wt = (K - 1) * nw;
         for (int w = w0; w < w1; ++w) {
             if (w == wt) a.n_oo[b] = pos;
@@ -786,6 +821,113 @@
         if (pk && a.share_stats) {
             atomicAdd(a.share_stats + 0, (unsigned long long)n_shared);
             atomicAdd(a.share_stats + 1, (unsigned long long)all);
+        }
+    }
+}
+
+constexpr int CKW = 256;
+static_assert(CHUNK_TOOL_KEYS == 32 * 16, "chunk_tool_key: 32 sectors x 16 rings");
+__global__ __launch_bounds__(CKW) void k_chunk_count(EdgeDev a) {
+    const int lane = threadIdx.x & 63;
+    const int nslots = a.N * a.ell_stride, nw = (nslots + 63) >> 6;
+    const int w = __builtin_amdgcn_readfirstlane((int)(blockIdx.x * (CKW / 64) + (threadIdx.x >> 6)));
+    if (w >= nw) return;
+    const int live = a.live ? min(*a.live, a.B) : a.B;
+    int n = 0;
+    for (int b0 = 0; b0 < live; b0 += 64) {
+        const unsigned long long m = b0 + lane < live ? a.ck_bits[(long)(b0 + lane) * 2 * nw + w] : 0ull;
+#pragma unroll
+        for (int s = 0; s < 64; ++s) {
+            const unsigned long long who = __ballot((m >> s & 1ull) != 0);
+            if (lane == s) n += __popcll(who);
+        }
+    }
+    const int e = w * 64 + lane;
+    if (e < nslots) { const int i = e / a.ell_stride, t = e - i * a.ell_stride; a.ck_off[2 + t * a.N + i] = n; }
+}
+__global__ __launch_bounds__(CKW) void k_chunk_fill(EdgeDev a) {
+    const int lane = threadIdx.x & 63;
+    const int nslots = a.N * a.ell_stride, nw = (nslots + 63) >> 6, wgs = (nw + CKW / 64 - 1) / (CKW / 64);
+    const int blk = (int)blockIdx.x % wgs, part = (int)blockIdx.x / wgs;
+    const int w = __builtin_amdgcn_readfirstlane(blk * (CKW / 64) + (int)(threadIdx.x >> 6));
+    if (w >= nw) return;
+    const int live = a.live ? min(*a.live, a.B) : a.B;
+    const int e = w * 64 + lane;
+    if (part == 0) {
+        int next = 0;
+        if (e < nslots) { const int i = e / a.ell_stride, t = e - i * a.ell_stride; next = a.ck_off[2 + t * a.N + i]; }
+        for (int b0 = 0; b0 < live; b0 += 64) {
+            const unsigned long long m = b0 + lane < live ? a.ck_bits[(long)(b0 + lane) * 2 * nw + w] : 0ull;
+            const unsigned cand = (unsigned)(b0 + lane) << a.ck_shift | (unsigned)(w * 64);
+#pragma unroll
+            for (int s = 0; s < 64; ++s) {
+                const bool mine = (m >> s & 1ull) != 0;
+                const unsigned long long who = __ballot(mine);
+                const int at = __builtin_amdgcn_readlane(next, s);
+                if (mine) a.ck_list[at + __popcll(who & lanes_below(lane))] = cand | (unsigned)s;
+                if (lane == s) next += __popcll(who);
+            }
+        }
+        return;
+    }
+    const int b = part - 1;
+    if (b >= live) return;
+    const unsigned long long m = a.ck_bits[((long)b * 2 + 1) * nw + w];
+    if (!(m >> lane & 1ull)) return;
+    const int i = e / a.ell_stride;
+    const int j = a.ell[(long)b * a.ell_bstride + e];
+    const int key = chunk_tool_key(a.pos + (long)b * a.pos_bstride, i, j, thr2_of(a, b, thr_of(a, b)));
+    const int at = atomicAdd(a.ck_off + 2 + nslots + (long)b * CHUNK_TOOL_KEYS + key, 1);
+    a.ck_list[at] = (unsigned)b << a.ck_shift | (unsigned)e;
+}
+__global__ __launch_bounds__(EW) void k_chunk_scan(EdgeDev a) {
+    __shared__ int wave_tot[EWAVES];
+    __shared__ int ktot[CHUNK_TOOL_KEYS];
+    const int tid = threadIdx.x, lane = tid & 63, wave = tid >> 6;
+    const int nslots = a.N * a.ell_stride, nk = nslots + CHUNK_TOOL_KEYS;
+    int* off = a.ck_off + 2;
+    int* tool = off + nslots;
+    if (tid < CHUNK_TOOL_KEYS) {
+        int tot = 0;
+#pragma unroll 8
+        for (int b = 0; b < a.B; ++b) tot += tool[(long)b * CHUNK_TOOL_KEYS + tid];
+        ktot[tid] = tot;
+    }
+    __syncthreads();
+    const int per = (nk + EW - 1) / EW;
+    const int k0 = min(nk, tid * per), k1 = min(nk, k0 + per);
+    int mine = 0;
+    for (int k = k0; k < k1; ++k) mine += k < nslots ? off[k] : ktot[k - nslots];
+    int incl = mine;
+#pragma unroll
+    for (int o = 1; o < 64; o <<= 1) {
+        const int v = __shfl_up(incl, o);
+        if (lane >= o) incl += v;
+    }
+    if (lane == 63) wave_tot[wave] = incl;
+    __syncthreads();
+    int before = 0, all = 0;
+#pragma unroll
+    for (int w = 0; w < EWAVES; ++w) { const int v = wave_tot[w]; before += w < wave ? v : 0; all += v; }
+    int pos = before + incl - mine;
+    for (int k = k0; k < k1; ++k) {
+        if (k == nslots) a.ck_off[1] = pos;
+        if (k < nslots) { const int n = off[k]; off[k] = pos; pos += n; }
+        else { const int n = ktot[k - nslots]; ktot[k - nslots] = pos; pos += n; }
+    }
+    if (tid == 0) a.ck_off[0] = all;
+    __syncthreads();
+    if (tid < CHUNK_TOOL_KEYS) {
+        int at = ktot[tid];
+        for (int b0 = 0; b0 < a.B; b0 += 8) {
+            int n[8];
+#pragma unroll
+            for (int u = 0; u < 8; ++u) n[u] = b0 + u < a.B ? tool[(long)(b0 + u) * CHUNK_TOOL_KEYS + tid] : 0;
+#pragma unroll
+            for (int u = 0; u < 8; ++u) {
+                if (b0 + u < a.B) tool[(long)(b0 + u) * CHUNK_TOOL_KEYS + tid] = at;
+                at += n[u];
+            }
         }
     }
 }
@@ -801,6 +943,7 @@
     a.ell_stride = a.ell_full ? h.ell_stride : a.k;
     a.ell_bstride = a.ell_full ? h.ell_bstride : (long)h.N * a.k;
     a.ns_edge = h.ns_edge; a.n_ns = h.n_ns; a.n_oo = h.n_oo; a.n_cls = 1;
+    a.ck_bits = h.ck_bits; a.ck_off = h.ck_off; a.ck_list = h.ck_list; a.ck_shift = h.ck_shift;
     a.recv = h.recv; a.send = h.send; a.row_ptr = h.row_ptr; a.n_edges = h.n_edges; a.overflow = h.overflow;
     a.max_nR = h.max_nR; a.zero_on_overflow = h.zero_on_overflow; a.live = h.live;
     a.send_pk = a.ell_full ? h.send_pk : nullptr; a.base_send = h.base_send; a.base_deg = h.base_deg; a.base_stride = h.base_stride;
@@ -818,10 +961,10 @@
         e = hipFuncSetAttribute(reinterpret_cast<const void*>(k_edge_emit), hipFuncAttributeMaxDynamicSharedMemorySize,
                                 160 * 1024 - 256);
         if (e != hipSuccess) return e;
-        e = hipFuncSetAttribute(reinterpret_cast<const void*>(k_ell_index<false>), hipFuncAttributeMaxDynamicSharedMemorySize,
+        e = hipFuncSetAttribute(reinterpret_cast<const void*>(k_ell_index<0>), hipFuncAttributeMaxDynamicSharedMemorySize,
                                 160 * 1024 - 256);
         if (e != hipSuccess) return e;
-        e = hipFuncSetAttribute(reinterpret_cast<const void*>(k_ell_index<true>), hipFuncAttributeMaxDynamicSharedMemorySize,
+        e = hipFuncSetAttribute(reinterpret_cast<const void*>(k_ell_index<1>), hipFuncAttributeMaxDynamicSharedMemorySize,
                                 160 * 1024 - 256);
         if (e != hipSuccess) return e;
         if (dev_id < 64) attr_devices |= 1ull << dev_id;
@@ -835,8 +978,15 @@
         if (nw > ELL_BITMAP_MAX_WORDS64) return hipErrorInvalidValue;
         const long budget = h.lds_words > 0 && h.lds_words < ELL_BITMAP_MAX_WORDS64 ? h.lds_words : ELL_BITMAP_MAX_WORDS64;
         a.n_cls = !a.n_oo ? 1 : ELL_CLASSES * nw <= budget ? ELL_CLASSES : 2 * nw <= budget ? 2 : 1;
-        if (a.n_cls > 1) hipLaunchKernelGGL(k_ell_index<true>, dim3(h.B), dim3(EW), (size_t)a.n_cls * nw * 8, st, a);
-        else hipLaunchKernelGGL(k_ell_index<false>, dim3(h.B), dim3(EW), (size_t)nw * 8, st, a);
+        if (a.ck_list) {
+            const unsigned wgs = (unsigned)((nw + CKW / 64 - 1) / (CKW / 64));
+            hipLaunchKernelGGL(k_ell_index<2>, dim3(h.B), dim3(EW), 0, st, a);
+            hipLaunchKernelGGL(k_chunk_count, dim3(wgs), dim3(CKW), 0, st, a);
+            hipLaunchKernelGGL(k_chunk_scan, dim3(1), dim3(EW), 0, st, a);
+            hipLaunchKernelGGL(k_chunk_fill, dim3(wgs * ((unsigned)h.B + 1u)), dim3(CKW), 0, st, a);
+        }
+        else if (a.n_cls > 1) hipLaunchKernelGGL(k_ell_index<1>, dim3(h.B), dim3(EW), (size_t)a.n_cls * nw * 8, st, a);
+        else hipLaunchKernelGGL(k_ell_index<0>, dim3(h.B), dim3(EW), (size_t)nw * 8, st, a);
     }
     else hipLaunchKernelGGL(k_edge_emit, dim3(h.B * h.slices), dim3(EW), lds, st, a);
     if (mark) mark(mark_ctx, FAM_EDGE_EMIT, 1);
diff --git a/adaptigraph_amd/csrc/ag_host.h b/adaptigraph_amd/csrc/ag_host.h
--- a/adaptigraph_amd/csrc/ag_host.h
+++ b/adaptigraph_amd/csrc/ag_host.h
@@ -24,6 +24,7 @@
 void diag_destroy(void* diag);
 int diag_fail_at_chunk(void* diag);
 int diag_timing_skip(void* diag);
+void diag_chunk_dump(void* diag, const EdgeArgs& ea, int n_tools, hipStream_t st);
 #endif
 
 struct Slab {
@@ -151,6 +152,7 @@
     int* ell; int* deg; int* slice_tot; int* cta_flag;
     int* recv; int* send; int* row_ptr; int* n_edges;
     int* ns_edge; int* n_ns; int* n_oo;
+    unsigned long long* ck_bits; int* ck_off; unsigned* ck_list;
     int* send_pk;
     int* rowlist; int* n_rows;
 };
@@ -177,6 +179,7 @@
 int clamp_chunk_for_offsets(int Bc, int N, int c_cap);
 int auto_chunk(const ag_ctx* c, int B, int N);
 bool lat_node_for(const ag_ctx* c, const GraphBufs& g);
+bool lat_edge_for(const ag_ctx* c, const GraphBufs& g);
 hipError_t node_enc_for(const ag_ctx* c, const GraphBufs& g, long row0, long nrows, hipStream_t st);
 int run_edge_chain(ag_ctx* c, const GraphBufs& g, hipStream_t st);
 int run_model(ag_ctx* c, const GraphBufs& g, float* pred_pos, float* pred_motion, hipStream_t st);
diff --git a/adaptigraph_amd/csrc/ag_mlp.hip b/adaptigraph_amd/csrc/ag_mlp.hip
--- a/adaptigraph_amd/csrc/ag_mlp.hip
+++ b/adaptigraph_amd/csrc/ag_mlp.hip
@@ -281,6 +281,7 @@
     long row0, nrows;
     const int* ns_edge; const int* n_ns;
     const int* n_oo;
+    const unsigned* ck_list; const int* ck_n; int ck_shift;
     const float* wb3;
     const float* Uin; const float* Vin; const int* deg; int ell_stride; int dedupe; unsigned self_row; const int* n_guard;
     int stagger_ticks; unsigned first_wave;
@@ -509,12 +510,13 @@
     int zi = 0;
     asm volatile("" : "+s"(zi));
     const float* const wts = g.w + zi;
-    const int b = (int)(blk % (unsigned)g.B);
-    const int e0 = (int)(blk / (unsigned)g.B) * WG_ROWS;
-    const int ne = g.n_ns ? g.n_ns[b] : g.n_edges[b];
+    const bool ck = g.ck_list != nullptr;
+    const int b = ck ? 0 : (int)(blk % (unsigned)g.B);
+    const int e0 = (int)(ck ? blk : blk / (unsigned)g.B) * WG_ROWS;
+    const int ne = ck ? g.ck_n[0] : g.n_ns ? g.n_ns[b] : g.n_edges[b];
     if (e0 >= ne) continue;
     int skip = 0;
-    if (ZS_EDGE) skip = g.zero_skip && (ZS_EDGE_ALL || (g.n_oo && e0 < g.n_oo[b])) ? 1 : 0;
+    if (ZS_EDGE) skip = g.zero_skip && (ZS_EDGE_ALL || (ck ? e0 < g.ck_n[1] : g.n_oo && e0 < g.n_oo[b])) ? 1 : 0;
 #ifdef AG_DIAG
     if (g.dbg && tid == 0) {
         g.dbg[blk * 4 + 0] = __builtin_amdgcn_s_memtime();
@@ -527,10 +529,13 @@
 
     const int t = e0 + wave * 32 + (lane & 31);
     const bool valid = t < ne;
-    const int el = g.ns_edge ? g.ns_edge[(long)b * g.edge_cap + (valid ? t : 0)] : t;
+    const unsigned ent = ck ? g.ck_list[valid ? t : e0] : 0u;
+    const int bl = ck ? (int)(ent >> g.ck_shift) : b;
+    const int el = ck ? (int)(ent & ((1u << g.ck_shift) - 1u))
+                      : g.ns_edge ? g.ns_edge[(long)b * g.edge_cap + (valid ? t : 0)] : t;
     const int elc = valid ? el : (g.ns_edge ? el : 0);
-    const int r = g.recv[(long)b * g.edge_cap + elc], s = g.send[(long)b * g.edge_cap + elc];
-    const long pr = (long)b * g.N + r, ps = (long)b * g.N + s;
+    const int r = g.recv[(long)bl * g.edge_cap + elc], s = g.send[(long)bl * g.edge_cap + elc];
+    const long pr = (long)bl * g.N + r, ps = (long)bl * g.N + s;
     float f[8 * EDGE_L1_CHUNKS];
     {
         const float* nr = g.node_in + pr * NODE_IN; const float* nsnd = g.node_in + ps * NODE_IN;
@@ -560,7 +565,7 @@
     layer160<Q_FLOATS, true, false, ZS_EDGE, HS_EDGE>(lds, wts + WL::E_L3, wts + WL::E_W1, x, y, tid, lane, live_of<HS_EDGE>(x, skip, g.half_step));
     relu_one(y, lane);
     layer160<0, true, false, ZS_EDGE, HS_EDGE>(lds, wts + WL::E_W1, nullptr, y, x, tid, lane, live_of<HS_EDGE>(y, skip, g.half_step));
-    store_rows_t(x, g.C, (int)((long)b * g.c_cap + el), valid, stg, lane);
+    store_rows_t(x, g.C, (int)((long)bl * g.c_cap + el), valid, stg, lane);
 #ifdef AG_DIAG
     if (g.dbg && tid == 0) {
         g.dbg[blk * 4 + 2] = __builtin_amdgcn_s_memtime();
@@ -990,6 +995,7 @@
     d.cls_on = g.cls_on; d.N_o = g.N_o; d.M = g.M; d.first_round = 0; d.vmask = g.vmask; d.c_eff = g.c_eff; d.c_P = g.c_P;
     d.row0 = 0; d.nrows = (long)g.B * g.N;
     d.ns_edge = g.ns_edge; d.n_ns = g.n_ns; d.n_oo = g.n_oo;
+    d.ck_list = g.ck_list; d.ck_n = g.ck_n; d.ck_shift = g.ck_shift;
     d.wb3 = g.wb3;
     d.Uin = nullptr; d.Vin = nullptr; d.deg = g.deg; d.ell_stride = g.ell_stride; d.dedupe = g.c_self ? 1 : 0;
     d.self_row = (unsigned)g.self_row; d.n_guard = g.n_guard;
```

New measurement: 52470 rollout-steps/s (median of 6 runs). +3.6%, better.
